# YangHai-1218/SCFlow

Measured on AMD Instinct MI355X. Metric: image-pairs/sec at 256x256, 8 GRU iters, higher is better.
Workload: dtype f32

## Files before the change

### include/scflow_hip.h

```cpp
#ifndef SCFLOW_HIP_H
#define SCFLOW_HIP_H

#include <stdint.h>

#ifdef __cplusplus
extern "C" {
#endif

typedef void* scf_stream_t;

enum {
  SCF_OK = 0,
  SCF_EINVAL = -1,
  SCF_EUNSUPPORTED = -2,
  SCF_ELAUNCH = -3,
  SCF_ENODEVICE = -4
};

#define SCF_MAX_LEVELS 12

enum { SCF_ACT_NONE = 0, SCF_ACT_RELU = 1, SCF_ACT_SIGMOID = 2, SCF_ACT_TANH = 3 };

enum {
  SCF_CONV_PLAIN = 0,
  SCF_CONV_GRU_ZR = 1,
  SCF_CONV_GRU_Q = 2
};

#define SCF_ABI_MAJOR 5
#define SCF_VERSION (SCF_ABI_MAJOR * 100 + 3)
int scf_version(void);
const char* scf_error_string(int code);
int scf_device_count(void);

int scf_corr_build(const float* feat1, const float* feat2, float* const* levels,
                   int N, int C, int h, int w, int L, scf_stream_t stream);

int scf_corr_lookup(const float* const* levels, const float* flow, float* out,
                    int N, int h, int w, int r, int L, scf_stream_t stream);

int64_t scf_corr_level_floats(int h, int w, int level, int tiled);
unsigned scf_corr_preferred_layout(int h, int w, int r, int L);
int scf_corr_build_ex(const float* feat1, const float* feat2, float* const* levels, int N, int C,
                      int h, int w, int L, unsigned tiled_levels, scf_stream_t stream);
int scf_corr_lookup_ex(const float* const* levels, const float* flow, float* out, int N, int h,
                       int w, int r, int L, unsigned tiled_levels, scf_stream_t stream);

typedef struct scf_conv_desc {
  const float* in0; const float* in1;
  int32_t C0, C1;
  int64_t in0_nstride, in1_nstride;
  int32_t N, H, W;
  const float* wp;
  int64_t w_nstride;
  int32_t Mld;
  int32_t Cout;
  int32_t KH, KW, stride, pad_h, pad_w;
  int32_t KC;
  float* out; int64_t out_nstride;
  const float* bias;
  const float* scale; const float* shift;
  const float* res; int64_t res_nstride;
  float out_div;
  int32_t act, act2, act_split;
  int32_t mode;
  const float* gru_h; int64_t gru_h_nstride;
  float* gru_aux; int64_t gru_aux_nstride;
  const float* gru_z; int64_t gru_z_nstride;
  const void* wp_f16;
  const float* wp_a4;
  int32_t a4_groups;
  int32_t a4_mld;
  const float* wp_a4s;
  int32_t a4s_groups;
  const float* wp_thin;
  int32_t out_tile8x4;
  const float* wp_taps;
  const float* wp_a4t;
  int32_t a4t_groups;
  const float* wp_wino1d;
  const float* wp_wino;
  const float* wp_wino1d4;
  int32_t k_slices;
  int64_t out_slice_stride;
} scf_conv_desc;

int scf_conv2d(const scf_conv_desc* desc, scf_stream_t stream);

int scf_conv_workspace(scf_stream_t stream, float* ptr, int64_t floats);

int scf_conv2d_pair(const scf_conv_desc* a, const scf_conv_desc* b, scf_stream_t stream);

int64_t scf_pack_conv_weight_size(int Cout, int Cin, int KH, int KW, int KC);
int scf_pack_conv_weight(const float* w, int Cout, int Cin, int KH, int KW, int KC, float* out);
int64_t scf_pack_conv_weight_a4_size(int Cout, int Cin, int KH, int KW, int groups);
int scf_pack_conv_weight_a4(const float* w, int Cout, int Cin, int KH, int KW, int groups, float* out);
int64_t scf_pack_conv_weight_taps_size(int Cout, int Cin, int KH, int KW);
int scf_pack_conv_weight_taps(const float* w, int Cout, int Cin, int KH, int KW, float* out);
int64_t scf_pack_conv_weight_wino1d_size(int32_t Cout, int32_t Cin);
int scf_pack_conv_weight_wino1d(const float* w, int32_t Cout, int32_t Cin, float* out);
int64_t scf_pack_conv_weight_wino1d4_size(int32_t Cout, int32_t Cin);
int scf_pack_conv_weight_wino1d4(const float* w, int32_t Cout, int32_t Cin, float* out);
int64_t scf_pack_conv_weight_wino_size(int32_t Cout, int32_t Cin);
int scf_pack_conv_weight_wino(const float* w, int32_t Cout, int32_t Cin, float* out);

typedef struct scf_gru_pass {
  int32_t KH, KW, pad_h, pad_w;
  const float* wp_zr; const float* bias_zr;
  const float* wp_q; const float* bias_q;
  const float* wp_zr_a4; const float* wp_q_a4; int32_t a4_groups;
  const void* wp_zr_f16; const void* wp_q_f16;
  const float* wp_zr_k32; const float* wp_q_k32;
  const float* wp_zr_a4s; const float* wp_q_a4s; int32_t a4s_groups;
  const float* wp_zr_a4t; const float* wp_q_a4t; int32_t a4t_groups;
  const float* wp_zr_wino1d; const float* wp_q_wino1d;
  const float* wp_zr_wino1d4; const float* wp_q_wino1d4;
} scf_gru_pass;

int scf_sepconv_gru(float* hx, int64_t hx_nstride, int N, int Ch, int Cx, int H, int W,
                    const scf_gru_pass* passes, int npass, float* z, float* rh,
                    scf_stream_t stream);

int scf_sepconv_gru_ctx(float* hx, int64_t hx_nstride, int N, int Ch, int Cc, int Cx, int H, int W,
                        const scf_gru_pass* passes, int npass, const float* const* ctx,
                        int64_t ctx_nstride, float* z, float* rh, scf_stream_t stream);

typedef struct scf_iter_gn {
  const float* gamma; const float* beta; float* out;
  int32_t C, HW, G; float eps;
} scf_iter_gn;

typedef struct scf_scflow_iter {
  int32_t struct_size;
  int32_t N, H, W, h, w;
  int32_t L, radius; uint32_t tiled_levels; int32_t corr_channels;
  const float* levels[SCF_MAX_LEVELS];
  float* flow_lr;
  float* corr;
  int32_t mask_flow, mask_corr;
  const float* mask_prev;
  float* flow_masked;
  scf_conv_desc flow0, flow1, corr0, corr1, outn;
  float* flow_copy_dst;
  float* hx; int64_t hx_nstride; int32_t Ch, Cc, Cx, npass;
  scf_gru_pass gru[2];
  const float* ctx[2]; int64_t ctx_nstride;
  float* z; float* rh;
  scf_conv_desc heads, fpred, mpred, menc0, menc1, denc0, denc1;
  scf_conv_desc pose[3];
  scf_iter_gn gn[3];
  const float* fc1_w; const float* fc1_b; float* fc1_out; int32_t fc1_K, fc1_O;
  const float* fc2_w; const float* fc2_b; float* fc2_out; int32_t fc2_O;
  int32_t fc_fused, fc1_slices, fc2_slices;
  const float* rot_w; const float* rot_b; float* rot_all; int32_t rot_O;
  const float* trans_w; const float* trans_b; float* trans_all; int32_t trans_O;
  const int64_t* label; int32_t num_class, label_mode;
  const float* depth; const float* K; const float* R0; const float* t0; float invalid_flow_num;
  const float* flow_in;
  const float* R_in; const float* t_in;
  float* flow_out; float* flow_pred; float* mask_up;
  float* R_out; float* t_out; float* d_rot; float* d_trans;
  scf_stream_t side_stream; int32_t overlap_flow, overlap_mask, overlap_up;
  void* lookup_timer;
} scf_scflow_iter;

int scf_scflow_iteration(const scf_scflow_iter* iter, scf_stream_t stream);

int scf_instance_norm(const float* x, const float* res, float* out, int64_t planes,
                      int HW, float eps, int relu, scf_stream_t stream);

int scf_group_norm_relu(const float* x, const float* gamma, const float* beta, float* out,
                        int N, int C, int HW, int G, float eps, scf_stream_t stream);
int scf_group_norm_relu_parts(const float* x, int parts, int64_t part_stride, const float* gamma,
                              const float* beta, float* out, int N, int C, int HW, int G, float eps,
                              scf_stream_t stream);

int scf_linear(const float* x, const float* W, const float* b, float* y, int N, int K,
               int O, int act, scf_stream_t stream);

int scf_linear_pair(const float* x, const float* W1, const float* b1, float* y1, int O1,
                    const float* W2, const float* b2, float* y2, int O2, int N, int K, int act,
                    scf_stream_t stream);

typedef struct scf_fc_desc {
  const float* x; int32_t x_parts; int64_t x_part_stride;
  const float* x_bias; int32_t x_relu;
  int32_t gn_groups, gn_hw; const float* gn_gamma; const float* gn_beta; float gn_eps;
  int32_t N, K;
  const float* W; const float* bias; float* y; int32_t O;
  const float* W2; const float* bias2; float* y2; int32_t O2;
  int32_t act;
  int32_t slices;
} scf_fc_desc;
int scf_fc_splitk(const scf_fc_desc* desc, scf_stream_t stream);

#define SCF_POSE_LABEL_PER_SAMPLE 1
#define SCF_POSE_DEPTH_LINEAR 2
int scf_pose_update(const float* rot_all, const float* trans_all, const int64_t* label,
                    int num_class, int label_mode, const float* R_in, const float* t_in,
                    float* d_rot, float* d_trans, float* R_out, float* t_out, int N,
                    scf_stream_t stream);

int scf_reproject_flow(const float* depth, const float* K, const float* R0, const float* t0,
                       const float* R, const float* t, float* flow, int N, int H, int W,
                       float invalid_num, scf_stream_t stream);

int scf_pose_error(const double* verts, int nv, const double* gt_r, const double* gt_t,
                   const double* pred_r, const double* pred_t, const double* K,
                   const int* sample_idx, int nsel, int symmetric, double* err3d, double* err2d,
                   scf_stream_t stream);

int scf_flow_corr_2d3d(const float* flow, const float* depth, const float* occ, float occ_thresh,
                       const float* K, const float* R0, const float* t0, int N, int H, int W,
                       float* pts2d, float* pts3d, float* conf, int32_t* count, scf_stream_t stream);

enum { SCF_PNP_SAMPLE_ALL = 0, SCF_PNP_SAMPLE_TOPK = 1, SCF_PNP_SAMPLE_RANDOM = 2 };
typedef struct scf_pnp_params {
  int32_t iterations;
  float reproj_error;
  int32_t sample_mode;
  int32_t sample_num;
  uint64_t seed;
} scf_pnp_params;
int64_t scf_pnp_workspace_bytes(int N, int capacity, const scf_pnp_params* params);
int scf_pnp_ransac(const float* pts2d, const float* pts3d, const float* conf, const int32_t* count, int N,
                   int capacity, const float* K, const float* R_ref, const float* t_ref,
                   const scf_pnp_params* params, float* R, float* t, int32_t* ok, int32_t* inliers,
                   void* workspace, scf_stream_t stream);

typedef struct scf_mesh_store {
  const float* verts;
  const float* normals;
  const float* colors;
  const int32_t* faces;
  const int32_t* vert_offset;
  const int32_t* face_offset;
  int32_t num_classes;
  int32_t max_faces;
} scf_mesh_store;
typedef struct scf_render_params {
  int32_t H, W;
  int32_t default_lights;
  int32_t seperate_lights;
  float background[3];
  float norm_mean[3];
  float norm_std[3];
} scf_render_params;
double scf_render_pixel_coord(int index, int size, int other);
int64_t scf_render_workspace_bytes(int N, int max_faces);
int scf_render_mesh(const scf_mesh_store* mesh, const int32_t* labels, const float* R, const float* t,
                    const float* K, int N, const scf_render_params* params, float* zbuf, int32_t* pix_to_face,
                    float* rgba, float* rgb_nchw, void* workspace, scf_stream_t stream);

typedef struct scf_patch_params {
  double aspect_ratio;
  double size_ratio;
  double min_expand;
  int32_t out_h, out_w;
  int32_t resize;
  int32_t vertex_stride;
  int32_t keep_ratio;
  int32_t clip_border;
  int32_t fix_clip_border_quirk;
  int32_t center;
  int32_t to_rgb;
  int32_t crop_pad_val[3];
  int32_t pad_val[3];
  float mean[3];
  float std[3];
} scf_patch_params;
int64_t scf_patch_workspace_bytes(int N);
int scf_patch_boxes(const scf_mesh_store* mesh, const int32_t* labels, const float* R, const float* t,
                    const float* K, const int32_t* crop_in, int N, int frame_h, int frame_w,
                    const scf_patch_params* params, float* box, int32_t* crop, float* scale, float* transform_matrix,
                    float* k, int32_t* valid, void* workspace, scf_stream_t stream);
int scf_patch_extract(const uint8_t* frames, int F, int frame_h, int frame_w, const int32_t* frame_index, int N,
                      const void* workspace, const scf_patch_params* params, float* out, scf_stream_t stream);

int scf_filter_flow_by_mask(float* flow, const float* mask, int N, int H, int W,
                            float invalid_num, int align_corners, scf_stream_t stream);

int64_t scf_cal_epe_workspace_bytes(int N, int H, int W);
int scf_cal_epe(const float* flow_tgt, const float* flow_pred, const float* mask, int N, int H, int W,
                float max_flow, const float* threshs, int nthr, int fix_threshold_quirk, float* err_map,
                float* mean, float* ratios, float* total_mean, float* total_ratios, void* workspace,
                scf_stream_t stream);

int scf_unproject_depth(const float* depth, const float* K, const float* R0, const float* t0,
                        float* pts, int N, int H, int W, scf_stream_t stream);

int scf_resize_bilinear(const float* a, const float* b, float* out, int64_t planes, int Hin,
                        int Win, int Hout, int Wout, float mul, scf_stream_t stream);

int scf_convex_upsample(const float* x, const float* mask, float* out, int N, int C, int h,
                        int w, int scale, float x_mul, float mask_mul, scf_stream_t stream);

int scf_avgpool2x2(const float* x, float* out, int64_t planes, int Hin, int Win,
                   scf_stream_t stream);

int scf_mul_mask(const float* x, int64_t x_nstride, const float* mask, float* out,
                 int64_t out_nstride, int N, int C, int HW, scf_stream_t stream);

int scf_copy_strided(const float* src, int64_t src_nstride, float* dst, int64_t dst_nstride,
                     int N, int64_t count, scf_stream_t stream);

#ifdef __cplusplus
}
#endif
#endif
```

### include/scflow_hip_prof.h

```cpp
#ifndef SCFLOW_HIP_PROF_H
#define SCFLOW_HIP_PROF_H

#include "scflow_hip.h"

#ifdef __cplusplus
extern "C" {
#endif

typedef void* scf_timer_t;
int scf_timer_create(scf_timer_t* timer);
int scf_timer_destroy(scf_timer_t timer);
int scf_timer_elapsed_us(scf_timer_t timer, float* microseconds);
int scf_timer_arm(scf_timer_t timer);

int scf_conv2d_query(const scf_conv_desc* desc, int32_t* info);

enum {
  SCF_KERNEL_THIN = 1,
  SCF_KERNEL_TAPS = 2,
  SCF_KERNEL_WINO = 3,
  SCF_KERNEL_WINO1D = 4,
  SCF_KERNEL_F16X3 = 5,
  SCF_KERNEL_DMA = 6,
  SCF_KERNEL_MFMA = 7,
  SCF_KERNEL_MFMA_KSPLIT = 8,
  SCF_KERNEL_WINO_Q = 9,
  SCF_KERNEL_WINO1D4 = 10
};
typedef struct scf_conv_log_entry {
  int32_t kernel;
  int32_t Cin, Cout, KH, KW, stride, Ho, Wo, N;
  int32_t mode;
  int32_t paired;
  int32_t variant;
} scf_conv_log_entry;
int scf_conv_log_enable(int capacity);
enum {
  SCF_TUNE_WINO_VARIANT = 1,
  SCF_TUNE_DMA_FORCE_KSPLIT = 2,
  SCF_TUNE_DMA_KSPLIT_GROUPS = 3,
  SCF_TUNE_WINO1D4 = 4,
  SCF_TUNE_CONV_AUTOSLICE = 7,
  SCF_TUNE_LOOKUP_STORE = 6,
  SCF_TUNE_ITER_MERGE = 8,
  SCF_TUNE_WINO1D4_HALF = 9,
  SCF_TUNE_CONV_PAIR = 10,
  SCF_TUNE_LOOKUP_PIPE = 5
};
int scf_tune(int key, int value);
int scf_conv_log_read(scf_conv_log_entry* out, int max_entries);

#ifdef __cplusplus
}
#endif
#endif
```

### scflow_amd/_lib.py

```python
from __future__ import annotations

import ctypes as C
import os

_HERE = os.path.dirname(os.path.abspath(__file__))
LIB_PATH = os.path.join(_HERE, 'csrc', 'libscflow_hip.so')

SCF_OK = 0
ACT_NONE, ACT_RELU, ACT_SIGMOID, ACT_TANH = 0, 1, 2, 3
CONV_PLAIN, CONV_GRU_ZR, CONV_GRU_Q = 0, 1, 2
MAX_LEVELS = 12
ABI_MAJOR = 5

_fp = C.c_void_p


class ConvDesc(C.Structure):
    _fields_ = [
        ('in0', _fp), ('in1', _fp),
        ('C0', C.c_int32), ('C1', C.c_int32),
        ('in0_nstride', C.c_int64), ('in1_nstride', C.c_int64),
        ('N', C.c_int32), ('H', C.c_int32), ('W', C.c_int32),
        ('wp', _fp), ('w_nstride', C.c_int64),
        ('Mld', C.c_int32), ('Cout', C.c_int32),
        ('KH', C.c_int32), ('KW', C.c_int32), ('stride', C.c_int32),
        ('pad_h', C.c_int32), ('pad_w', C.c_int32), ('KC', C.c_int32),
        ('out', _fp), ('out_nstride', C.c_int64),
        ('bias', _fp), ('scale', _fp), ('shift', _fp),
        ('res', _fp), ('res_nstride', C.c_int64),
        ('out_div', C.c_float),
        ('act', C.c_int32), ('act2', C.c_int32), ('act_split', C.c_int32),
        ('mode', C.c_int32),
        ('gru_h', _fp), ('gru_h_nstride', C.c_int64),
        ('gru_aux', _fp), ('gru_aux_nstride', C.c_int64),
        ('gru_z', _fp), ('gru_z_nstride', C.c_int64),
        ('wp_f16', _fp),
        ('wp_a4', _fp),
        ('a4_groups', C.c_int32),
        ('a4_mld', C.c_int32),
        ('wp_a4s', _fp),
        ('a4s_groups', C.c_int32),
        ('wp_thin', _fp),
        ('out_tile8x4', C.c_int32),
        ('wp_taps', _fp),
        ('wp_a4t', _fp),
        ('a4t_groups', C.c_int32),
        ('wp_wino1d', _fp),
        ('wp_wino', _fp),
        ('wp_wino1d4', _fp),
        ('k_slices', C.c_int32),
        ('out_slice_stride', C.c_int64),
    ]


class GruPass(C.Structure):
    _fields_ = [
        ('KH', C.c_int32), ('KW', C.c_int32), ('pad_h', C.c_int32), ('pad_w', C.c_int32),
        ('wp_zr', _fp), ('bias_zr', _fp), ('wp_q', _fp), ('bias_q', _fp),
        ('wp_zr_a4', _fp), ('wp_q_a4', _fp), ('a4_groups', C.c_int32),
        ('wp_zr_f16', _fp), ('wp_q_f16', _fp),
        ('wp_zr_k32', _fp), ('wp_q_k32', _fp),
        ('wp_zr_a4s', _fp), ('wp_q_a4s', _fp), ('a4s_groups', C.c_int32),
        ('wp_zr_a4t', _fp), ('wp_q_a4t', _fp), ('a4t_groups', C.c_int32),
        ('wp_zr_wino1d', _fp), ('wp_q_wino1d', _fp),
        ('wp_zr_wino1d4', _fp), ('wp_q_wino1d4', _fp),
    ]


class ConvLogEntry(C.Structure):
    _fields_ = [(n, C.c_int32) for n in ('kernel', 'Cin', 'Cout', 'KH', 'KW', 'stride', 'Ho', 'Wo', 'N', 'mode', 'paired', 'variant')]


KERNEL_NAMES = {1: 'thin', 2: 'taps', 3: 'winograd', 4: 'winograd F(2,5)', 5: 'f16x3', 6: 'direct-dma',
                7: 'direct-mfma', 8: 'direct-mfma-ksplit', 9: 'winograd-q', 10: 'winograd F(4,5)'}


class FcDesc(C.Structure):
    _fields_ = [('x', _fp), ('x_parts', C.c_int32), ('x_part_stride', C.c_int64),
                ('x_bias', _fp), ('x_relu', C.c_int32),
                ('gn_groups', C.c_int32), ('gn_hw', C.c_int32), ('gn_gamma', _fp), ('gn_beta', _fp), ('gn_eps', C.c_float),
                ('N', C.c_int32), ('K', C.c_int32),
                ('W', _fp), ('bias', _fp), ('y', _fp), ('O', C.c_int32),
                ('W2', _fp), ('bias2', _fp), ('y2', _fp), ('O2', C.c_int32),
                ('act', C.c_int32), ('slices', C.c_int32)]


class PnpParams(C.Structure):
    _fields_ = [('iterations', C.c_int32), ('reproj_error', C.c_float), ('sample_mode', C.c_int32),
                ('sample_num', C.c_int32), ('seed', C.c_uint64)]


PNP_SAMPLE_ALL, PNP_SAMPLE_TOPK, PNP_SAMPLE_RANDOM = 0, 1, 2


class MeshStore(C.Structure):
    _fields_ = [('verts', _fp), ('normals', _fp), ('colors', _fp), ('faces', _fp), ('vert_offset', _fp),
                ('face_offset', _fp), ('num_classes', C.c_int32), ('max_faces', C.c_int32)]


class RenderParams(C.Structure):
    _fields_ = [('H', C.c_int32), ('W', C.c_int32), ('default_lights', C.c_int32), ('seperate_lights', C.c_int32),
                ('background', C.c_float * 3), ('norm_mean', C.c_float * 3), ('norm_std', C.c_float * 3)]


class PatchParams(C.Structure):
    _fields_ = [('aspect_ratio', C.c_double), ('size_ratio', C.c_double), ('min_expand', C.c_double),
                ('out_h', C.c_int32), ('out_w', C.c_int32), ('resize', C.c_int32), ('vertex_stride', C.c_int32),
                ('keep_ratio', C.c_int32), ('clip_border', C.c_int32), ('fix_clip_border_quirk', C.c_int32),
                ('center', C.c_int32), ('to_rgb', C.c_int32), ('crop_pad_val', C.c_int32 * 3),
                ('pad_val', C.c_int32 * 3), ('mean', C.c_float * 3), ('std', C.c_float * 3)]


class IterGN(C.Structure):
    _fields_ = [('gamma', _fp), ('beta', _fp), ('out', _fp),
                ('C', C.c_int32), ('HW', C.c_int32), ('G', C.c_int32), ('eps', C.c_float)]


class ScflowIter(C.Structure):
    _fields_ = [
        ('struct_size', C.c_int32),
        ('N', C.c_int32), ('H', C.c_int32), ('W', C.c_int32), ('h', C.c_int32), ('w', C.c_int32),
        ('L', C.c_int32), ('radius', C.c_int32), ('tiled_levels', C.c_uint32), ('corr_channels', C.c_int32),
        ('levels', _fp * MAX_LEVELS),
        ('flow_lr', _fp), ('corr', _fp),
        ('mask_flow', C.c_int32), ('mask_corr', C.c_int32), ('mask_prev', _fp), ('flow_masked', _fp),
        ('flow0', ConvDesc), ('flow1', ConvDesc), ('corr0', ConvDesc), ('corr1', ConvDesc), ('outn', ConvDesc),
        ('flow_copy_dst', _fp),
        ('hx', _fp), ('hx_nstride', C.c_int64), ('Ch', C.c_int32), ('Cc', C.c_int32), ('Cx', C.c_int32),
        ('npass', C.c_int32),
        ('gru', GruPass * 2), ('ctx', _fp * 2), ('ctx_nstride', C.c_int64), ('z', _fp), ('rh', _fp),
        ('heads', ConvDesc), ('fpred', ConvDesc), ('mpred', ConvDesc), ('menc0', ConvDesc), ('menc1', ConvDesc),
        ('denc0', ConvDesc), ('denc1', ConvDesc),
        ('pose', ConvDesc * 3), ('gn', IterGN * 3),
        ('fc1_w', _fp), ('fc1_b', _fp), ('fc1_out', _fp), ('fc1_K', C.c_int32), ('fc1_O', C.c_int32),
        ('fc2_w', _fp), ('fc2_b', _fp), ('fc2_out', _fp), ('fc2_O', C.c_int32),
        ('fc_fused', C.c_int32), ('fc1_slices', C.c_int32), ('fc2_slices', C.c_int32),
        ('rot_w', _fp), ('rot_b', _fp), ('rot_all', _fp), ('rot_O', C.c_int32),
        ('trans_w', _fp), ('trans_b', _fp), ('trans_all', _fp), ('trans_O', C.c_int32),
        ('label', _fp), ('num_class', C.c_int32), ('label_mode', C.c_int32),
        ('depth', _fp), ('K', _fp), ('R0', _fp), ('t0', _fp), ('invalid_flow_num', C.c_float),
        ('flow_in', _fp), ('R_in', _fp), ('t_in', _fp),
        ('flow_out', _fp), ('flow_pred', _fp), ('mask_up', _fp),
        ('R_out', _fp), ('t_out', _fp), ('d_rot', _fp), ('d_trans', _fp),
        ('side_stream', _fp), ('overlap_flow', C.c_int32), ('overlap_mask', C.c_int32), ('overlap_up', C.c_int32),
        ('lookup_timer', _fp),
    ]


SIGNATURES = {
    'scf_version': (C.c_int, []),
    'scf_error_string': (C.c_char_p, [C.c_int]),
    'scf_device_count': (C.c_int, []),
    'scf_corr_build': (C.c_int, [_fp, _fp, C.POINTER(_fp), C.c_int, C.c_int, C.c_int, C.c_int,
                                 C.c_int, _fp]),
    'scf_corr_lookup': (C.c_int, [C.POINTER(_fp), _fp, _fp, C.c_int, C.c_int, C.c_int, C.c_int,
                                  C.c_int, _fp]),
    'scf_corr_build_ex': (C.c_int, [_fp, _fp, C.POINTER(_fp), C.c_int, C.c_int, C.c_int, C.c_int,
                                    C.c_int, C.c_uint, _fp]),
    'scf_corr_lookup_ex': (C.c_int, [C.POINTER(_fp), _fp, _fp, C.c_int, C.c_int, C.c_int, C.c_int,
                                     C.c_int, C.c_uint, _fp]),
    'scf_corr_level_floats': (C.c_int64, [C.c_int, C.c_int, C.c_int, C.c_int]),
    'scf_corr_preferred_layout': (C.c_uint, [C.c_int, C.c_int, C.c_int, C.c_int]),
    'scf_pose_error': (C.c_int, [_fp, C.c_int, _fp, _fp, _fp, _fp, _fp, _fp, C.c_int, C.c_int, _fp, _fp, _fp]),
    'scf_filter_flow_by_mask': (C.c_int, [_fp, _fp, C.c_int, C.c_int, C.c_int, C.c_float, C.c_int, _fp]),
    'scf_cal_epe_workspace_bytes': (C.c_int64, [C.c_int, C.c_int, C.c_int]),
    'scf_cal_epe': (C.c_int, [_fp, _fp, _fp, C.c_int, C.c_int, C.c_int, C.c_float, C.POINTER(C.c_float), C.c_int, C.c_int,
                              _fp, _fp, _fp, _fp, _fp, _fp, _fp]),
    'scf_timer_create': (C.c_int, [C.POINTER(_fp)]),
    'scf_timer_destroy': (C.c_int, [_fp]),
    'scf_timer_arm': (C.c_int, [_fp]),
    'scf_timer_elapsed_us': (C.c_int, [_fp, C.POINTER(C.c_float)]),
    'scf_conv2d': (C.c_int, [C.POINTER(ConvDesc), _fp]),
    'scf_conv2d_pair': (C.c_int, [C.POINTER(ConvDesc), C.POINTER(ConvDesc), _fp]),
    'scf_conv2d_query': (C.c_int, [C.POINTER(ConvDesc), C.POINTER(C.c_int32)]),
    'scf_tune': (C.c_int, [C.c_int, C.c_int]),
    'scf_conv_log_enable': (C.c_int, [C.c_int]),
    'scf_conv_log_read': (C.c_int, [C.POINTER(ConvLogEntry), C.c_int]),
    'scf_pack_conv_weight_size': (C.c_int64, [C.c_int, C.c_int, C.c_int, C.c_int, C.c_int]),
    'scf_pack_conv_weight': (C.c_int, [_fp, C.c_int, C.c_int, C.c_int, C.c_int, C.c_int, _fp]),
    'scf_pack_conv_weight_a4_size': (C.c_int64, [C.c_int, C.c_int, C.c_int, C.c_int, C.c_int]),
    'scf_pack_conv_weight_a4': (C.c_int, [_fp, C.c_int, C.c_int, C.c_int, C.c_int, C.c_int, _fp]),
    'scf_pack_conv_weight_taps_size': (C.c_int64, [C.c_int, C.c_int, C.c_int, C.c_int]),
    'scf_pack_conv_weight_taps': (C.c_int, [_fp, C.c_int, C.c_int, C.c_int, C.c_int, _fp]),
    'scf_pack_conv_weight_wino1d_size': (C.c_int64, [C.c_int32, C.c_int32]),
    'scf_pack_conv_weight_wino1d': (C.c_int, [_fp, C.c_int32, C.c_int32, _fp]),
    'scf_pack_conv_weight_wino1d4_size': (C.c_int64, [C.c_int32, C.c_int32]),
    'scf_pack_conv_weight_wino1d4': (C.c_int, [_fp, C.c_int32, C.c_int32, _fp]),
    'scf_pack_conv_weight_wino_size': (C.c_int64, [C.c_int32, C.c_int32]),
    'scf_pack_conv_weight_wino': (C.c_int, [_fp, C.c_int32, C.c_int32, _fp]),
    'scf_sepconv_gru': (C.c_int, [_fp, C.c_int64, C.c_int, C.c_int, C.c_int, C.c_int, C.c_int,
                                  C.POINTER(GruPass), C.c_int, _fp, _fp, _fp]),
    'scf_sepconv_gru_ctx': (C.c_int, [_fp, C.c_int64, C.c_int, C.c_int, C.c_int, C.c_int, C.c_int,
                                      C.c_int, C.POINTER(GruPass), C.c_int, C.POINTER(_fp),
                                      C.c_int64, _fp, _fp, _fp]),
    'scf_scflow_iteration': (C.c_int, [C.POINTER(ScflowIter), _fp]),
    'scf_instance_norm': (C.c_int, [_fp, _fp, _fp, C.c_int64, C.c_int, C.c_float, C.c_int, _fp]),
    'scf_group_norm_relu': (C.c_int, [_fp, _fp, _fp, _fp, C.c_int, C.c_int, C.c_int, C.c_int,
                                      C.c_float, _fp]),
    'scf_conv_workspace': (C.c_int, [_fp, _fp, C.c_int64]),
    'scf_group_norm_relu_parts': (C.c_int, [_fp, C.c_int, C.c_int64, _fp, _fp, _fp, C.c_int, C.c_int, C.c_int, C.c_int,
                                            C.c_float, _fp]),
    'scf_fc_splitk': (C.c_int, [C.POINTER(FcDesc), _fp]),
    'scf_linear': (C.c_int, [_fp, _fp, _fp, _fp, C.c_int, C.c_int, C.c_int, C.c_int, _fp]),
    'scf_linear_pair': (C.c_int, [_fp, _fp, _fp, _fp, C.c_int, _fp, _fp, _fp, C.c_int, C.c_int, C.c_int,
                                  C.c_int, _fp]),
    'scf_pose_update': (C.c_int, [_fp, _fp, _fp, C.c_int, C.c_int, _fp, _fp, _fp, _fp, _fp, _fp,
                                  C.c_int, _fp]),
    'scf_reproject_flow': (C.c_int, [_fp, _fp, _fp, _fp, _fp, _fp, _fp, C.c_int, C.c_int,
                                     C.c_int, C.c_float, _fp]),
    'scf_flow_corr_2d3d': (C.c_int, [_fp, _fp, _fp, C.c_float, _fp, _fp, _fp, C.c_int, C.c_int, C.c_int,
                                     _fp, _fp, _fp, _fp, _fp]),
    'scf_pnp_workspace_bytes': (C.c_int64, [C.c_int, C.c_int, C.POINTER(PnpParams)]),
    'scf_pnp_ransac': (C.c_int, [_fp, _fp, _fp, _fp, C.c_int, C.c_int, _fp, _fp, _fp, C.POINTER(PnpParams),
                                 _fp, _fp, _fp, _fp, _fp, _fp]),
    'scf_render_pixel_coord': (C.c_double, [C.c_int, C.c_int, C.c_int]),
    'scf_render_workspace_bytes': (C.c_int64, [C.c_int, C.c_int]),
    'scf_render_mesh': (C.c_int, [C.POINTER(MeshStore), _fp, _fp, _fp, _fp, C.c_int, C.POINTER(RenderParams),
                                  _fp, _fp, _fp, _fp, _fp, _fp]),
    'scf_patch_workspace_bytes': (C.c_int64, [C.c_int]),
    'scf_patch_boxes': (C.c_int, [C.POINTER(MeshStore), _fp, _fp, _fp, _fp, _fp, C.c_int, C.c_int, C.c_int,
                                  C.POINTER(PatchParams), _fp, _fp, _fp, _fp, _fp, _fp, _fp, _fp]),
    'scf_patch_extract': (C.c_int, [_fp, C.c_int, C.c_int, C.c_int, _fp, C.c_int, _fp, C.POINTER(PatchParams), _fp,
                                    _fp]),
    'scf_unproject_depth': (C.c_int, [_fp, _fp, _fp, _fp, _fp, C.c_int, C.c_int, C.c_int, _fp]),
    'scf_resize_bilinear': (C.c_int, [_fp, _fp, _fp, C.c_int64, C.c_int, C.c_int, C.c_int,
                                      C.c_int, C.c_float, _fp]),
    'scf_convex_upsample': (C.c_int, [_fp, _fp, _fp, C.c_int, C.c_int, C.c_int, C.c_int, C.c_int,
                                      C.c_float, C.c_float, _fp]),
    'scf_avgpool2x2': (C.c_int, [_fp, _fp, C.c_int64, C.c_int, C.c_int, _fp]),
    'scf_mul_mask': (C.c_int, [_fp, C.c_int64, _fp, _fp, C.c_int64, C.c_int, C.c_int, C.c_int, _fp]),
    'scf_copy_strided': (C.c_int, [_fp, C.c_int64, _fp, C.c_int64, C.c_int, C.c_int64, _fp]),
}

_lib = None


class ScflowHipError(RuntimeError):
    pass


def load() -> C.CDLL:
    global _lib
    if _lib is not None:
        return _lib
    if not os.path.exists(LIB_PATH):
        raise ScflowHipError(
            f'{LIB_PATH} is missing: the HIP kernels are the product and there is no fallback. '
            'Build it with `python scflow_amd/csrc/build.py` (hipcc --offload-arch=gfx950).')
    lib = C.CDLL(LIB_PATH)
    lib.scf_version.restype = C.c_int
    have = lib.scf_version()
    if have // 100 != ABI_MAJOR:
        raise ScflowHipError(f'{LIB_PATH} was built with ABI major {have // 100}, this binding expects '
                             f'{ABI_MAJOR}: rebuild it (python scflow_amd/csrc/build.py --force)')
    for name, (res, args) in SIGNATURES.items():
        fn = getattr(lib, name)
        fn.restype = res
        fn.argtypes = args
    _lib = lib
    return lib


def check(code: int, what: str) -> None:
    if code != SCF_OK:
        msg = load().scf_error_string(code).decode()
        raise ScflowHipError(f'{what} failed: {msg} ({code})')
```

### scflow_amd/csrc/conv_kernels.h

```cpp
#pragma once
#include "scf_common.h"

struct ConvK {
  const float* in0; const float* in1;
  int C0, Cin;
  long long in0_ns, in1_ns;
  int H, W, Ho, Wo;
  const float* wp; long long w_ns;
  const void* wp16;
  const float* wthin;
  const float* wp4; int G4, Mld4;
  const float* wp4s; int G4s;
  const float* wp4t; int G4t;
  int Mld, Cout, Krows;
  int KH, KW, T, stride, pad_h, pad_w, KC, nchunk;
  int fc_log2, tiles_x, tiles_y, mblocks, PH, PW, PWin;
  int px_off;
  int in_step;
  int wvec;
  int out_tile;
  int ksplit;
  float* out; long long out_ns;
  const float* bias; const float* scale; const float* shift;
  const float* res; long long res_ns;
  float out_div;
  int out_div_pow2;
  int act, act2, act_split, mode;
  const float* gru_h; long long gru_h_ns;
  float* gru_aux; long long gru_aux_ns;
  const float* gru_z; long long gru_z_ns;
  int kslices;
  long long slice_ns;
  int slice_blocks;
};

struct ConvEpi {
  float* out; const float* res; const float* gru_h; float* gru_aux; const float* gru_z;
  int HWo;
};

__device__ __forceinline__ ConvEpi scf_conv_epi(const ConvK& p, int n) {
  ConvEpi e;
  e.out = p.out + (long long)n * p.out_ns;
  e.res = p.res ? p.res + (long long)n * p.res_ns : nullptr;
  e.gru_h = p.gru_h ? p.gru_h + (long long)n * p.gru_h_ns : nullptr;
  e.gru_aux = p.gru_aux ? p.gru_aux + (long long)n * p.gru_aux_ns : nullptr;
  e.gru_z = p.gru_z ? p.gru_z + (long long)n * p.gru_z_ns : nullptr;
  e.HWo = p.Ho * p.Wo;
  return e;
}

typedef float scf_f32x16 __attribute__((ext_vector_type(16)));
typedef float scf_f32x4 __attribute__((ext_vector_type(4)));

enum { SCF_EPI_AFFINE = 0, SCF_EPI_GENERAL = 1, SCF_EPI_GRU_ZR = 2, SCF_EPI_GRU_Q = 3 };

__device__ __forceinline__ int scf_conv_epi_kind(const ConvK& p) {
  if (p.mode == SCF_CONV_GRU_ZR) return SCF_EPI_GRU_ZR;
  if (p.mode == SCF_CONV_GRU_Q) return SCF_EPI_GRU_Q;
  const bool lin1 = p.act == SCF_ACT_NONE || p.act == SCF_ACT_RELU;
  const bool lin2 = p.act_split <= 0 || p.act2 == SCF_ACT_NONE || p.act2 == SCF_ACT_RELU;
  return (lin1 && lin2) ? SCF_EPI_AFFINE : SCF_EPI_GENERAL;
}

__device__ __forceinline__ void scf_epi_affine_group(const ConvK& p, const ConvEpi& e,
                                                     const float (&acc)[4], int cb, int pix,
                                                     bool use_div) {
  if (cb >= p.Cout) return;
  const bool full = cb + 3 < p.Cout;
  float v[4] = {acc[0], acc[1], acc[2], acc[3]};
  if (use_div) {
    if (p.out_div_pow2) {
      const float rd = 1.0f / p.out_div;
#pragma unroll
      for (int q = 0; q < 4; ++q) v[q] = v[q] * rd;
    } else {
#pragma unroll
      for (int q = 0; q < 4; ++q) v[q] = v[q] / p.out_div;
    }
  }
  int off = cb * e.HWo + pix;
  float r[4] = {0.f, 0.f, 0.f, 0.f};
  if (e.res) {
#pragma unroll
    for (int q = 0; q < 4; ++q)
      if (full || cb + q < p.Cout) r[q] = e.res[off + q * e.HWo];
  }
  if (p.bias) {
#pragma unroll
    for (int q = 0; q < 4; ++q) v[q] += p.bias[(full || cb + q < p.Cout) ? cb + q : cb];
  }
  if (p.scale) {
#pragma unroll
    for (int q = 0; q < 4; ++q) {
      const int c = (full || cb + q < p.Cout) ? cb + q : cb;
      v[q] = v[q] * p.scale[c] + p.shift[c];
    }
  }
  if (e.res) {
#pragma unroll
    for (int q = 0; q < 4; ++q) v[q] += r[q];
  }
#pragma unroll
  for (int q = 0; q < 4; ++q) {
    const int a = (p.act_split > 0 && cb + q >= p.act_split) ? p.act2 : p.act;
    if (a == SCF_ACT_RELU) v[q] = v[q] > 0.f ? v[q] : 0.f;
  }
#pragma unroll
  for (int q = 0; q < 4; ++q)
    if (full || cb + q < p.Cout) e.out[off + q * e.HWo] = v[q];
}

template <int KIND>
__device__ __forceinline__ void scf_epi_general_group(const ConvK& p, const ConvEpi& e,
                                                      const float (&acc)[4], int cb, int pix,
                                                      bool use_div) {
  const bool need_aux = (KIND == SCF_EPI_GENERAL) ? (e.res != nullptr) : true;
// ... 260 lines not shown
```

### scflow_amd/csrc/conv_mfma.hip

```cpp
#include <atomic>
#include <mutex>
#include <vector>
#include "scf_common.h"

typedef float f32x16 __attribute__((ext_vector_type(16)));
typedef float f32x4 __attribute__((ext_vector_type(4)));

#include "conv_kernels.h"

template <int WM, int WN, int NCP>
__device__ __forceinline__ void mfma_taps(f32x16 (&acc)[WM][WN], const float* wl, const float* pl,
                                          const int (&boff)[WN], int T, int KW, int KC, int BM,
                                          int PW, int PHW, int half, int l32) {
  for (int t = 0; t < T; ++t) {
    const int ky = t / KW, kx = t - ky * KW;
    const float* wt = wl + (t * KC + half) * BM + l32;
    const float* pt = pl + ky * PW + kx;
#pragma unroll
    for (int c = 0; c < NCP; ++c) {
      const int cp = 2 * c;
      float a[WM], b[WN];
#pragma unroll
      for (int i = 0; i < WM; ++i) a[i] = wt[cp * BM + i * 32];
#pragma unroll
// ... 272 lines not shown
      for (int t = 0; t < T; ++t) {
        const int ky = t / p.KW, kx = t - ky * p.KW;
        const float* wt = wl + (t * KC + half) * BM + l32;
        const float* pt = pl + ky * PW + kx + boff;
#pragma unroll
        for (int c = 0; c < NCP; ++c) {
          if (((t * NCP + c) & 3) == wave)
            acc = __builtin_amdgcn_mfma_f32_32x32x2f32(wt[2 * c * BM], pt[2 * c * PHW], acc, 0, 0, 0);
        }
      }
    }
  }

  __syncthreads();
  float* red = lds;
#pragma unroll
  for (int r = 0; r < 16; ++r) red[(wave * 16 + r) * 64 + lane] = acc[r];
  __syncthreads();
  float v[4];
#pragma unroll
  for (int q = 0; q < 4; ++q) {
    const int r = 4 * wave + q;
    v[q] = ((red[(0 * 16 + r) * 64 + lane] + red[(1 * 16 + r) * 64 + lane]) +
            red[(2 * 16 + r) * 64 + lane]) + red[(3 * 16 + r) * 64 + lane];
  }
  const int oy = ty0 + fr, ox = tx0 + fc;
  if (oy < p.Ho && ox < p.Wo) {
    const ConvEpi epi = scf_conv_epi(p, n);
    const int pixk = p.out_tile ? (((oy >> 2) * (p.Wo >> 3) + (ox >> 3)) * 32 + (oy & 3) * 8 + (ox & 7))
                                : oy * p.Wo + ox;
    scf_conv_epilogue_group(p, epi, v, m0 + 8 * wave + 4 * half, pixk, p.out_div != 1.0f);
  }
}

template <int KC>
static int launch_ksplit(const ConvK& k, int nblk, size_t lds_bytes, hipStream_t st) {
  scf_launch((conv_mfma_ksplit_kernel<KC>), dim3(nblk), dim3(256), lds_bytes, st, k);
  return scf_launch_status();
}

template <int WM, int WN>
static int launch_conv(const ConvK& k, int nblk, size_t lds_bytes, hipStream_t st) {
  if (k.KC == 32)
    scf_launch((conv_mfma_kernel<WM, WN, 32>), dim3(nblk), dim3(256), lds_bytes, st, k);
  else if (k.KC == 8)
    scf_launch((conv_mfma_kernel<WM, WN, 8>), dim3(nblk), dim3(256), lds_bytes, st, k);
  else
    scf_launch((conv_mfma_kernel<WM, WN, 2>), dim3(nblk), dim3(256), lds_bytes, st, k);
  return scf_launch_status();
}

static int next_pow2(int v) {
  int p = 1;
  while (p < v) p <<= 1;
  return p;
}

struct ConvPlan {
  ConvK k;
  int WM, WN;
  long long nblk;
  size_t lds_bytes;
};

static int conv_plan(const scf_conv_desc* d, ConvPlan* plan) {
  if (!d || !d->in0 || !d->wp || !d->out) return SCF_EINVAL;
  if (d->N <= 0 || d->H <= 0 || d->W <= 0 || d->C0 <= 0 || d->C1 < 0 || d->Cout <= 0) return SCF_EINVAL;
  if (d->KH <= 0 || d->KW <= 0 || d->stride <= 0 || d->pad_h < 0 || d->pad_w < 0) return SCF_EINVAL;
  if (d->C1 > 0 && !d->in1) return SCF_EINVAL;
  if (d->KC != 2 && d->KC != 8 && d->KC != 32) return SCF_EUNSUPPORTED;
  if (d->C1 > 0 && (d->C0 % d->KC) != 0) return SCF_EUNSUPPORTED;
  if (d->Mld < d->Cout) return SCF_EINVAL;
  if (d->mode == SCF_CONV_GRU_ZR && (!d->gru_h || !d->gru_aux || (d->Cout & 1))) return SCF_EINVAL;
  if (d->mode == SCF_CONV_GRU_Q && (!d->gru_h || !d->gru_z)) return SCF_EINVAL;
  if ((d->scale == nullptr) != (d->shift == nullptr)) return SCF_EINVAL;
  if (d->out_tile8x4 && (d->mode != SCF_CONV_PLAIN || d->res)) return SCF_EUNSUPPORTED;
  if (d->k_slices > 1) {
    if (d->k_slices > 16 || d->out_slice_stride < (int64_t)d->N * d->out_nstride) return SCF_EINVAL;
    if (d->bias || d->scale || d->res || d->act != SCF_ACT_NONE || d->act_split > 0 || d->mode != SCF_CONV_PLAIN ||
        d->out_tile8x4 || (d->out_div != 0.f && d->out_div != 1.f) || d->w_nstride != 0)
      return SCF_EINVAL;
  }

  ConvK& k = plan->k;
  k.in0 = d->in0; k.in1 = d->C1 > 0 ? d->in1 : nullptr;
  k.C0 = d->C0; k.Cin = d->C0 + d->C1;
  k.in0_ns = d->in0_nstride; k.in1_ns = d->in1_nstride;
  k.H = d->H; k.W = d->W;
  k.Ho = (d->H + 2 * d->pad_h - d->KH) / d->stride + 1;
  k.Wo = (d->W + 2 * d->pad_w - d->KW) / d->stride + 1;
  if (k.Ho <= 0 || k.Wo <= 0) return SCF_EINVAL;
  k.wp = d->wp; k.w_ns = d->w_nstride; k.Mld = d->Mld; k.Cout = d->Cout;
  k.wp16 = d->wp_f16;
  k.wthin = d->wp_thin;
  k.wp4 = d->wp_a4; k.G4 = d->a4_groups; k.Mld4 = d->a4_mld;
  k.wp4s = d->wp_a4s; k.G4s = d->a4s_groups;
  k.wp4t = d->wp_a4t; k.G4t = d->a4t_groups;
  k.out_tile = d->out_tile8x4;
  k.KH = d->KH; k.KW = d->KW; k.T = d->KH * d->KW; k.stride = d->stride; k.in_step = 1;
  k.pad_h = d->pad_h; k.pad_w = d->pad_w; k.KC = d->KC;
  k.nchunk = (k.Cin + k.KC - 1) / k.KC;
  k.Krows = d->w_nstride ? k.Cin * k.T : k.nchunk * k.KC * k.T;
  k.wvec = ((d->Mld & 3) == 0) && ((d->w_nstride & 3) == 0) && (((uintptr_t)d->wp & 15) == 0);
  k.out = d->out; k.out_ns = d->out_nstride;
  k.bias = d->bias; k.scale = d->scale; k.shift = d->shift;
  k.res = d->res; k.res_ns = d->res_nstride;
  k.out_div = d->out_div == 0.f ? 1.f : d->out_div;
  {
    int ex = 0;
    k.out_div_pow2 = (k.out_div > 0.f && frexpf(k.out_div, &ex) == 0.5f) ? 1 : 0;
  }
  k.act = d->act; k.act2 = d->act2; k.act_split = d->act_split; k.mode = d->mode;
  k.gru_h = d->gru_h; k.gru_h_ns = d->gru_h_nstride;
  k.gru_aux = d->gru_aux; k.gru_aux_ns = d->gru_aux_nstride;
  k.gru_z = d->gru_z; k.gru_z_ns = d->gru_z_nstride;
  k.kslices = d->k_slices > 1 ? d->k_slices : 1; k.slice_ns = d->out_slice_stride; k.slice_blocks = 0;

  int FC = next_pow2(k.Wo) < 32 ? next_pow2(k.Wo) : 32;
  if (k.Wo > 32) {
    int best_w = (k.Wo + 31) / 32 * 32;
    for (int c = 16; c >= 8; c >>= 1) {
      const int wpad = (k.Wo + c - 1) / c * c;
      if (wpad * 10 <= best_w * 9) { best_w = wpad; FC = c; }
    }
  }
  int fl = 0;
  while ((1 << fl) < FC) ++fl;
  k.fc_log2 = fl;
  const int FR = 32 / FC;

  const int frags_m = (k.Cout + 31) / 32;
  auto tiles = [&](int WN) {
    const int TR = WN * 4 * FR;
    return (long long)d->N * ((k.Ho + TR - 1) / TR) * ((k.Wo + FC - 1) / FC);
  };
  auto fits = [&](int WM, int WN, size_t* lds_out) {
    const int TR = WN * 4 * FR;
    const int PH = (TR - 1) * k.stride + k.KH, PW = (FC - 1) * k.stride + k.KW;
    const long long PE = (long long)k.KC * PH * PW, WE = (long long)k.KC * k.T * WM * 8;
    const size_t lds = ((size_t)k.KC * k.T * WM * 32 + (size_t)PE) * sizeof(float);
    if (lds_out) *lds_out = lds;
    return (PE + 255) / 256 <= pu_max(k.KC, WM * WN) && (WE + 255) / 256 <= wu_max(k.KC) && lds <= 64 * 1024;
  };
  int WM = frags_m >= 4 ? ((frags_m % 4 == 0 || frags_m % 3 != 0) ? 4 : 3) : frags_m;
  int WN = 1;
  auto nblocks = [&](int wm, int wn) { return tiles(wn) * ((frags_m + wm - 1) / wm); };
  while (WM > 1 && (nblocks(WM, 1) < 512 || !fits(WM, 1, nullptr))) {
    int next = WM - 1;
    while (next > 1 && frags_m % next != 0) --next;
    WM = next;
  }
  if (WM <= 2 && nblocks(WM, 2) >= 2048 && fits(WM, 2, nullptr)) WN = 2;
  size_t lds_bytes = 0;
  const bool normal_fits = fits(WM, WN, &lds_bytes);
  k.mblocks = (frags_m + WM - 1) / WM;
  {
    const int TR = WN * 4 * FR;
    k.PH = (TR - 1) * k.stride + k.KH;
    k.PW = (FC - 1) * k.stride + k.KW;
    k.tiles_y = (k.Ho + TR - 1) / TR;
    k.tiles_x = (k.Wo + FC - 1) / FC;
  }
  plan->nblk = (long long)d->N * k.tiles_y * k.tiles_x * k.mblocks;
  if (plan->nblk > 0x7fffffffLL) return SCF_EUNSUPPORTED;
  k.ksplit = 0;
  if (!normal_fits && !(WM == 1 && WN == 1)) return SCF_EUNSUPPORTED;
  if (WM == 1 && WN == 1 && (plan->nblk < 128 || !normal_fits)) {
    const int PHk = (FR - 1) * k.stride + k.KH, PWk = (FC - 1) * k.stride + k.KW;
    const long long PEk = (long long)k.KC * PHk * PWk, WEk = (long long)k.KC * k.T * 8;
    size_t ldsk = ((size_t)k.KC * k.T * 32 + (size_t)PEk) * sizeof(float);
    if (ldsk < 4 * 16 * 64 * sizeof(float)) ldsk = 4 * 16 * 64 * sizeof(float);
    if ((PEk + 255) / 256 <= pu_max(k.KC, 1) && (WEk + 255) / 256 <= wu_max(k.KC) && ldsk <= 64 * 1024) {
      k.ksplit = 1;
      k.PH = PHk; k.PW = PWk;
      k.tiles_y = (k.Ho + FR - 1) / FR;
      k.tiles_x = (k.Wo + FC - 1) / FC;
      k.mblocks = frags_m;
      lds_bytes = ldsk;
      plan->nblk = (long long)d->N * k.tiles_y * k.tiles_x * k.mblocks;
    }
  }
  if (!normal_fits && !k.ksplit) return SCF_EUNSUPPORTED;
  plan->WM = WM; plan->WN = WN; plan->lds_bytes = lds_bytes;
  return SCF_OK;
}

static bool want_f16x3(const scf_conv_desc* d) {
  return d->wp_f16 != nullptr && !d->out_tile8x4 && d->w_nstride == 0 && d->KH * d->KW > 1 && d->C0 + d->C1 >= 16;
}

static std::atomic<int> g_pair_mode{0};
static std::atomic<int> g_wino1d4{1};

static bool want_dma(const scf_conv_desc* d) {
  return (d->wp_a4 != nullptr || d->wp_a4s != nullptr) && (d->stride == 1 || d->stride == 2) &&
         d->w_nstride == 0 && d->a4_mld >= d->Cout;
}

int scf_conv_kcombine_launch(const ConvK& k, const float* parts, int S, long long slice_ns, int N, hipStream_t st);
int scf_conv_dma_autoslice(const ConvK& k, int N);
namespace {
struct KWorkspace { hipStream_t st; float* ptr; int64_t floats; };
std::mutex g_kws_mu;
std::vector<KWorkspace> g_kws;
std::atomic<int> g_autoslice{1};
}
extern "C" int scf_conv_workspace(scf_stream_t stream, float* ptr, int64_t floats) {
  if (floats < 0 || (ptr == nullptr) != (floats == 0)) return SCF_EINVAL;
  std::lock_guard<std::mutex> lk(g_kws_mu);
  hipStream_t st = scf_stream(stream);
  for (size_t i = 0; i < g_kws.size(); ++i)
    if (g_kws[i].st == st) {
      if (ptr) { g_kws[i].ptr = ptr; g_kws[i].floats = floats; }
      else g_kws.erase(g_kws.begin() + (long)i);
      return SCF_OK;
    }
  if (ptr) g_kws.push_back({st, ptr, floats});
  return SCF_OK;
}
static bool kws_lookup(hipStream_t st, float** ptr, int64_t* floats) {
  std::lock_guard<std::mutex> lk(g_kws_mu);
  for (const KWorkspace& w : g_kws)
    if (w.st == st) { *ptr = w.ptr; *floats = w.floats; return true; }
  return false;
}

struct ConvReq {
  int32_t* info = nullptr;
  ScfLaunchCap* cap = nullptr;
  int which = 0;
};

static int conv2d_walk(const scf_conv_desc* d, scf_stream_t stream, ConvReq& r) {
  ConvPlan pl;
  const int rc = conv_plan(d, &pl);
  if (rc != SCF_OK) return rc;
  const ConvK& k = pl.k;
  const int N = d->N;
  const bool dry = r.info || r.cap;
  int32_t scratch[4];
  int32_t* info = r.info ? r.info : r.cap ? scratch : nullptr;
  hipStream_t st = scf_stream(stream);
  int out = SCF_EUNSUPPORTED;
  auto took = [&](int which, int rf) { r.which = which; out = rf; return rf != SCF_EUNSUPPORTED; };
  if (d->k_slices > 1) {
    r.which = SCF_KERNEL_DMA;
    return want_dma(d) ? scf_conv_dma_dispatch(k, N, dry, info, st, r.cap) : SCF_EUNSUPPORTED;
  }
  if (took(SCF_KERNEL_THIN, scf_conv_thin_dispatch(k, N, dry, st, r.cap))) return out;
  if (d->wp_taps && took(SCF_KERNEL_TAPS, scf_conv_taps_dispatch(k, d->wp_taps, N, dry, info, st, r.cap))) return out;
  if (d->wp_wino) {
    int quarter = 0;
    const int rw = scf_conv_wino_dispatch(k, d->wp_wino, N, dry, info, st, &quarter, r.cap);
    if (took(quarter ? SCF_KERNEL_WINO_Q : SCF_KERNEL_WINO, rw)) return out;
  }
  const int w4 = g_wino1d4.load(std::memory_order_relaxed);
  if (d->wp_wino1d4 && w4 && took(SCF_KERNEL_WINO1D4, scf_conv_wino1d4_dispatch(k, d->wp_wino1d4, N, w4 == 2, dry, info, st)))
    return out;
  if (d->wp_wino1d && took(SCF_KERNEL_WINO1D, scf_conv_wino1d_dispatch(k, d->wp_wino1d, N, dry, info, st))) return out;
  if (want_f16x3(d) && took(SCF_KERNEL_F16X3, scf_conv_f16x3_dispatch(k, N, dry, info, st))) return out;
  if (want_dma(d)) {
    float* ws = nullptr;
    int64_t ws_floats = 0;
    const bool sliced = !r.info && g_autoslice.load(std::memory_order_relaxed) && kws_lookup(st, &ws, &ws_floats);
    if (sliced && !dry) {
      const int S = scf_conv_dma_autoslice(k, N);
      const int64_t per_slice = (int64_t)N * d->Cout * k.Ho * k.Wo;
      if (S > 1 && per_slice * S <= ws_floats) {
        ConvK part = k;
        part.out = ws; part.out_ns = (long long)d->Cout * k.Ho * k.Wo;
        part.bias = nullptr; part.scale = nullptr; part.shift = nullptr; part.res = nullptr; part.res_ns = 0;
        part.out_div = 1.f; part.out_div_pow2 = 1; part.act = SCF_ACT_NONE; part.act2 = SCF_ACT_NONE; part.act_split = 0;
        part.mode = SCF_CONV_PLAIN; part.gru_h = nullptr; part.gru_aux = nullptr; part.gru_z = nullptr;
        part.kslices = S; part.slice_ns = per_slice;
        r.which = SCF_KERNEL_DMA;
        const int rs = scf_conv_dma_dispatch(part, N, false, nullptr, st);
        if (rs == SCF_OK) return scf_conv_kcombine_launch(k, ws, S, per_slice, N, st);
        if (rs != SCF_EUNSUPPORTED) return rs;
      }
    }
    if (took(SCF_KERNEL_DMA, scf_conv_dma_dispatch(k, N, dry, info, st, r.cap))) {
      if (sliced && r.cap) r.cap->variant = -1;
      return out;
    }
  }
  r.which = k.ksplit ? SCF_KERNEL_MFMA_KSPLIT : SCF_KERNEL_MFMA;
  const int WM = pl.WM, WN = pl.WN;
  if (dry) {
    if (r.info) {
      r.info[0] = WM; r.info[1] = WN; r.info[2] = (int32_t)pl.nblk;
      r.info[3] = k.T * (k.KC / 2) * WM * WN / (k.ksplit ? 4 : 1);
    }
    return SCF_OK;
  }
  const int nblk = (int)pl.nblk;
  if (k.ksplit) {
    if (k.KC == 32) return launch_ksplit<32>(k, nblk, pl.lds_bytes, st);
    if (k.KC == 8) return launch_ksplit<8>(k, nblk, pl.lds_bytes, st);
    return launch_ksplit<2>(k, nblk, pl.lds_bytes, st);
  }
#define SCF_CASE(M, Nn) if (WM == M && WN == Nn) return launch_conv<M, Nn>(k, nblk, pl.lds_bytes, st);
  SCF_CASE(1, 1) SCF_CASE(1, 2) SCF_CASE(2, 1) SCF_CASE(2, 2)
  SCF_CASE(3, 1) SCF_CASE(4, 1)
#undef SCF_CASE
  return SCF_EUNSUPPORTED;
}

namespace {
std::mutex g_log_mu;
std::vector<scf_conv_log_entry> g_log;
std::atomic<int> g_log_cap{0};
}

int scf_wino_variant_set(int v);
int scf_dma_force_ksplit_set(int v);
int scf_dma_ksplit_groups_set(int v);
int scf_lookup_pipe_set(int v);
int scf_lookup_store_set(int v);
int scf_iter_merge_set(int v);
int scf_wino1d4_half_set(int v);

extern "C" int scf_tune(int key, int value) {
  if (key == SCF_TUNE_WINO_VARIANT) return scf_wino_variant_set(value);
  if (key == SCF_TUNE_DMA_FORCE_KSPLIT) return scf_dma_force_ksplit_set(value);
  if (key == SCF_TUNE_DMA_KSPLIT_GROUPS) return scf_dma_ksplit_groups_set(value);
  if (key == SCF_TUNE_LOOKUP_PIPE) return scf_lookup_pipe_set(value);
  if (key == SCF_TUNE_LOOKUP_STORE) return scf_lookup_store_set(value);
  if (key == SCF_TUNE_ITER_MERGE) return scf_iter_merge_set(value);
  if (key == SCF_TUNE_WINO1D4_HALF) return scf_wino1d4_half_set(value);
  if (key == SCF_TUNE_CONV_AUTOSLICE) {
    if (value < 0 || value > 1) return SCF_EINVAL;
    return g_autoslice.exchange(value);
  }
  if (key == SCF_TUNE_CONV_PAIR) {
    if (value < 0 || value > 1) return SCF_EINVAL;
    return g_pair_mode.exchange(value);
  }
  if (key == SCF_TUNE_WINO1D4) {
    if (value < 0 || value > 2) return SCF_EINVAL;
    return g_wino1d4.exchange(value);
  }
  return SCF_EINVAL;
}

extern "C" int scf_conv_log_enable(int capacity) {
  std::lock_guard<std::mutex> lk(g_log_mu);
  g_log.clear();
  if (capacity > 0) g_log.reserve((size_t)capacity);
  else g_log.shrink_to_fit();
  g_log_cap.store(capacity > 0 ? capacity : 0);
  return SCF_OK;
}

extern "C" int scf_conv_log_read(scf_conv_log_entry* out, int max_entries) {
  std::lock_guard<std::mutex> lk(g_log_mu);
  const int n = (int)g_log.size();
  if (out)
    for (int i = 0; i < n && i < max_entries; ++i) out[i] = g_log[(size_t)i];
  return n;
}

static void conv_log_push(const scf_conv_desc* d, int which, int paired, int variant = -1);
extern "C" int scf_conv2d(const scf_conv_desc* d, scf_stream_t stream) {
  ConvReq r;
  const int rc = conv2d_walk(d, stream, r);
  if (rc == SCF_OK) conv_log_push(d, r.which, 0);
  return rc;
}

static void conv_log_push(const scf_conv_desc* d, int which, int paired, int variant) {
  if (g_log_cap.load(std::memory_order_relaxed) <= 0) return;
  std::lock_guard<std::mutex> lk(g_log_mu);
  if ((int)g_log.size() >= g_log_cap.load()) return;
  scf_conv_log_entry e;
  e.kernel = which; e.Cin = d->C0 + d->C1; e.Cout = d->Cout; e.KH = d->KH; e.KW = d->KW; e.stride = d->stride;
  e.Ho = (d->H + 2 * d->pad_h - d->KH) / d->stride + 1;
  e.Wo = (d->W + 2 * d->pad_w - d->KW) / d->stride + 1;
  e.N = d->N; e.mode = d->mode; e.paired = paired; e.variant = variant;
  g_log.push_back(e);
}

static bool pairable(int which, const ScfLaunchCap& c) {
  switch (which) {
    case SCF_KERNEL_THIN: return true;
    case SCF_KERNEL_TAPS: return c.variant >= 1;
    case SCF_KERNEL_WINO_Q: return c.variant >= 10 && c.variant < 20;
    case SCF_KERNEL_WINO: return c.variant >= 20;
    case SCF_KERNEL_DMA: return c.variant >= 0;
    default: return false;
  }
}

static bool capture(const scf_conv_desc* d, scf_stream_t stream, ScfLaunchCap* cap, int* which) {
  ConvReq r;
  r.cap = cap;
  const bool ok = conv2d_walk(d, stream, r) == SCF_OK && pairable(r.which, *cap);
  *which = r.which;
  return ok;
}

typedef int (*PairLaunch)(const ScfLaunchCap&, const ScfLaunchCap&, hipStream_t);

extern "C" int scf_conv2d_pair(const scf_conv_desc* a, const scf_conv_desc* b, scf_stream_t stream) {
  if (!a || !b) return SCF_EINVAL;
  ScfLaunchCap ca, cb;
  int fa = 0, fb = 0;
  if (g_pair_mode.load(std::memory_order_relaxed) != 1 && capture(a, stream, &ca, &fa) && capture(b, stream, &cb, &fb)) {
    const size_t lmax = ca.ldsb > cb.ldsb ? ca.ldsb : cb.ldsb;
    const long long slots = (long long)scf_cu_count() * (((fa == SCF_KERNEL_DMA || fb == SCF_KERNEL_DMA) && lmax > 80 * 1024) ? 1 : 2);
    const long long na = ca.nblk, nb = cb.nblk;
    auto rounds = [](long long n, long long s) { return (n + s - 1) / s; };
    auto fewer_rounds = [&](long long s) { return rounds(na + nb, s) < rounds(na, s) + rounds(nb, s); };
// ... 128 lines not shown
```

### scflow_amd/csrc/conv_taps.hip

```cpp
#include "scf_common.h"
#include "conv_kernels.h"
#include "scf_dma.h"

#include "conv_taps_body.h"

template <int WM>
__global__ __launch_bounds__(256, 2) void conv_taps_kernel(ConvK p, const float* __restrict__ wt, int Kp, int PWp) {
  conv_taps_body<WM>(p, wt, Kp, PWp, (int)blockIdx.x, (int)gridDim.x);
}

template <int WMA, int WMB>
__global__ __launch_bounds__(256, 2) void conv_taps_pair_kernel(ConvK pa, const float* __restrict__ wta, int Kpa, int PWpa, ConvK pb,
                                                                const float* __restrict__ wtb, int Kpb, int PWpb, int nba) {
  if ((int)blockIdx.x < nba) conv_taps_body<WMA>(pa, wta, Kpa, PWpa, (int)blockIdx.x, nba);
  else conv_taps_body<WMB>(pb, wtb, Kpb, PWpb, (int)blockIdx.x - nba, (int)gridDim.x - nba);
}

#define CT_MAXU 12

template <int WM>
__global__ __launch_bounds__(256, 2) void conv_taps_persist_kernel(ConvK p, const float* __restrict__ wt, int Kp, int PWp, int ntiles) {
  extern __shared__ __attribute__((aligned(16))) float ct_lds[];
  constexpr int BM = WM * 32;
  const int tid = threadIdx.x, lane = tid & 63;
  const int wave = __builtin_amdgcn_readfirstlane(tid >> 6);
  const int l32 = lane & 31, half = lane >> 5;

  const int lb = scf_xcd_remap(blockIdx.x, gridDim.x);
  const int mblk = __builtin_amdgcn_readfirstlane(lb % p.mblocks);
  const int slot = __builtin_amdgcn_readfirstlane(lb / p.mblocks);
  const int nslots = __builtin_amdgcn_readfirstlane((int)gridDim.x / p.mblocks);
  const int m0 = mblk * BM;
  const int FC = 1 << p.fc_log2, FR = 32 >> p.fc_log2, TR = 4 * FR;
  const int st = p.stride;
  const int PH = p.PH, PHW = PH * PWp, T = p.T;
  const int q4 = BM / 4, n4 = Kp * q4;
  const int w_cells = (n4 + 63) & ~63;
  const int PE = p.Cin * PHW;
  const int x_cells = (PE + 63) & ~63;
  float* Ws = ct_lds;
  float* Xs = Ws + w_cells * 4;
  int* koff = (int*)(Xs + 2 * x_cells);
  const int HW = p.H * p.W;

  int rel[CT_MAXU], pyx[CT_MAXU];
  {
    const float rPHW = 1.0f / (float)PHW, rPW = 1.0f / (float)PWp;
#pragma unroll
    for (int u = 0; u < CT_MAXU; ++u) {
      rel[u] = -1; pyx[u] = 0;
      if (wave * 64 + u * 256 >= x_cells) continue;
      const int e = wave * 64 + u * 256 + lane;
      int c = (int)((float)e * rPHW);
      int r = e - c * PHW;
      if (r < 0) { --c; r += PHW; } else if (r >= PHW) { ++c; r -= PHW; }
      int py = (int)((float)r * rPW);
      int px = r - py * PWp;
      if (px < 0) { --py; px += PWp; } else if (px >= PWp) { ++py; px -= PWp; }
      rel[u] = e < PE ? c * HW + py * p.W + px : -1;
      pyx[u] = (py << 16) | px;
    }
  }
  auto tile_coords = [&](int tile, int& n, int& ty0, int& tx0) {
    const int txi = __builtin_amdgcn_readfirstlane(tile % p.tiles_x);
    const int t2 = tile / p.tiles_x;
    const int tyi = __builtin_amdgcn_readfirstlane(t2 % p.tiles_y);
    n = __builtin_amdgcn_readfirstlane(t2 / p.tiles_y);
    ty0 = tyi * TR; tx0 = txi * FC;
  };
  const unsigned xl = scf_lds_addr(Xs);
  auto stage_x = [&](int tile, int b) {
    int n, ty0, tx0;
    tile_coords(tile, n, ty0, tx0);
    const int iy0 = ty0 * st - p.pad_h, ix0 = tx0 * st - p.pad_w;
    const scf_rsrc4 xrs = scf_make_rsrc(p.in0 + (long long)n * p.in0_ns, (unsigned)((long long)p.Cin * HW * 4));
    const int tbase = iy0 * p.W + ix0;
    const unsigned dst = xl + (unsigned)(b * x_cells + wave * 64) * 4u;
#pragma unroll
    for (int u = 0; u < CT_MAXU; ++u) {
      if (wave * 64 + u * 256 < x_cells) {
        const int iy = iy0 + (pyx[u] >> 16), ix = ix0 + (pyx[u] & 0xffff);
        const bool ok = rel[u] >= 0 && (unsigned)iy < (unsigned)p.H && (unsigned)ix < (unsigned)p.W;
        scf_bdma_b32(xrs, ok ? (unsigned)((rel[u] + tbase) * 4) : SCF_BUF_OOB, dst + (unsigned)u * 1024u);
      }
    }
  };

  {
    const scf_rsrc4 wrs = scf_make_rsrc(wt + m0, (unsigned)(((long long)(Kp - 1) * p.Mld + BM) * 4));
    const unsigned wl = scf_lds_addr(Ws);
    for (int c0 = wave * 64; c0 < w_cells; c0 += 256) {
      const int e = c0 + lane;
      const int row = e / q4, c4 = e - row * q4;
      const unsigned voff = e < n4 ? (unsigned)((row * p.Mld + 4 * c4) * 4) : SCF_BUF_OOB;
      scf_bdma_b128(wrs, voff, wl + (unsigned)c0 * 16u);
    }
  }
  if (slot < ntiles) stage_x(slot, 0);
  for (int k = tid; k < Kp; k += 256) {
    int o = 0;
    if (k < p.Cin * T) {
      const int c = k / T, t = k - c * T;
      const int ky = t / p.KW, kx = t - ky * p.KW;
      o = c * PHW + ky * PWp + kx;
    }
    koff[k] = o;
  }
  __builtin_amdgcn_s_waitcnt(0x0F70);
  __syncthreads();

  const int fr = l32 >> p.fc_log2, fc = l32 & (FC - 1);
  const float* wb = Ws + half * BM + l32;
  const int* kb = koff + half;
  const int ntrip = Kp >> 3;
  int buf = 0;
#pragma nounroll
  for (int tile = slot; tile < ntiles; tile += nslots) {
    if (tile + nslots < ntiles) stage_x(tile + nslots, buf ^ 1);

    ct_f32x16 acc[WM][1];
#pragma unroll
    for (int i = 0; i < WM; ++i)
#pragma unroll
      for (int r = 0; r < 16; ++r) acc[i][0][r] = 0.f;

    const float* xb = Xs + buf * x_cells + ((wave * FR + fr) * st) * PWp + fc * st;
    int oN[4];
    float bC[4], aC[4][WM];
#pragma unroll
    for (int u = 0; u < 4; ++u) oN[u] = kb[2 * u];
#pragma unroll
    for (int u = 0; u < 4; ++u) {
      bC[u] = xb[oN[u]];
#pragma unroll
      for (int i = 0; i < WM; ++i) aC[u][i] = wb[2 * u * BM + 32 * i];
    }
    {
      const int t1 = ntrip > 1 ? 1 : 0;
#pragma unroll
      for (int u = 0; u < 4; ++u) oN[u] = kb[8 * t1 + 2 * u];
    }
#pragma nounroll
    for (int t = 0; t < ntrip; ++t) {
      const int tn = t + 1 < ntrip ? t + 1 : ntrip - 1, tnn = t + 2 < ntrip ? t + 2 : ntrip - 1;
      float bN[4], aN[4][WM];
      int oNN[4];
#pragma unroll
      for (int u = 0; u < 4; ++u) {
        bN[u] = xb[oN[u]];
#pragma unroll
        for (int i = 0; i < WM; ++i) aN[u][i] = wb[(8 * tn + 2 * u) * BM + 32 * i];
      }
#pragma unroll
      for (int u = 0; u < 4; ++u) oNN[u] = kb[8 * tnn + 2 * u];
      __builtin_amdgcn_sched_barrier(0);
#pragma unroll
      for (int u = 0; u < 4; ++u)
#pragma unroll
// ... 97 lines not shown
```

### scflow_amd/csrc/conv_taps_body.h

```cpp
#pragma once
#include "scf_common.h"
#include "conv_kernels.h"
#include "scf_dma.h"

typedef float ct_f32x16 __attribute__((ext_vector_type(16)));

template <int WM>
__device__ __forceinline__ void conv_taps_body(const ConvK& p, const float* __restrict__ wt, const int Kp, const int PWp, const int bid,
                                               const int nblk) {
  extern __shared__ __attribute__((aligned(16))) float ct_lds[];
  constexpr int BM = WM * 32;
  const int tid = threadIdx.x, lane = tid & 63;
  const int wave = __builtin_amdgcn_readfirstlane(tid >> 6);
  const int l32 = lane & 31, half = lane >> 5;

  const int lb = scf_xcd_remap(bid, nblk);
  const int mblk = __builtin_amdgcn_readfirstlane(lb % p.mblocks);
  const int tile = __builtin_amdgcn_readfirstlane(lb / p.mblocks);
  const int m0 = mblk * BM;
  const int FC = 1 << p.fc_log2, FR = 32 >> p.fc_log2, TR = 4 * FR;
  const int txi = __builtin_amdgcn_readfirstlane(tile % p.tiles_x);
  const int t2 = tile / p.tiles_x;
  const int tyi = __builtin_amdgcn_readfirstlane(t2 % p.tiles_y);
  const int n = __builtin_amdgcn_readfirstlane(t2 / p.tiles_y);
  const int ty0 = tyi * TR, tx0 = txi * FC;
  const int st = p.stride;
  const int iy0 = ty0 * st - p.pad_h, ix0 = tx0 * st - p.pad_w;
  const int PH = p.PH, PHW = PH * PWp, T = p.T;
  const int q4 = BM / 4, n4 = Kp * q4;
  const int w_cells = (n4 + 63) & ~63;
  const int PE = p.Cin * PHW;
  const int x_cells = (PE + 63) & ~63;
  float* Ws = ct_lds;
  float* Xs = Ws + w_cells * 4;
  int* koff = (int*)(Xs + x_cells);

  {
    const scf_rsrc4 wrs = scf_make_rsrc(wt + m0, (unsigned)(((long long)(Kp - 1) * p.Mld + BM) * 4));
    const unsigned wl = scf_lds_addr(Ws);
    for (int c0 = wave * 64; c0 < w_cells; c0 += 256) {
      const int e = c0 + lane;
      const int row = e / q4, c4 = e - row * q4;
      const unsigned voff = e < n4 ? (unsigned)((row * p.Mld + 4 * c4) * 4) : SCF_BUF_OOB;
      scf_bdma_b128(wrs, voff, wl + (unsigned)c0 * 16u);
    }
    const int HW = p.H * p.W;
    const scf_rsrc4 xrs = scf_make_rsrc(p.in0 + (long long)n * p.in0_ns, (unsigned)((long long)p.Cin * HW * 4));
    const unsigned xl = scf_lds_addr(Xs);
    const float rPHW = 1.0f / (float)PHW, rPW = 1.0f / (float)PWp;
    for (int c0 = wave * 64; c0 < x_cells; c0 += 256) {
      const int e = c0 + lane;
      int c = (int)((float)e * rPHW);
      int r = e - c * PHW;
      if (r < 0) { --c; r += PHW; } else if (r >= PHW) { ++c; r -= PHW; }
      int py = (int)((float)r * rPW);
      int px = r - py * PWp;
      if (px < 0) { --py; px += PWp; } else if (px >= PWp) { ++py; px -= PWp; }
      const int iy = iy0 + py, ix = ix0 + px;
      const bool ok = e < PE && iy >= 0 && iy < p.H && ix >= 0 && ix < p.W;
      scf_bdma_b32(xrs, ok ? (unsigned)((c * HW + iy * p.W + ix) * 4) : SCF_BUF_OOB, xl + (unsigned)c0 * 4u);
    }
  }
  for (int k = tid; k < Kp; k += 256) {
    int o = 0;
    if (k < p.Cin * T) {
      const int c = k / T, t = k - c * T;
      const int ky = t / p.KW, kx = t - ky * p.KW;
      o = c * PHW + ky * PWp + kx;
    }
    koff[k] = o;
  }
  __builtin_amdgcn_s_waitcnt(0x0F70);
  __syncthreads();

  ct_f32x16 acc[WM][1];
#pragma unroll
  for (int i = 0; i < WM; ++i)
#pragma unroll
    for (int r = 0; r < 16; ++r) acc[i][0][r] = 0.f;

  const int fr = l32 >> p.fc_log2, fc = l32 & (FC - 1);
  const float* xb = Xs + ((wave * FR + fr) * st) * PWp + fc * st;
  const float* wb = Ws + half * BM + l32;
  const int* kb = koff + half;
  const int ntrip = Kp >> 3;
  int oN[4];
  float bC[4], aC[4][WM];
#pragma unroll
  for (int u = 0; u < 4; ++u) oN[u] = kb[2 * u];
#pragma unroll
  for (int u = 0; u < 4; ++u) {
    bC[u] = xb[oN[u]];
#pragma unroll
    for (int i = 0; i < WM; ++i) aC[u][i] = wb[2 * u * BM + 32 * i];
  }
  {
    const int t1 = ntrip > 1 ? 1 : 0;
#pragma unroll
    for (int u = 0; u < 4; ++u) oN[u] = kb[8 * t1 + 2 * u];
  }
  for (int t = 0; t < ntrip; ++t) {
    const int tn = t + 1 < ntrip ? t + 1 : ntrip - 1, tnn = t + 2 < ntrip ? t + 2 : ntrip - 1;
    float bN[4], aN[4][WM];
    int oNN[4];
#pragma unroll
    for (int u = 0; u < 4; ++u) {
      bN[u] = xb[oN[u]];
#pragma unroll
      for (int i = 0; i < WM; ++i) aN[u][i] = wb[(8 * tn + 2 * u) * BM + 32 * i];
    }
#pragma unroll
    for (int u = 0; u < 4; ++u) oNN[u] = kb[8 * tnn + 2 * u];
    __builtin_amdgcn_sched_barrier(0);
#pragma unroll
    for (int u = 0; u < 4; ++u)
#pragma unroll
      for (int i = 0; i < WM; ++i)
        acc[i][0] = __builtin_amdgcn_mfma_f32_32x32x2f32(aC[u][i], bC[u], acc[i][0], 0, 0, 0);
    __builtin_amdgcn_sched_barrier(0);
#pragma unroll
    for (int u = 0; u < 4; ++u) {
      bC[u] = bN[u];
      oN[u] = oNN[u];
#pragma unroll
      for (int i = 0; i < WM; ++i) aC[u][i] = aN[u][i];
    }
  }

  const ConvEpi epi = scf_conv_epi(p, n);
  int pix[1];
// ... 8 lines not shown
```

### scflow_amd/csrc/corr_gemm.hip

```cpp
#include "scf_common.h"

typedef float cg_f32x16 __attribute__((ext_vector_type(16)));

struct CorrGemmParams {
  const float* f1; const float* f2;
  float* lvl0; float* lvl1;
  int C, h, w, hw;
  int nchunk;
  int mblocks, nblocks;
  int tiled;
  int ntiles_x;
  float scale; int exact_scale;
  float divisor;
  int l1_pw4, l1_msz;
};

#define CG_KC 16
#define CG_BM 128
#define CG_BN 128
#define CG_STAGE_FLOATS (CG_KC * (CG_BM + CG_BN))
#define CG_NSTAGE 3

__device__ __forceinline__ unsigned cg_lds_addr(const void* p) {
  return (unsigned)(uintptr_t)(__attribute__((address_space(3))) const void*)p;
// ... 111 lines not shown
  float* o0 = p.lvl0 + (long long)n * hw * hw;
  float* o1 = POOL ? p.lvl1 + (long long)n * hw * hw1 : nullptr;
#pragma unroll
  for (int fj = 0; fj < 2; ++fj) {
    const int F = nb * 4 + wn * 2 + fj;
    bool fok;
    int pos0, pos1 = 0;
    bool pool_lane = false;
    if (TILED) {
      const int ntile = (p.h >> 2) * p.ntiles_x;
      fok = F < ntile;
      pos0 = F * 32 + l32;
      if (POOL) {
        const int ty = F / p.ntiles_x, tx = F - ty * p.ntiles_x;
        const int x = l32 & 7, y = l32 >> 3;
        pool_lane = fok && !(x & 1) && !(y & 1);
        const int y1 = ty * 2 + (y >> 1), x1 = tx * 4 + (x >> 1);
        pos1 = p.l1_pw4 ? (y1 >> 2) * p.l1_pw4 + (x1 >> 3) * 32 + (y1 & 3) * 8 + (x1 & 7) : y1 * w1 + x1;
      }
    } else {
      pos0 = F * 32 + l32;
      fok = pos0 < hw;
    }
#pragma unroll
    for (int fi = 0; fi < 2; ++fi) {
      const int ib = i0 + wm * 64 + fi * 32 + 4 * half;
#pragma unroll
      for (int r = 0; r < 16; ++r) {
        const int i = ib + (r & 3) + 8 * (r >> 2);
        float v = acc[fi][fj][r];
        v = p.exact_scale ? v * p.scale : v / p.divisor;
        if (fok && i < hw) o0[(long long)i * hw + pos0] = v;
        if (POOL) {
          const int vi = __builtin_bit_cast(int, v);
          const float vx = __builtin_bit_cast(float, __builtin_amdgcn_update_dpp(0, vi, 0xB1, 0xF, 0xF, false));
          const float vy = __builtin_bit_cast(float, __builtin_amdgcn_update_dpp(0, vi, 0x128, 0xF, 0xF, false));
          const float vxy = __builtin_bit_cast(float, __builtin_amdgcn_update_dpp(0, __builtin_bit_cast(int, vx), 0x128, 0xF, 0xF, false));
          const float s = (((v + vx) + vy) + vxy) * 0.25f;
          if (pool_lane && i < hw) o1[(long long)i * hw1 + pos1] = s;
        }
      }
    }
  }
}

static int corr_gemm_dispatch(const float* feat1, const float* feat2, float* lvl0, float* lvl1, int l1_tiled,
                              int N, int C, int h, int w, int tiled, hipStream_t st) {
  const long long hw = (long long)h * w;
  if (C % CG_KC != 0 || (hw & 3) != 0 || hw > 0x3fffffffLL) return SCF_EUNSUPPORTED;
  if ((long long)C * hw * 4 > 0x7fffffffLL) return SCF_EUNSUPPORTED;
  if (tiled && ((w & 7) || (h & 3))) return SCF_EUNSUPPORTED;
  if (lvl1 && (!tiled || h < 2 || w < 2)) return SCF_EUNSUPPORTED;
  if ((((uintptr_t)feat1 | (uintptr_t)feat2) & 15) != 0) return SCF_EUNSUPPORTED;
  CorrGemmParams p;
  p.f1 = feat1; p.f2 = feat2; p.lvl0 = lvl0; p.lvl1 = lvl1;
  p.C = C; p.h = h; p.w = w; p.hw = (int)hw;
  p.nchunk = C / CG_KC;
  p.mblocks = (int)((hw + CG_BM - 1) / CG_BM);
  p.tiled = tiled ? 1 : 0;
  p.ntiles_x = w >> 3;
  const long long nfrag = tiled ? (long long)(h >> 2) * (w >> 3) : (hw + 31) / 32;
  p.nblocks = (int)((nfrag + 3) / 4);
  const float sq = sqrtf((float)C);
  int ex = 0;
  p.exact_scale = (frexpf(sq, &ex) == 0.5f) ? 1 : 0;
  p.scale = 1.0f / sq;
  p.divisor = sq;
  p.l1_pw4 = (lvl1 && l1_tiled) ? (((w >> 1) + 7) / 8 * 8) * 4 : 0;
  p.l1_msz = lvl1 ? (int)scf_corr_level_floats(h, w, 1, l1_tiled) : 0;
  const long long nblk = (long long)N * p.mblocks * p.nblocks;
  if (nblk <= 0 || nblk > 0x7fffffffLL) return SCF_EUNSUPPORTED;
  const size_t lds = (size_t)CG_NSTAGE * CG_STAGE_FLOATS * sizeof(float);
  if (tiled) {
    if (lvl1) scf_launch((corr_gemm_kernel<true, true>), dim3((unsigned)nblk), dim3(256), lds, st, p);
    else scf_launch((corr_gemm_kernel<true, false>), dim3((unsigned)nblk), dim3(256), lds, st, p);
  } else {
    scf_launch((corr_gemm_kernel<false, false>), dim3((unsigned)nblk), dim3(256), lds, st, p);
  }
  return scf_launch_status();
}

int scf_avgpool2x2_layout(const float* x, float* out, int64_t planes, int Hin, int Win, int in_tiled,
                          int out_tiled, hipStream_t st);

extern "C" int scf_corr_build_ex(const float* feat1, const float* feat2, float* const* levels, int N,
                                 int C, int h, int w, int L, unsigned tiled_levels, scf_stream_t stream) {
  if (!feat1 || !feat2 || !levels || N <= 0 || C <= 0 || h <= 0 || w <= 0 || L <= 0) return SCF_EINVAL;
  if (L > SCF_MAX_LEVELS) return SCF_EUNSUPPORTED;
  if ((tiled_levels & 1u) && ((w & 7) || (h & 3))) return SCF_EUNSUPPORTED;
  for (int l = 0; l < L; ++l)
    if (!levels[l] || (h >> l) < 1 || (w >> l) < 1) return SCF_EINVAL;
  hipStream_t st = scf_stream(stream);
  const int hw = h * w;
  const int t0 = tiled_levels & 1u, t1 = (tiled_levels >> 1) & 1u;
  float* l1 = (t0 && L >= 2) ? levels[1] : nullptr;
  int rc = corr_gemm_dispatch(feat1, feat2, levels[0], l1, t1, N, C, h, w, t0, st);
  int done = (rc == SCF_OK && l1) ? 2 : 1;
  if (rc == SCF_EUNSUPPORTED) {
    scf_conv_desc d = {};
    d.in0 = feat2; d.C0 = C; d.in0_nstride = (int64_t)C * hw;
    d.N = N; d.H = h; d.W = w;
    d.wp = feat1; d.w_nstride = (int64_t)C * hw; d.Mld = hw; d.Cout = hw;
    d.KH = d.KW = 1; d.stride = 1; d.pad_h = d.pad_w = 0;
    d.KC = (C % 32 == 0) ? 32 : (C % 8 == 0) ? 8 : 2;
    d.out = levels[0]; d.out_nstride = (int64_t)hw * hw;
    d.out_div = sqrtf((float)C);
    d.act = SCF_ACT_NONE; d.mode = SCF_CONV_PLAIN;
    d.out_tile8x4 = t0;
    rc = scf_conv2d(&d, stream);
    done = 1;
  }
  if (rc != SCF_OK) return rc;
  for (int l = done; l < L; ++l) {
    rc = scf_avgpool2x2_layout(levels[l - 1], levels[l], (int64_t)N * hw, h >> (l - 1), w >> (l - 1),
                               (tiled_levels >> (l - 1)) & 1u, (tiled_levels >> l) & 1u, st);
    if (rc != SCF_OK) return rc;
  }
  return SCF_OK;
}

extern "C" int scf_corr_build(const float* feat1, const float* feat2, float* const* levels, int N,
                              int C, int h, int w, int L, scf_stream_t stream) {
  return scf_corr_build_ex(feat1, feat2, levels, N, C, h, w, L, 0u, stream);
}
```

### scflow_amd/csrc/norm.hip

```cpp
#include "scf_common.h"

__device__ __forceinline__ float wave_sum(float v) {
#pragma unroll
  for (int off = 32; off > 0; off >>= 1) v += __shfl_xor(v, off);
  return v;
}

template <int NT>
__device__ __forceinline__ float block_sum(float v, float* red) {
  v = wave_sum(v);
  const int wave = threadIdx.x >> 6, lane = threadIdx.x & 63;
  __syncthreads();
  if (lane == 0) red[wave] = v;
  __syncthreads();
  float s = 0.f;
#pragma unroll
  for (int w = 0; w < NT / 64; w += 4) s += (red[w] + red[w + 1]) + (red[w + 2] + red[w + 3]);
  return s;
}

__device__ __forceinline__ float block_sum_256(float v, float* red) {
  v = wave_sum(v);
  const int wave = threadIdx.x >> 6, lane = threadIdx.x & 63;
  __syncthreads();
// ... 13 lines not shown
  const int n4 = HW >> 2;
  float4 v[VEC4];
  float s = 0.f;
#pragma unroll
  for (int i = 0; i < VEC4; ++i) {
    const int idx = i * NT + threadIdx.x;
    v[i] = idx < n4 ? xp[idx] : make_float4(0.f, 0.f, 0.f, 0.f);
    s += (v[i].x + v[i].y) + (v[i].z + v[i].w);
  }
  const float mean = block_sum<NT>(s, red) / (float)HW;
  float q = 0.f;
#pragma unroll
  for (int i = 0; i < VEC4; ++i) {
    const int idx = i * NT + threadIdx.x;
    if (idx < n4) {
      const float a = v[i].x - mean, b = v[i].y - mean, c = v[i].z - mean, d = v[i].w - mean;
      q += (a * a + b * b) + (c * c + d * d);
    }
  }
  const float var = block_sum<NT>(q, red) / (float)HW;
  const float rstd = 1.0f / sqrtf(var + eps);
  float4* op = reinterpret_cast<float4*>(out + pl * HW);
  const float4* rp = res ? reinterpret_cast<const float4*>(res + pl * HW) : nullptr;
#pragma unroll
  for (int i = 0; i < VEC4; ++i) {
    const int idx = i * NT + threadIdx.x;
    if (idx < n4) {
      float4 o;
      o.x = (v[i].x - mean) * rstd;
      o.y = (v[i].y - mean) * rstd;
      o.z = (v[i].z - mean) * rstd;
      o.w = (v[i].w - mean) * rstd;
      if (rp) {
        const float4 r = rp[idx];
        o.x += r.x; o.y += r.y; o.z += r.z; o.w += r.w;
      }
      if (relu) {
        o.x = fmaxf(o.x, 0.f); o.y = fmaxf(o.y, 0.f); o.z = fmaxf(o.z, 0.f); o.w = fmaxf(o.w, 0.f);
      }
      scf_store4<(SCF_ST_SC1 & 2) != 0>(reinterpret_cast<float*>(op + idx), o.x, o.y, o.z, o.w);
    }
  }
}

__global__ __launch_bounds__(256) void instance_norm_generic_kernel(const float* x,
                                                                    const float* res,
                                                                    float* out, int HW,
                                                                    float eps, int relu) {
  __shared__ float red[4];
  const long long pl = blockIdx.x;
  const float* xp = x + pl * HW;
  float s = 0.f;
  for (int i = threadIdx.x; i < HW; i += 256) s += xp[i];
  const float mean = block_sum_256(s, red) / (float)HW;
  float q = 0.f;
  for (int i = threadIdx.x; i < HW; i += 256) {
    const float a = xp[i] - mean;
    q += a * a;
  }
  const float var = block_sum_256(q, red) / (float)HW;
  const float rstd = 1.0f / sqrtf(var + eps);
  for (int i = threadIdx.x; i < HW; i += 256) {
    float o = (xp[i] - mean) * rstd;
    if (res) o += res[pl * HW + i];
    if (relu) o = fmaxf(o, 0.f);
    out[pl * HW + i] = o;
  }
}

extern "C" int scf_instance_norm(const float* x, const float* res, float* out, int64_t planes,
                                 int HW, float eps, int relu, scf_stream_t stream) {
  if (!x || !out || planes <= 0 || HW <= 0) return SCF_EINVAL;
  if (planes > 0x7fffffffLL) return SCF_EUNSUPPORTED;
  hipStream_t st = scf_stream(stream);
  const dim3 grid((unsigned)planes), blk(256);
  const bool vec = (HW % 4 == 0) && ((((uintptr_t)x | (uintptr_t)out | (uintptr_t)res) & 15) == 0);
  const int n4 = HW / 4;
  if (vec && n4 <= 256) scf_launch(instance_norm_kernel<1>, grid, blk, 0, st, x, res, out, HW, eps, relu);
  else if (vec && n4 <= 1024) scf_launch(instance_norm_kernel<4>, grid, blk, 0, st, x, res, out, HW, eps, relu);
  else if (vec && n4 <= 4096) scf_launch(instance_norm_kernel<16>, grid, blk, 0, st, x, res, out, HW, eps, relu);
  else if (vec && n4 <= 8192) scf_launch((instance_norm_kernel<8, 1024>), grid, dim3(1024), 0, st, x, res, out, HW, eps, relu);
  else if (vec && n4 <= 20480) scf_launch((instance_norm_kernel<20, 1024>), grid, dim3(1024), 0, st, x, res, out, HW, eps, relu);
  else scf_launch(instance_norm_generic_kernel, grid, blk, 0, st, x, res, out, HW, eps, relu);
  return scf_launch_status();
}

__global__ __launch_bounds__(256) void group_norm_relu_kernel(const float* __restrict__ x, int parts,
                                                              long long part_stride,
                                                              const float* __restrict__ gamma,
                                                              const float* __restrict__ beta,
                                                              float* __restrict__ out, int C, int HW,
                                                              int G, float eps) {
  __shared__ float red[4];
  const int n = blockIdx.x / G, g = blockIdx.x % G;
  const int cpg = C / G;
  const int cnt = cpg * HW;
  const long long base = ((long long)n * C + (long long)g * cpg) * HW;
  const float* xp = x + base;
  auto at = [&](int i) {
    float v = xp[i];
    for (int sl = 1; sl < parts; ++sl) v += xp[(long long)sl * part_stride + i];
    return v;
  };
  constexpr int KEEP = 8;
  const bool keep = cnt <= KEEP * 256;
  float kv[KEEP];
  if (keep) {
    float u[4][KEEP];
#pragma unroll
    for (int j = 0; j < KEEP; ++j) {
      const int i = threadIdx.x + j * 256;
#pragma unroll
      for (int sl = 0; sl < 4; ++sl) u[sl][j] = (i < cnt && sl < parts) ? xp[(long long)sl * part_stride + i] : 0.f;
    }
#pragma unroll
    for (int j = 0; j < KEEP; ++j) {
      kv[j] = u[0][j];
#pragma unroll
      for (int sl = 1; sl < 4; ++sl)
        if (sl < parts) kv[j] += u[sl][j];
    }
    for (int sl = 4; sl < parts; ++sl) {
#pragma unroll
      for (int j = 0; j < KEEP; ++j) {
        const int i = threadIdx.x + j * 256;
        if (i < cnt) kv[j] += xp[(long long)sl * part_stride + i];
      }
    }
  }
  float s = 0.f;
  if (keep) {
#pragma unroll
    for (int j = 0; j < KEEP; ++j) s += kv[j];
  } else {
    for (int i = threadIdx.x; i < cnt; i += 256) s += at(i);
  }
  const float mean = block_sum_256(s, red) / (float)cnt;
  float q = 0.f;
  if (keep) {
#pragma unroll
    for (int j = 0; j < KEEP; ++j) {
      const float a = kv[j] - mean;
      q += (threadIdx.x + j * 256 < cnt) ? a * a : 0.f;
    }
  } else {
    for (int i = threadIdx.x; i < cnt; i += 256) {
      const float a = at(i) - mean;
      q += a * a;
    }
  }
  const float var = block_sum_256(q, red) / (float)cnt;
  const float rstd = 1.0f / sqrtf(var + eps);
  if (keep) {
#pragma unroll
    for (int j = 0; j < KEEP; ++j) {
      const int i = threadIdx.x + j * 256;
      if (i < cnt) {
        const int c = g * cpg + i / HW;
        out[base + i] = fmaxf((kv[j] - mean) * rstd * gamma[c] + beta[c], 0.f);
      }
    }
  } else {
    for (int i = threadIdx.x; i < cnt; i += 256) {
      const int c = g * cpg + i / HW;
      const float o = (at(i) - mean) * rstd * gamma[c] + beta[c];
      out[base + i] = fmaxf(o, 0.f);
// ... 102 lines not shown
```

### scflow_amd/csrc/resample.hip

```cpp
#include "scf_common.h"

struct ResizeJob {
  const float* a; const float* b; float* out; float mul;
};
template <bool VEC>
__global__ __launch_bounds__(256) void resize_bilinear_kernel(ResizeJob j0, ResizeJob j1, int planes0,
                                                              int planes, int Hin, int Win,
                                                              int Hout, int Wout, float sh, float sw,
                                                              float* __restrict__ out2, int out2_group, long long out2_gs) {
#pragma clang fp contract(off)
  const int ox0 = (blockIdx.x * 64 + (threadIdx.x & 63)) * 4;
  const int oy = blockIdx.y * 4 + (threadIdx.x >> 6);
  if (ox0 >= Wout || oy >= Hout) return;
  const float fy = sh * (float)oy;
  const int y0 = (int)fy;
  const int y1 = y0 + (y0 < Hin - 1 ? 1 : 0);
  const float ly = fy - (float)y0, hy = 1.f - ly;
  int x0[4], x1[4];
  float lx[4];
#pragma unroll
  for (int i = 0; i < 4; ++i) {
    const float fx = sw * (float)(ox0 + i);
    x0[i] = (int)fx;
    if (x0[i] > Win - 1) x0[i] = Win - 1;
    x1[i] = x0[i] + (x0[i] < Win - 1 ? 1 : 0);
    lx[i] = fx - (float)x0[i];
  }
  for (int plg = blockIdx.z; plg < planes; plg += gridDim.z) {
    const bool second = plg >= planes0;
    const int pl = second ? plg - planes0 : plg;
    const float* a = second ? j1.a : j0.a;
    const float* b = second ? j1.b : j0.b;
    float* out = second ? j1.out : j0.out;
    const float mul = second ? j1.mul : j0.mul;
    const long long base = (long long)pl * Hin * Win;
    const float* r0 = a + base + (long long)y0 * Win;
    const float* r1 = a + base + (long long)y1 * Win;
    const float* s0 = b ? b + base + (long long)y0 * Win : nullptr;
    const float* s1 = b ? b + base + (long long)y1 * Win : nullptr;
    float v[4];
#pragma unroll
    for (int i = 0; i < 4; ++i) {
      float v00 = r0[x0[i]], v01 = r0[x1[i]], v10 = r1[x0[i]], v11 = r1[x1[i]];
      if (b) {
        v00 += s0[x0[i]];
        v01 += s0[x1[i]];
        v10 += s1[x0[i]];
        v11 += s1[x1[i]];
      }
      const float hx = 1.f - lx[i];
      v[i] = mul * (hy * (hx * v00 + lx[i] * v01) + ly * (hx * v10 + lx[i] * v11));
    }
    float* o = out + ((long long)pl * Hout + oy) * Wout + ox0;
    float* o2 = (out2 && !second) ? out2 + (long long)(pl / out2_group) * out2_gs +
                                        ((long long)(pl % out2_group) * Hout + oy) * Wout + ox0
                                  : nullptr;
    if (VEC) {
      scf_store4<(SCF_ST_SC1 & 1) != 0>(o, v[0], v[1], v[2], v[3]);
      if (o2) scf_store4<(SCF_ST_SC1 & 1) != 0>(o2, v[0], v[1], v[2], v[3]);
    } else {
#pragma unroll
      for (int i = 0; i < 4; ++i)
        if (ox0 + i < Wout) {
          o[i] = v[i];
          if (o2) o2[i] = v[i];
        }
    }
  }
}

int scf_resize_bilinear_jobs(const float* a, const float* b, float* out, int64_t planes, float mul,
                             const float* a1, const float* b1, float* out1, int64_t planes1, float mul1,
                             float* out2, int out2_group, int64_t out2_gstride,
                             int Hin, int Win, int Hout, int Wout, scf_stream_t stream) {
  if (!a || !out || planes <= 0 || Hin <= 0 || Win <= 0 || Hout <= 0 || Wout <= 0) return SCF_EINVAL;
  if (planes1 < 0 || (planes1 > 0 && (!a1 || !out1)) || (out2 && out2_group <= 0)) return SCF_EINVAL;
  const long long total = (long long)planes + planes1;
  if (total > 0x7fffffffLL) return SCF_EINVAL;
  const float sh = Hout > 1 ? (float)(Hin - 1) / (float)(Hout - 1) : 0.f;
  const float sw = Wout > 1 ? (float)(Win - 1) / (float)(Wout - 1) : 0.f;
  const long long gxy = scf_cdiv(Wout, 256) * scf_cdiv(Hout, 4);
  long long gz = (4LL * scf_cu_count() + gxy - 1) / gxy;
  gz = gz < 1 ? 1 : gz > total ? total : gz > 65535 ? 65535 : gz;
  const dim3 grid((unsigned)scf_cdiv(Wout, 256), (unsigned)scf_cdiv(Hout, 4), (unsigned)gz);
  if (grid.y > 65535u) return SCF_EUNSUPPORTED;
  const ResizeJob j0 = {a, b, out, mul}, j1 = {a1, b1, out1, mul1};
  const bool vec = (Wout & 3) == 0 && ((uintptr_t)out & 15) == 0 && (planes1 == 0 || ((uintptr_t)out1 & 15) == 0) &&
                   (!out2 || (((uintptr_t)out2 & 15) == 0 && (out2_gstride & 3) == 0));
  if (vec)
    scf_launch(resize_bilinear_kernel<true>, grid, dim3(256), 0, scf_stream(stream), j0, j1, (int)planes, (int)total,
               Hin, Win, Hout, Wout, sh, sw, out2, out2_group, (long long)out2_gstride);
  else
    scf_launch(resize_bilinear_kernel<false>, grid, dim3(256), 0, scf_stream(stream), j0, j1, (int)planes, (int)total,
               Hin, Win, Hout, Wout, sh, sw, out2, out2_group, (long long)out2_gstride);
  return scf_launch_status();
}

extern "C" int scf_resize_bilinear(const float* a, const float* b, float* out, int64_t planes,
                                   int Hin, int Win, int Hout, int Wout, float mul,
                                   scf_stream_t stream) {
  return scf_resize_bilinear_jobs(a, b, out, planes, mul, nullptr, nullptr, nullptr, 0, 1.0f, nullptr, 1, 0,
                                  Hin, Win, Hout, Wout, stream);
}

__global__ __launch_bounds__(256) void avgpool2x2_kernel(const float* __restrict__ x,
                                                         float* __restrict__ out, long long planes,
                                                         int Hin, int Win, int Ho, int Wo) {
  const long long total = planes * Ho * Wo;
  for (long long idx = (long long)blockIdx.x * blockDim.x + threadIdx.x; idx < total;
       idx += (long long)gridDim.x * blockDim.x) {
    const int ox = (int)(idx % Wo);
    const long long t = idx / Wo;
    const int oy = (int)(t % Ho);
    const long long pl = t / Ho;
    const float* s = x + pl * Hin * Win + (long long)(2 * oy) * Win + 2 * ox;
    out[idx] = (((s[0] + s[1]) + s[Win]) + s[Win + 1]) * 0.25f;
  }
}

extern "C" int scf_avgpool2x2(const float* x, float* out, int64_t planes, int Hin, int Win,
                              scf_stream_t stream) {
  if (!x || !out || planes <= 0 || Hin < 2 || Win < 2) return SCF_EINVAL;
  const int Ho = Hin / 2, Wo = Win / 2;
  const long long total = (long long)planes * Ho * Wo;
  const int grid = (int)(scf_cdiv(total, 256) < 262144 ? scf_cdiv(total, 256) : 262144);
  scf_launch(avgpool2x2_kernel, dim3(grid), dim3(256), 0, scf_stream(stream), x, out,
                     (long long)planes, Hin, Win, Ho, Wo);
  return scf_launch_status();
}

__device__ __forceinline__ int pyr_offset(int y, int x, int pw4, int lw) {
  return pw4 ? (y >> 2) * pw4 + (x >> 3) * 32 + (y & 3) * 8 + (x & 7) : y * lw + x;
}
__global__ __launch_bounds__(256) void avgpool2x2_layout_kernel(const float* __restrict__ x,
                                                                float* __restrict__ out,
                                                                long long planes, int Win, int in_pw4,
                                                                int in_msz, int Ho, int Wo, int out_pw4,
                                                                int out_msz) {
  const long long total = planes * Ho * Wo;
  for (long long idx = (long long)blockIdx.x * blockDim.x + threadIdx.x; idx < total;
       idx += (long long)gridDim.x * blockDim.x) {
    const int ox = (int)(idx % Wo);
    const long long t = idx / Wo;
    const int oy = (int)(t % Ho);
    const long long pl = t / Ho;
    const float* s = x + pl * in_msz;
    const int y = 2 * oy, xx = 2 * ox;
    const float a = s[pyr_offset(y, xx, in_pw4, Win)], b = s[pyr_offset(y, xx + 1, in_pw4, Win)];
    const float c = s[pyr_offset(y + 1, xx, in_pw4, Win)], d = s[pyr_offset(y + 1, xx + 1, in_pw4, Win)];
    out[pl * out_msz + pyr_offset(oy, ox, out_pw4, Wo)] = (((a + b) + c) + d) * 0.25f;
  }
}

int scf_avgpool2x2_layout(const float* x, float* out, int64_t planes, int Hin, int Win, int in_tiled,
                          int out_tiled, hipStream_t st) {
  if (!x || !out || planes <= 0 || Hin < 2 || Win < 2) return SCF_EINVAL;
  const int Ho = Hin / 2, Wo = Win / 2;
  const int in_pw = (Win + 7) / 8 * 8, in_ph = (Hin + 3) / 4 * 4;
  const int out_pw = (Wo + 7) / 8 * 8, out_ph = (Ho + 3) / 4 * 4;
  const long long total = (long long)planes * Ho * Wo;
  const int grid = (int)(scf_cdiv(total, 256) < 262144 ? scf_cdiv(total, 256) : 262144);
  scf_launch(avgpool2x2_layout_kernel, dim3(grid), dim3(256), 0, st, x, out, (long long)planes, Win,
             in_tiled ? in_pw * 4 : 0, in_tiled ? in_ph * in_pw : Hin * Win, Ho, Wo,
             out_tiled ? out_pw * 4 : 0, out_tiled ? out_ph * out_pw : Ho * Wo);
  return scf_launch_status();
}

__global__ __launch_bounds__(256) void mul_mask_kernel(const float* __restrict__ x, long long xns,
                                                       const float* __restrict__ mask,
                                                       float* __restrict__ out, long long ons, int N,
                                                       int C, int HW) {
  const long long per = (long long)C * HW, total = (long long)N * per;
  for (long long idx = (long long)blockIdx.x * blockDim.x + threadIdx.x; idx < total;
       idx += (long long)gridDim.x * blockDim.x) {
    const long long n = idx / per, r = idx - n * per;
    const int px = (int)(r % HW);
    out[n * ons + r] = x[n * xns + r] * mask[n * HW + px];
  }
}

extern "C" int scf_mul_mask(const float* x, int64_t x_nstride, const float* mask, float* out,
                            int64_t out_nstride, int N, int C, int HW, scf_stream_t stream) {
  if (!x || !mask || !out || N <= 0 || C <= 0 || HW <= 0) return SCF_EINVAL;
  const long long total = (long long)N * C * HW;
  const int grid = (int)(scf_cdiv(total, 256) < 262144 ? scf_cdiv(total, 256) : 262144);
  scf_launch(mul_mask_kernel, dim3(grid), dim3(256), 0, scf_stream(stream), x, (long long)x_nstride, mask,
             out, (long long)out_nstride, N, C, HW);
  return scf_launch_status();
}

template <bool VEC>
__global__ __launch_bounds__(256) void copy_strided_kernel(const float* __restrict__ src,
                                                           long long sns, float* __restrict__ dst,
                                                           long long dns, int N, long long count) {
  if (VEC) {
    const long long c4 = count >> 2, total = (long long)N * c4;
    for (long long idx = (long long)blockIdx.x * blockDim.x + threadIdx.x; idx < total;
         idx += (long long)gridDim.x * blockDim.x) {
      const long long n = idx / c4, r = idx - n * c4;
      reinterpret_cast<float4*>(dst + n * dns)[r] = reinterpret_cast<const float4*>(src + n * sns)[r];
    }
  } else {
    const long long total = (long long)N * count;
    for (long long idx = (long long)blockIdx.x * blockDim.x + threadIdx.x; idx < total;
         idx += (long long)gridDim.x * blockDim.x) {
      const long long n = idx / count, r = idx - n * count;
      dst[n * dns + r] = src[n * sns + r];
    }
  }
}

extern "C" int scf_copy_strided(const float* src, int64_t src_nstride, float* dst,
                                int64_t dst_nstride, int N, int64_t count, scf_stream_t stream) {
  if (!src || !dst || N <= 0 || count <= 0) return SCF_EINVAL;
  const bool vec = ((count | src_nstride | dst_nstride) & 3) == 0 && ((((uintptr_t)src) | ((uintptr_t)dst)) & 15) == 0;
  const long long units = (long long)N * (vec ? count >> 2 : count);
  const long long cap = 8LL * scf_cu_count();
  const int grid = (int)(scf_cdiv(units, 256) < cap ? scf_cdiv(units, 256) : cap);
  if (vec)
    scf_launch(copy_strided_kernel<true>, dim3(grid), dim3(256), 0, scf_stream(stream), src, (long long)src_nstride, dst,
               (long long)dst_nstride, N, (long long)count);
  else
    scf_launch(copy_strided_kernel<false>, dim3(grid), dim3(256), 0, scf_stream(stream), src, (long long)src_nstride, dst,
               (long long)dst_nstride, N, (long long)count);
  return scf_launch_status();
}

template <int S>
__global__ __launch_bounds__(256) void convex_upsample_kernel(const float* __restrict__ x,
                                                              const float* __restrict__ mask,
                                                              float* __restrict__ out, int C, int h,
                                                              int w, float x_mul, float mask_mul) {
  constexpr int SS = S * S;
  extern __shared__ float tile[];
  const int xt = blockIdx.x, y = blockIdx.y, n = blockIdx.z;
  const int xl = threadIdx.x & 31, sub0 = threadIdx.x >> 5;
  const int px = xt * 32 + xl;
  const long long hw = (long long)h * w;
  const bool ok = px < w;
  float wall[SS / 8][9];
#pragma unroll
  for (int it = 0; it < SS / 8; ++it) {
    const int sub = sub0 + it * 8;
#pragma unroll
    for (int k = 0; k < 9; ++k)
      wall[it][k] = ok ? mask[((long long)n * 9 * SS + k * SS + sub) * hw + (long long)y * w + px] : 0.f;
  }
#pragma unroll
  for (int it = 0; it < SS / 8; ++it) {
    const int sub = sub0 + it * 8;
// ... 49 lines not shown
```

### scflow_amd/modules.py

```python
from __future__ import annotations

from typing import Dict, List, Optional, Sequence, Tuple, Union

import torch
import torch.nn as nn

from . import ops
from .ops import (ACT_NONE, ACT_RELU, ACT_SIGMOID, ACT_TANH, CONV_GRU_Q, CONV_GRU_ZR, PackedConv)
from .registry import DECODERS, ENCODERS, HEAD, build_head

Tensor = torch.Tensor

_ACTS = {None: ACT_NONE, 'ReLU': ACT_RELU, 'Sigmoid': ACT_SIGMOID, 'Tanh': ACT_TANH}


def _act_code(act_cfg: Optional[dict]) -> int:
    if act_cfg is None:
        return ACT_NONE
    kind = act_cfg.get('type')
    if kind not in _ACTS:
        raise NotImplementedError(f'activation {kind} has no HIP epilogue')
    return _ACTS[kind]


# ... 53 lines not shown

    @property
    def packed(self):
        d = self.__dict__
        key = self._pack_key()
        if d.get('_packed') is None or d.get('_packed_key') != key:
            with torch.no_grad():
                d['_packed'] = self._pack()
            d['_packed_key'] = key
        return d['_packed']


class ConvBlock(HipModule):

    def __init__(self, cin, cout, kernel_size, stride=1, padding=0, act_cfg=dict(type='ReLU'),
                 norm_cfg: Optional[dict] = None):
        super().__init__()
        self.conv = nn.Conv2d(cin, cout, kernel_size, stride=stride, padding=padding,
                              bias=norm_cfg is None)
        self.act = _act_code(act_cfg)
        self.groups = None
        if norm_cfg is not None:
            if norm_cfg.get('type') != 'GN':
                raise NotImplementedError('ConvBlock supports GN only (pose head)')
            self.groups = norm_cfg['num_groups']
            self.gn = nn.GroupNorm(self.groups, cout, eps=norm_cfg.get('eps', 1e-5))

    def _pack(self) -> PackedConv:
        c = self.conv
        return PackedConv.from_weight(c.weight, c.bias, stride=c.stride[0], padding=c.padding)

    def forward(self, x0: Tensor, x1: Optional[Tensor] = None, out: Optional[Tensor] = None) -> Tensor:
        if self.groups is None:
            return ops.conv2d(self.packed, x0, x1, out=out, act=self.act)
        if self.act != ACT_RELU:
            raise NotImplementedError('GN is fused with ReLU only')
        ks = ops.conv_kslices_for(self.packed, x0, x1)
        y = ops.conv2d(self.packed, x0, x1, kslices=ks)
        return ops.group_norm_relu(y, self.gn.weight, self.gn.bias, self.groups, self.gn.eps, out=out)


class _BasicBlock(HipModule):

    def __init__(self, inplanes, planes, stride, kind, downsample: bool):
        super().__init__()
        tag = 'in' if kind == 'IN' else 'bn'
        mk = (lambda c: nn.InstanceNorm2d(c)) if kind == 'IN' else (lambda c: nn.BatchNorm2d(c))
        self.kind, self.stride, self.tag = kind, stride, tag
        self.conv1 = nn.Conv2d(inplanes, planes, 3, stride=stride, padding=1, bias=True)
        setattr(self, tag + '1', mk(planes))
        self.conv2 = nn.Conv2d(planes, planes, 3, padding=1, bias=True)
        setattr(self, tag + '2', mk(planes))
        self.downsample = None
        if downsample:
            self.downsample = nn.Sequential(nn.Conv2d(inplanes, planes, 1, stride=stride, bias=True),
                                            mk(planes))

    def _bn(self, m):
        return (m.weight, m.bias, m.running_mean, m.running_var) if self.kind == 'BN' else None

    def _pack(self):
        n1, n2 = getattr(self, self.tag + '1'), getattr(self, self.tag + '2')
        eps = n1.eps
        p = dict(c1=PackedConv.from_weight(self.conv1.weight, self.conv1.bias, self.stride, 1,
                                           bn=self._bn(n1), eps=eps),
                 c2=PackedConv.from_weight(self.conv2.weight, self.conv2.bias, 1, 1,
                                           bn=self._bn(n2), eps=eps))
        if self.downsample is not None:
            ds = self.downsample[0]
            p['ds'] = PackedConv.from_weight(ds.weight, ds.bias, self.stride, 0,
                                             bn=self._bn(self.downsample[1]), eps=eps)
        return p

    def forward(self, x: Tensor) -> Tensor:
        p = self.packed
        if self.kind == 'BN':
            y = ops.conv2d(p['c1'], x, act=ACT_RELU)
            idt = ops.conv2d(p['ds'], x) if 'ds' in p else x
            return ops.conv2d(p['c2'], y, res=idt, act=ACT_RELU)
        y = ops.conv2d(p['c1'], x)
        ops.instance_norm(y, relu=True, out=y)
        y2 = ops.conv2d(p['c2'], y)
        if 'ds' in p:
            idt = ops.conv2d(p['ds'], x)
            ops.instance_norm(idt, out=idt)
        else:
            idt = x
        return ops.instance_norm(y2, res=idt, relu=True, out=y2)


@ENCODERS.register_module()
class RAFTEncoder(HipModule):

    def __init__(self, in_channels: int, out_channels: int, scale: float = 1 / 8,
                 net_type: str = 'Basic', norm_cfg: dict = dict(type='BN', requires_grad=True),
                 init_cfg=None, **unsupported) -> None:
        super().__init__()
        if net_type != 'Basic':
            raise NotImplementedError("only net_type='Basic' is built (SCFlow config)")
        bad = {k: v for k, v in unsupported.items()
               if v not in (None, False, -1) and k not in ('conv_cfg',)}
        if bad:
            raise NotImplementedError(f'RAFTEncoder options not built: {sorted(bad)}')
        kind = norm_cfg['type']
        if kind not in ('IN', 'BN', 'SyncBN'):
            raise NotImplementedError(f'norm {kind}')
        kind = 'IN' if kind == 'IN' else 'BN'
        self.kind, self.tag = kind, ('in' if kind == 'IN' else 'bn')
        self.in_channels, self.out_channels, self.scale = in_channels, out_channels, scale
        mk = (lambda c: nn.InstanceNorm2d(c)) if kind == 'IN' else (lambda c: nn.BatchNorm2d(c))
        self.stem_stride = 1 if scale == 1 / 4 else 2
        self.conv1 = nn.Conv2d(in_channels, 64, 7, stride=self.stem_stride, padding=3, bias=True)
        setattr(self, self.tag + '1', mk(64))
        inplanes = 64
        self.res_layers = []
        for i, (planes, stride) in enumerate(zip((64, 96, 128), (1, 2, 2)), start=1):
            layer = nn.Sequential(
                _BasicBlock(inplanes, planes, stride, kind, stride != 1 or inplanes != planes),
                _BasicBlock(planes, planes, 1, kind, False))
            self.add_module(f'res_layer{i}', layer)
            self.res_layers.append(f'res_layer{i}')
            inplanes = planes
        self.conv2 = nn.Conv2d(128, out_channels, 1)

    def _pack(self):
        n1 = getattr(self, self.tag + '1')
        bn = (n1.weight, n1.bias, n1.running_mean, n1.running_var) if self.kind == 'BN' else None
        return dict(stem=PackedConv.from_weight(self.conv1.weight, self.conv1.bias,
                                                self.stem_stride, 3, bn=bn, eps=n1.eps),
                    head=PackedConv.from_weight(self.conv2.weight, self.conv2.bias, 1, 0))

    def forward(self, x: Tensor, out: Optional[Tensor] = None, head_act: int = ACT_NONE,
                head_act2: int = ACT_NONE, head_split: int = 0) -> Tensor:
        p = self.packed
        if self.kind == 'BN':
            x = ops.conv2d(p['stem'], x, act=ACT_RELU)
        else:
            x = ops.conv2d(p['stem'], x)
            ops.instance_norm(x, relu=True, out=x)
        for name in self.res_layers:
            for blk in getattr(self, name):
                x = blk(x)
        return ops.conv2d(p['head'], x, out=out, act=head_act, act2=head_act2,
                          act_split=head_split)


def encoder_pair_supported(fe: 'RAFTEncoder', ce: 'RAFTEncoder') -> bool:
    return (fe.kind == 'IN' and ce.kind == 'BN' and fe.stem_stride == ce.stem_stride and fe.in_channels == ce.in_channels
            and fe.res_layers == ce.res_layers)


def raft_encoder_pair(fe: 'RAFTEncoder', xf: Tensor, ce: 'RAFTEncoder', xc: Tensor, out_c: Optional[Tensor] = None,
                      head_act: int = ACT_NONE, head_act2: int = ACT_NONE, head_split: int = 0) -> Tuple[Tensor, Tensor]:
    if not encoder_pair_supported(fe, ce):
        raise ValueError('raft_encoder_pair: (InstanceNorm feature encoder, BatchNorm context encoder) of one layer geometry')
    pf, pc = fe.packed, ce.packed
    yf, yc = ops.conv2d_pair((pf['stem'], xf), (pc['stem'], xc, dict(act=ACT_RELU)))
    ops.instance_norm(yf, relu=True, out=yf)
    for name in fe.res_layers:
        for bf, bc in zip(getattr(fe, name), getattr(ce, name)):
            qf, qc = bf.packed, bc.packed
            tf_, tc_ = ops.conv2d_pair((qf['c1'], yf), (qc['c1'], yc, dict(act=ACT_RELU)))
            ops.instance_norm(tf_, relu=True, out=tf_)
            if 'ds' in qf:
                if_, ic_ = ops.conv2d_pair((qf['ds'], yf), (qc['ds'], yc))
                ops.instance_norm(if_, out=if_)
            else:
                if_, ic_ = yf, yc
            uf_, yc = ops.conv2d_pair((qf['c2'], tf_), (qc['c2'], tc_, dict(res=ic_, act=ACT_RELU)))
            yf = ops.instance_norm(uf_, res=if_, relu=True, out=uf_)
    return ops.conv2d_pair((pf['head'], yf), (pc['head'], yc, dict(out=out_c, act=head_act, act2=head_act2,
                                                                  act_split=head_split)))


class CorrelationPyramid(HipModule):

    def __init__(self, num_levels: int = 4) -> None:
        super().__init__()
        self.num_levels = num_levels

    def forward(self, feat1: Tensor, feat2: Tensor, tiled_levels: int = 0) -> List[Tensor]:
        return ops.corr_build(feat1, feat2, self.num_levels, tiled_levels=tiled_levels)


class CorrLookup(HipModule):

    def __init__(self, radius: int = 4, mode: str = 'bilinear', padding_mode: str = 'zeros',
                 align_corners: bool = True) -> None:
        super().__init__()
        if mode != 'bilinear' or padding_mode != 'zeros' or not align_corners:
            raise NotImplementedError('HIP CorrLookup: bilinear / zeros / align_corners=True')
        self.r = radius

    def forward(self, corr_pyramid: Sequence[Tensor], flow: Tensor,
                tiled_levels: int = 0) -> Tensor:
        return ops.corr_lookup(corr_pyramid, flow, self.r, tiled_levels=tiled_levels)


def _pyramid_layout(feat: Tensor, radius: int, num_levels: int, allow: bool = True) -> int:
    return ops.pyramid_layout(feat.shape[-2], feat.shape[-1], radius, num_levels) if allow else 0


class MotionEncoder(HipModule):

    def __init__(self, num_levels: int = 4, radius: int = 4, net_type: str = 'Basic',
                 conv_cfg=None, norm_cfg=None, act_cfg=dict(type='ReLU')) -> None:
        super().__init__()
        if net_type not in ('Basic', 'Large') or norm_cfg is not None:
            raise NotImplementedError('MotionEncoder: Basic, no norm')
        cin = num_levels * (2 * radius + 1) ** 2
        self.corr_net = nn.Sequential(ConvBlock(cin, 256, 1, padding=0, act_cfg=act_cfg),
                                      ConvBlock(256, 192, 3, padding=1, act_cfg=act_cfg))
        self.flow_net = nn.Sequential(ConvBlock(2, 128, 7, padding=3, act_cfg=act_cfg),
                                      ConvBlock(128, 64, 3, padding=1, act_cfg=act_cfg))
        self.out_net = nn.Sequential(ConvBlock(256, 126, 3, padding=1, act_cfg=act_cfg))
        self.out_channels = [126]

    def forward(self, corr: Tensor, flow: Tensor, out: Optional[Tensor] = None,
                overlap: bool = False, cf: Optional[Tensor] = None, fork=None) -> Tensor:
        n, _, h, w = flow.shape
        dev = flow.device
        if out is None:
            out = torch.empty((n, 128, h, w), dtype=torch.float32, device=dev)
        if cf is None:
            if overlap:
                raise ValueError('overlap=True needs a cf buffer allocated before the fork point')
            cf = torch.empty((n, 256, h, w), dtype=torch.float32, device=dev)
        if not overlap and 'flow' in ops.PAIR_BRANCHES and ops._CONV_EVENTS is None:
            cn, fn = self.corr_net, self.flow_net
            c1, f1 = ops.conv2d_pair((cn[0].packed, corr, dict(act=cn[0].act)), (fn[0].packed, flow, dict(act=fn[0].act)))
            ops.conv2d_pair((cn[1].packed, c1, dict(out=cf[:, :192], act=cn[1].act)),
                            (fn[1].packed, f1, dict(out=cf[:, 192:], act=fn[1].act)))
            del c1, f1
        else:
            br = ops.side_stream(overlap, after=fork)
            with br:
                f1 = self.flow_net[0](flow)
                self.flow_net[1](f1, out=cf[:, 192:])
                del f1
            c1 = self.corr_net[0](corr)
            self.corr_net[1](c1, out=cf[:, :192])
            br.join()
        self.out_net[0](cf, out=out[:, :126])
        ops.copy_channels(flow, out[:, 126:128])
        return out


class ConvGRU(HipModule):
    _kernel = {'Conv': [3], 'SeqConv': [(1, 5), (5, 1)]}
    _padding = {'Conv': [1], 'SeqConv': [(0, 2), (2, 0)]}

    def __init__(self, h_channels: int, x_channels: int, net_type: str = 'SeqConv') -> None:
        super().__init__()
# ... 513 lines not shown
```

### scflow_amd/ops.py

```python
from __future__ import annotations

import ctypes as C
import os
import math
from dataclasses import dataclass
from typing import List, Optional, Sequence, Tuple

import torch

from . import _lib
from ._lib import (ACT_NONE, ACT_RELU, ACT_SIGMOID, ACT_TANH, CONV_GRU_Q, CONV_GRU_ZR,
                   CONV_PLAIN, ConvDesc)

Tensor = torch.Tensor

__all__ = ['record_conv_kernels', 'PackedConv', 'conv_desc', 'gru_passes', 'scflow_iteration', 'side_stream_handle', 'pyramid_layout', 'untile_level', 'level_storage_shape', 'sepconv_gru', 'pack_conv_weight', 'pack_conv_weight_f16x3', 'set_conv_precision', 'set_conv_winograd', 'get_conv_winograd', 'pack_conv_weight_wino', 'pack_conv_weight_wino1d', 'pack_conv_weight_wino1d4',
           'get_conv_precision', 'set_conv_kslices', 'conv_kslices', 'conv_kslices_for', 'constant', 'clear_constants', 'register_conv_workspace', 'choose_kc', 'conv2d', 'conv2d_pair', 'corr_build', 'corr_lookup',
           'instance_norm', 'group_norm_relu', 'linear', 'fc_splitk', 'fc_slices', 'pose_update', 'reproject_flow',
           'flow_corr_2d3d', 'pnp_params', 'pnp_ransac', 'pnp',
           'unproject_depth', 'linear_pair', 'resize_bilinear', 'convex_upsample', 'avgpool2x2', 'copy_channels',
           'ACT_NONE', 'ACT_RELU', 'ACT_SIGMOID', 'ACT_TANH', 'CONV_PLAIN', 'CONV_GRU_ZR',
           'CONV_GRU_Q']


_cur_dev = torch._C._cuda_getDevice
_raw_stream = torch._C._cuda_getCurrentRawStream


_KWS = {}
_KWS_FLOATS = 1 << 20


def register_conv_workspace(enable: bool = True) -> None:
    dev = _cur_dev()
    handle = _raw_stream(dev)
    if enable:
        ws = torch.empty((_KWS_FLOATS,), dtype=torch.float32, device=f'cuda:{dev}')
        _lib.check(_lib.load().scf_conv_workspace(handle, ws.data_ptr(), _KWS_FLOATS), 'scf_conv_workspace')
        _KWS[(dev, handle)] = ws
    elif _KWS.pop((dev, handle), None) is not None:
        _lib.check(_lib.load().scf_conv_workspace(handle, None, 0), 'scf_conv_workspace')


def _stream() -> int:
    return _raw_stream(_cur_dev())


def _dev(t: Tensor, name: str) -> None:
    if not isinstance(t, torch.Tensor) or not t.is_cuda:
        raise _lib.ScflowHipError(f'{name}: expected a tensor on the GPU (HIP path only, no CPU '
                                  'fallback)')
    if t.dtype != torch.float32:
        raise _lib.ScflowHipError(f'{name}: expected float32, got {t.dtype}')
    if t.device.index != _cur_dev():
        raise _lib.ScflowHipError(
            f'{name} lives on cuda:{t.device.index} but the current device is '
            f'cuda:{_cur_dev()}: wrap the call in torch.cuda.device(tensor.device)')


def _dense(t: Tensor, name: str) -> int:
    _dev(t, name)
    if not t.is_contiguous():
        raise _lib.ScflowHipError(f'{name}: expected a contiguous tensor')
    return t.data_ptr()


def _nchw(t: Tensor, name: str) -> Tuple[int, int, int, int, int, int]:
    _dev(t, name)
    if t.dim() != 4:
        raise _lib.ScflowHipError(f'{name}: expected 4-D NCHW')
    n, c, h, w = t.shape
    sn, sc, sh, sw = t.stride()
    ok = (sw == 1 or w == 1) and (sh == w or h == 1) and (sc == h * w or c == 1)
    if not ok:
        raise _lib.ScflowHipError(f'{name}: not a sample-strided NCHW view (strides {t.stride()})')
    if n == 1:
        sn = c * h * w
    return t.data_ptr(), n, c, h, w, sn


def _opt(t: Optional[Tensor], name: str) -> Optional[int]:
    return None if t is None else _dense(t, name)


_SIDE = {}


OVERLAP_BRANCHES = set()
OVERLAP_MAX_PIXELS = {'context': 4 * 256 * 256, 'flow': 4 * 256 * 256, 'mask': 4 * 256 * 256, 'upsample': 4 * 256 * 256}


PAIR_BRANCHES = {'context', 'flow', 'mask'}
PAIR_MAX_PIXELS = {'context': 4 * 256 * 256, 'flow': None, 'mask': None}


def branch_mode(n: int, h: int, w: int, branch: str) -> int:
    if branch in PAIR_BRANCHES:
        lim = PAIR_MAX_PIXELS.get(branch, 4 * 256 * 256)
        return 2 if lim is None or n * h * w <= lim else 0
    lim = OVERLAP_MAX_PIXELS.get(branch, 4 * 256 * 256)
    return 1 if n * h * w <= lim and branch in OVERLAP_BRANCHES else 0
# ... 212 lines not shown
    g4: int = 0
    wthin: Optional[Tensor] = None
    wp4s: Optional[Tensor] = None
    g4s: int = 0
    wtaps: Optional[Tensor] = None
    desc: Optional[ConvDesc] = None
    wp4t: Optional[Tensor] = None
    g4t: int = 0
    wwino: Optional[Tensor] = None
    wwino1d: Optional[Tensor] = None
    wwino1d4: Optional[Tensor] = None

    @staticmethod
    def from_weight(weight: Tensor, bias: Optional[Tensor], stride: int = 1,
                    padding=0, bn: Optional[Sequence[Tensor]] = None,
                    eps: float = 1e-5, dma_packing: bool = True) -> 'PackedConv':
        cout, cin, kh, kw = weight.shape
        kc = choose_kc(cin, kh, kw, stride)
        wp, mld = pack_conv_weight(weight, kc)
        wp_alt = pack_conv_weight(weight, 32)[0] if (kc == 8 and cin >= 32) else None
        wp16 = pack_conv_weight_f16x3(weight) if (cin >= 16 and kh * kw > 1) else None
        ph, pw = (padding, padding) if isinstance(padding, int) else padding
        scale = shift = None
        if bn is not None:
            gamma, beta, mean, var = [b.float() for b in bn]
            scale = (gamma / torch.sqrt(var + eps)).contiguous()
            shift = (beta - mean * scale).contiguous()
        g4 = choose_a4_groups(cin, kh, kw, stride) if dma_packing else 0
        wp4 = pack_conv_weight_a4(weight, g4)[0] if g4 else None
        g4s = choose_a4s_groups(cin, kh, kw, stride) if dma_packing else 0
        wp4s = pack_conv_weight_a4(weight, g4s)[0] if g4s else None
        return PackedConv(wp, None if bias is None else bias.float().contiguous(), scale, shift,
                          cin, cout, kh, kw, stride, ph, pw, kc, mld, wp_alt, {}, wp16, wp4, g4,
                          pack_conv_weight_thin(weight) if (cout <= 4 and stride == 1 and cin >= 32) else None,
                          wp4s, g4s, pack_conv_weight_taps(weight) if (cin <= 4 and dma_packing) else None,
                          None, *PackedConv._tiny(weight, kh, kw, stride, dma_packing),
                          pack_conv_weight_wino(weight) if (dma_packing and (kh, kw, stride, ph, pw) == (3, 3, 1, 1, 1)
                                                            and cin >= 8) else None,
                          pack_conv_weight_wino1d(weight) if (dma_packing and stride == 1 and cin >= 16 and cout % 64 == 0
                                                              and (kh, kw, ph, pw) in ((1, 5, 0, 2), (5, 1, 2, 0))) else None,
                          pack_conv_weight_wino1d4(weight) if (dma_packing and stride == 1 and cin >= 16 and cout % 64 == 0
                                                               and (kh, kw, ph, pw) in ((1, 5, 0, 2), (5, 1, 2, 0))) else None)

    @staticmethod
    def _tiny(weight, kh, kw, stride, dma_packing):
        g = choose_a4t_groups(weight.shape[1], kh, kw, stride) if dma_packing else 0
        return (pack_conv_weight_a4(weight, g)[0] if g else None), g

    def out_hw(self, h: int, w: int) -> Tuple[int, int]:
        return ((h + 2 * self.pad_h - self.kh) // self.stride + 1,
                (w + 2 * self.pad_w - self.kw) // self.stride + 1)


def _desc_template(pc: 'PackedConv') -> ConvDesc:
    d = ConvDesc()
    d.wp, d.w_nstride, d.Mld, d.Cout = pc.wp.data_ptr(), 0, pc.mld, pc.cout
    d.KH, d.KW, d.stride, d.pad_h, d.pad_w, d.KC = pc.kh, pc.kw, pc.stride, pc.pad_h, pc.pad_w, pc.kc
    d.bias = None if pc.bias is None else pc.bias.data_ptr()
    d.scale = None if pc.scale is None else pc.scale.data_ptr()
    d.shift = None if pc.shift is None else pc.shift.data_ptr()
    d.out_div = 1.0
    if pc.wthin is not None:
        d.wp_thin = pc.wthin.data_ptr()
    if pc.wtaps is not None:
        d.wp_taps = pc.wtaps.data_ptr()
    if pc.wp4 is not None:
        d.wp_a4, d.a4_groups, d.a4_mld = pc.wp4.data_ptr(), pc.g4, pc.mld
    if pc.wp4s is not None:
        d.wp_a4s, d.a4s_groups, d.a4_mld = pc.wp4s.data_ptr(), pc.g4s, pc.mld
    if pc.wp4t is not None:
        d.wp_a4t, d.a4t_groups, d.a4_mld = pc.wp4t.data_ptr(), pc.g4t, pc.mld
    return d


def conv_desc(pc: PackedConv, x0: Tensor, x1: Optional[Tensor] = None, out: Optional[Tensor] = None,
              **kw) -> Tuple[ConvDesc, Tensor]:
    return conv2d(pc, x0, x1, out, _launch=False, **kw)


def conv2d(pc: PackedConv, x0: Tensor, x1: Optional[Tensor] = None, out: Optional[Tensor] = None,
           *, res: Optional[Tensor] = None, act: int = ACT_NONE, act2: int = ACT_NONE,
           act_split: int = 0, mode: int = CONV_PLAIN, gru_h: Optional[Tensor] = None,
           gru_aux: Optional[Tensor] = None, gru_z: Optional[Tensor] = None, kslices: int = 1,
           _launch: bool = True):
    p0, n, c0, h, w, s0 = _nchw(x0, 'x0')
    p1, c1, s1 = None, 0, 0
    if x1 is not None:
        p1, n1, c1, h1, w1, s1 = _nchw(x1, 'x1')
        if (n1, h1, w1) != (n, h, w):
            raise _lib.ScflowHipError('x0/x1 shape mismatch')
    if c0 + c1 != pc.cin:
        raise _lib.ScflowHipError(f'conv expects {pc.cin} input channels, got {c0}+{c1}')
    ho, wo = pc.out_hw(h, w)
    sliced = None
    if kslices > 1:
        if pc.bias is not None or pc.scale is not None or res is not None or act != ACT_NONE or mode != CONV_PLAIN:
            raise _lib.ScflowHipError('conv2d(kslices > 1): partial sums take a plain epilogue (no bias / BN / res / act)')
        sliced = out if out is not None else torch.empty((kslices, n, pc.cout, ho, wo), dtype=torch.float32, device=x0.device)
        if tuple(sliced.shape) != (kslices, n, pc.cout, ho, wo) or not sliced.is_contiguous():
            raise _lib.ScflowHipError(f'conv2d(kslices={kslices}): out must be a contiguous {(kslices, n, pc.cout, ho, wo)} tensor')
        out = sliced[0]
    if out is None:
        out = torch.empty((n, pc.cout // 2 if mode == CONV_GRU_ZR else pc.cout, ho, wo),
                          dtype=torch.float32, device=x0.device)
    po, no, co, oh, ow, so = _nchw(out, 'out')
    want_c = pc.cout // 2 if mode == CONV_GRU_ZR else pc.cout
    if (no, co, oh, ow) != (n, want_c, ho, wo):
        raise _lib.ScflowHipError(f'out has shape {tuple(out.shape)}, expected '
                                  f'{(n, want_c, ho, wo)}')
    tmpl = pc.desc
    if tmpl is None:
        tmpl = pc.desc = _desc_template(pc)
    d = ConvDesc.from_buffer_copy(tmpl)
    d.in0, d.in1, d.C0, d.C1 = p0, p1, c0, c1
    d.in0_nstride, d.in1_nstride = s0, s1
    d.N, d.H, d.W = n, h, w
    d.out, d.out_nstride = po, so
    if sliced is not None:
        d.k_slices, d.out_slice_stride = kslices, sliced.stride(0)
        out = sliced
    if res is not None:
        pr, nr, cr, hr, wr, sr = _nchw(res, 'res')
        if (nr, cr, hr, wr) != (n, pc.cout, ho, wo):
            raise _lib.ScflowHipError('res shape mismatch')
        d.res, d.res_nstride = pr, sr
    d.act, d.act2, d.act_split, d.mode = act, act2, act_split, mode
    if gru_h is not None:
        ph_, _, _, _, _, sh_ = _nchw(gru_h, 'gru_h')
        d.gru_h, d.gru_h_nstride = ph_, sh_
    if gru_aux is not None:
        pa_, _, _, _, _, sa_ = _nchw(gru_aux, 'gru_aux')
        d.gru_aux, d.gru_aux_nstride = pa_, sa_
    if gru_z is not None:
        pz_, _, _, _, _, sz_ = _nchw(gru_z, 'gru_z')
        d.gru_z, d.gru_z_nstride = pz_, sz_
    if _CONV_PRECISION == 'f16x3' and pc.wp16 is not None:
        d.wp_f16 = pc.wp16.data_ptr()
    elif _CONV_WINOGRAD and pc.wwino is not None and mode == CONV_PLAIN:
        d.wp_wino = pc.wwino.data_ptr()
    elif _CONV_WINOGRAD and pc.wwino1d is not None:
        d.wp_wino1d = pc.wwino1d.data_ptr()
        d.wp_wino1d4 = pc.wwino1d4.data_ptr() if pc.wwino1d4 is not None else None
    if x1 is not None:
        d.wp_taps = None
    if pc.wp_alt is not None and (c1 == 0 or c0 % 32 == 0):
        key = (n, h, w, c0, c1, d.wp_f16 is not None)
        use_alt = pc.plans.get(key)
        if use_alt is None:
            lib = _lib.load()
            info = (C.c_int32 * 4)()
            use_alt = False
            ww, ww1, ww4, d.wp_wino, d.wp_wino1d, d.wp_wino1d4 = d.wp_wino, d.wp_wino1d, d.wp_wino1d4, None, None, None
            if (lib.scf_conv2d_query(C.byref(d), info) == 0 and info[0] * info[1] == 1
                    and 0 <= info[3] * 64 < 6000):
                d.wp, d.KC = pc.wp_alt.data_ptr(), 32
                use_alt = lib.scf_conv2d_query(C.byref(d), info) == 0
                d.wp, d.KC = pc.wp.data_ptr(), pc.kc
            d.wp_wino, d.wp_wino1d, d.wp_wino1d4 = ww, ww1, ww4
            pc.plans[key] = use_alt
        if use_alt:
            d.wp, d.KC = pc.wp_alt.data_ptr(), 32
    if not _launch:
        return d, out
    if _CONV_EVENTS is not None:
        lib = _lib.load()
        tm = C.c_void_p()
        _lib.check(lib.scf_timer_create(C.byref(tm)), 'scf_timer_create')
        lib.scf_timer_arm(tm)
        try:
            _lib.check(lib.scf_conv2d(C.byref(d), _stream()), 'scf_conv2d')
        finally:
            lib.scf_timer_arm(None)
        tag = ''
        if d.wp_wino or d.wp_wino1d:
            info = (C.c_int32 * 4)()
            if lib.scf_conv2d_query(C.byref(d), info) == 0 and info[3] < 0 and info[0] in (16, 6, 8):
                tag = {16: ' [winograd]', 6: ' [winograd F(2,5)]', 8: ' [winograd F(4,5)]'}[info[0]]
        _CONV_EVENTS.append((tm, 2.0 * pc.cin * pc.kh * pc.kw * pc.cout * ho * wo * n,
                             f'{pc.cin}->{pc.cout} {pc.kh}x{pc.kw}/s{pc.stride} @{ho}x{wo} N{n}' + tag))
        return out
    rc = _lib.load().scf_conv2d(C.byref(d), _stream())
    if rc == -2 and x1 is not None and sliced is None:
        return conv2d(pc, torch.cat([x0, x1], 1), None, out, res=res, act=act, act2=act2, act_split=act_split, mode=mode,
                      gru_h=gru_h, gru_aux=gru_aux, gru_z=gru_z)
    _lib.check(rc, 'scf_conv2d')
    return out


def _pair_operand(layer):
    pc, x0 = layer[0], layer[1]
    kw = dict(layer[2]) if len(layer) > 2 else {}
    d, out = conv2d(pc, x0, _launch=False, **kw)
    if kw.get('x1') is not None and kw.get('kslices', 1) <= 1:
        info = (C.c_int32 * 4)()
        if _lib.load().scf_conv2d_query(C.byref(d), info) == -2:
            x0, kw['x1'], kw['out'] = torch.cat([x0, kw['x1']], 1), None, out
            d, out = conv2d(pc, x0, _launch=False, **kw)
            return d, out, x0
    return d, out, None
# ... 90 lines not shown
            g.wp_zr_a4s, g.wp_q_a4s, g.a4s_groups = pzr.wp4s.data_ptr(), pq.wp4s.data_ptr(), pzr.g4s
        if pzr.wp4t is not None and pq.wp4t is not None and pzr.g4t == pq.g4t:
            g.wp_zr_a4t, g.wp_q_a4t, g.a4t_groups = pzr.wp4t.data_ptr(), pq.wp4t.data_ptr(), pzr.g4t
        if _CONV_WINOGRAD and not f16 and pzr.wwino1d is not None and pq.wwino1d is not None:
            g.wp_zr_wino1d, g.wp_q_wino1d = pzr.wwino1d.data_ptr(), pq.wwino1d.data_ptr()
            if pzr.wwino1d4 is not None and pq.wwino1d4 is not None:
                g.wp_zr_wino1d4, g.wp_q_wino1d4 = pzr.wwino1d4.data_ptr(), pq.wwino1d4.data_ptr()
    return arr


gru_passes = _gru_passes


def side_stream_handle() -> int:
    main = torch.cuda.current_stream()
    key = (torch.cuda.current_device(), main.cuda_stream)
    side = _SIDE.get(key)
    if side is None:
        side = _SIDE[key] = torch.cuda.Stream(device=key[0])
    return side.cuda_stream


def scflow_iteration(it: '_lib.ScflowIter') -> None:
    lib = _lib.load()
    it.lookup_timer = _LOOKUP_TIMERS.take() if _LOOKUP_TIMERS is not None else None
    _lib.check(lib.scf_scflow_iteration(C.byref(it), _stream()), 'scf_scflow_iteration')


def sepconv_gru(packs, hx: Tensor, h_channels: int, z: Tensor, rh: Tensor,
                ctx: Optional[Sequence[Tensor]] = None, ctx_channels: int = 0) -> None:
    hc = h_channels
    if ctx is not None and (ctx_channels <= 0 or len(ctx) != len(packs)):
        raise _lib.ScflowHipError('sepconv_gru: one context term per pass, ctx_channels > 0')
    if _CONV_EVENTS is not None:
        hv, xv = hx[:, :hc], hx[:, hc + ctx_channels:]
        for i, (pzr, pq) in enumerate(packs):
            if ctx is None:
                conv2d(pzr, hx, out=z, mode=CONV_GRU_ZR, gru_h=hv, gru_aux=rh)
                conv2d(pq, rh, xv, out=hv, mode=CONV_GRU_Q, gru_h=hv, gru_z=z)
            else:
                conv2d(pzr, hv, xv, out=z, mode=CONV_GRU_ZR, gru_h=hv, gru_aux=rh, res=ctx[i][:, :2 * hc])
                conv2d(pq, rh, xv, out=hv, mode=CONV_GRU_Q, gru_h=hv, gru_z=z, res=ctx[i][:, 2 * hc:])
        return
    p, n, c, h, w, sn = _nchw(hx, 'hx')
    arr = _gru_passes(packs)
    if ctx is None:
        _lib.check(_lib.load().scf_sepconv_gru(p, sn, n, hc, c - hc, h, w, arr, len(packs),
                                               _dense(z, 'z'), _dense(rh, 'rh'), _stream()),
                   'scf_sepconv_gru')
        return
    ptrs, cs = (C.c_void_p * len(ctx))(), None
    for i, t in enumerate(ctx):
        pc_, nc, cc_, hh, ww, s_ = _nchw(t, 'ctx')
        if (nc, cc_, hh, ww) != (n, 3 * hc, h, w) or (cs is not None and s_ != cs):
            raise _lib.ScflowHipError('sepconv_gru: ctx must be (N, 3*h_channels, H, W), equal strides')
        ptrs[i], cs = pc_, s_
    _lib.check(_lib.load().scf_sepconv_gru_ctx(p, sn, n, hc, ctx_channels, c - hc - ctx_channels, h, w,
                                               arr, len(packs), ptrs, cs, _dense(z, 'z'),
                                               _dense(rh, 'rh'), _stream()),
               'scf_sepconv_gru_ctx')


def _read_timers(timers):
    lib = _lib.load()
    out = []
    for tm in timers:
        us = C.c_float()
        _lib.check(lib.scf_timer_elapsed_us(tm, C.byref(us)), 'scf_timer_elapsed_us')
        lib.scf_timer_destroy(tm)
        out.append(float(us.value))
    return out


def conv_timing(enable: bool):
    global _CONV_EVENTS
    if enable:
        _CONV_EVENTS = []
        return None
    evs, _CONV_EVENTS = _CONV_EVENTS or [], None
    torch.cuda.synchronize()
    return list(zip(_read_timers([e[0] for e in evs]), [e[1] for e in evs], [e[2] for e in evs]))


TUNE_KEYS = {'wino_variant': 1, 'dma_force_ksplit': 2, 'dma_ksplit_groups': 3, 'wino1d4': 4, 'lookup_pipe': 5, 'lookup_store': 6, 'conv_autoslice': 7, 'iter_merge': 8, 'wino1d4_half': 9, 'conv_pair': 10}


def tune(key: str, value: int) -> int:
    if key not in TUNE_KEYS:
        raise ValueError(f'unknown tune key {key!r}; known: {sorted(TUNE_KEYS)}')
    prev = int(_lib.load().scf_tune(TUNE_KEYS[key], int(value)))
    if prev < 0:
        _lib.check(prev, f'scf_tune({key}, {value})')
    return prev


class record_conv_kernels:

    _active = False

    def __init__(self, capacity: int = 1 << 16) -> None:
        self.capacity, self.ran, self.paired, self.variants = capacity, [], [], []

    def __enter__(self):
        if record_conv_kernels._active:
            raise RuntimeError('record_conv_kernels does not nest (one process-wide dispatch log)')
        _lib.check(_lib.load().scf_conv_log_enable(self.capacity), 'scf_conv_log_enable')
        record_conv_kernels._active = True
        return self.ran

    def __exit__(self, *exc):
        record_conv_kernels._active = False
        lib = _lib.load()
        n = lib.scf_conv_log_read(None, 0)
        buf = (_lib.ConvLogEntry * max(n, 1))()
        n = min(lib.scf_conv_log_read(buf, n), n)
        lib.scf_conv_log_enable(0)
        for e in buf[:n]:
            self.ran.append((f'{e.Cin}->{e.Cout} {e.KH}x{e.KW}/s{e.stride} @{e.Ho}x{e.Wo} N{e.N}',
                             _lib.KERNEL_NAMES.get(e.kernel, str(e.kernel))))
            self.paired.append(e.paired)
            self.variants.append(e.variant)
        return False


def time_first_kernel(fn) -> float:
    lib = _lib.load()
    tm = C.c_void_p()
    _lib.check(lib.scf_timer_create(C.byref(tm)), 'scf_timer_create')
    lib.scf_timer_arm(tm)
    try:
        fn()
    finally:
        lib.scf_timer_arm(None)
    torch.cuda.synchronize()
    return _read_timers([tm])[0]


def pyramid_layout(h: int, w: int, radius: int = 4, num_levels: int = 4) -> int:
    return int(_lib.load().scf_corr_preferred_layout(h, w, radius, num_levels))


def level_storage_shape(h: int, w: int, level: int, tiled: bool) -> Tuple[int, int]:
    lh, lw = h >> level, w >> level
    return ((lh + 3) // 4 * 4, (lw + 7) // 8 * 8) if tiled else (lh, lw)


def untile_level(level: Tensor, lh: int, lw: int) -> Tensor:
    q, _, ph, pw = level.shape
    return (level.reshape(q, ph // 4, pw // 8, 4, 8).permute(0, 1, 3, 2, 4).reshape(q, 1, ph, pw)
            [:, :, :lh, :lw].contiguous())


def untile_level0(level0: Tensor) -> Tensor:
    return untile_level(level0, level0.shape[-2], level0.shape[-1])


def _pyramid_shapes(n: int, h: int, w: int, num_levels: int, tiled_levels: int):
    return [(n * h * w, 1, *level_storage_shape(h, w, l, bool((tiled_levels >> l) & 1)))
            for l in range(num_levels)]


def corr_build(feat1: Tensor, feat2: Tensor, num_levels: int = 4,
               out: Optional[List[Tensor]] = None, tiled_levels: int = 0) -> List[Tensor]:
    p1 = _dense(feat1, 'feat1')
    p2 = _dense(feat2, 'feat2')
    if feat1.shape != feat2.shape or feat1.dim() != 4:
        raise _lib.ScflowHipError('feat1/feat2 must be equal-shape NCHW')
# ... 75 lines not shown
        return out

    def reset(self) -> None:
        self.used = 0

    def destroy(self) -> None:
        lib = _lib.load()
        for tm in self.timers:
            lib.scf_timer_destroy(tm)
        self.timers, self.used = [], 0


_LOOKUP_TIMERS: Optional[_TimerPool] = None
_CORR_TIMERS: Optional[_TimerPool] = None


def corr_build_timing(enable: bool, reserve: int = 16):
    global _CORR_TIMERS
    if enable:
        if _CORR_TIMERS is not None:
            _CORR_TIMERS.destroy()
        _CORR_TIMERS = _TimerPool(reserve)
        return None
    pool, _CORR_TIMERS = _CORR_TIMERS, None
    if pool is None:
        return []
    torch.cuda.synchronize()
    out = pool.read()
    pool.destroy()
    return out


def corr_build_timing_reset() -> None:
    if _CORR_TIMERS is not None:
        torch.cuda.synchronize()
        _CORR_TIMERS.reset()


def corr_build_timing_read():
    if _CORR_TIMERS is None:
        return []
    torch.cuda.synchronize()
    return _CORR_TIMERS.read()


def lookup_timing(enable: bool, reserve: int = 64):
    global _LOOKUP_TIMERS
    if enable:
        if _LOOKUP_TIMERS is not None:
            _LOOKUP_TIMERS.destroy()
        _LOOKUP_TIMERS = _TimerPool(reserve)
        return None
    pool, _LOOKUP_TIMERS = _LOOKUP_TIMERS, None
    if pool is None:
        return []
    torch.cuda.synchronize()
    out = pool.read()
    pool.destroy()
    return out


def lookup_timing_reset() -> None:
    if _LOOKUP_TIMERS is not None:
        torch.cuda.synchronize()
        _LOOKUP_TIMERS.reset()


def lookup_timing_read():
    if _LOOKUP_TIMERS is None:
        return []
    torch.cuda.synchronize()
    return _LOOKUP_TIMERS.read()


def instance_norm(x: Tensor, res: Optional[Tensor] = None, relu: bool = False,
                  out: Optional[Tensor] = None, eps: float = 1e-5) -> Tensor:
    px = _dense(x, 'x')
    n, c, h, w = x.shape
    if out is None:
        out = torch.empty_like(x)
    _lib.check(_lib.load().scf_instance_norm(px, _opt(res, 'res'), _dense(out, 'out'), n * c,
                                             h * w, eps, int(relu), _stream()),
               'scf_instance_norm')
    return out


def group_norm_relu(x: Tensor, gamma: Tensor, beta: Tensor, groups: int, eps: float = 1e-5,
                    out: Optional[Tensor] = None) -> Tensor:
    px = _dense(x, 'x')
    parts, pstride = 1, 0
    if x.dim() == 5:
        parts, pstride = x.shape[0], x.stride(0)
        x = x[0]
    n, c, h, w = x.shape
    if out is None:
        out = torch.empty_like(x)
    _lib.check(_lib.load().scf_group_norm_relu_parts(px, parts, pstride, _dense(gamma, 'gamma'), _dense(beta, 'beta'),
                                                     _dense(out, 'out'), n, c, h * w, groups, eps,
                                                     _stream()), 'scf_group_norm_relu')
    return out


def linear(x: Tensor, weight: Tensor, bias: Optional[Tensor], act: int = ACT_NONE,
           out: Optional[Tensor] = None) -> Tensor:
    px = _dense(x, 'x')
    n, k = x.shape
    o = weight.shape[0]
    if weight.shape[1] != k:
        raise _lib.ScflowHipError('linear: weight/in_features mismatch')
    if out is None:
        out = torch.empty((n, o), dtype=torch.float32, device=x.device)
    _lib.check(_lib.load().scf_linear(px, _dense(weight, 'weight'), _opt(bias, 'bias'),
                                      _dense(out, 'out'), n, k, o, act, _stream()), 'scf_linear')
    return out


def fc_slices(k: int) -> int:
    if k % 8 == 0 and k <= 256:
        return 1
    return k // 256 if k % 256 == 0 else 0


def fc_splitk(x: Tensor, weight: Tensor, bias: Optional[Tensor] = None, *, x_bias: Optional[Tensor] = None,
              x_relu: bool = False, gn=None, weight2: Optional[Tensor] = None, bias2: Optional[Tensor] = None,
              act: int = ACT_NONE, slices: int = 1):
    _dev(x, 'x')
    if x.dim() == 2:
        x = x.unsqueeze(0)
    if x.dim() != 3 or not x.is_contiguous():
        raise _lib.ScflowHipError('fc_splitk: x must be a contiguous (N, K) or (parts, N, K) tensor')
    parts, n, k = x.shape
    o = weight.shape[0]
    if weight.shape[1] != k or (weight2 is not None and weight2.shape[1] != k):
        raise _lib.ScflowHipError('fc_splitk: weight / in_features mismatch')
    d = _lib.FcDesc()
    d.x, d.x_parts, d.x_part_stride = x.data_ptr(), parts, n * k
    d.x_bias, d.x_relu = _opt(x_bias, 'x_bias'), int(bool(x_relu))
    if gn is not None:
        groups, hw, gamma, beta, eps = gn
        d.gn_groups, d.gn_hw, d.gn_gamma, d.gn_beta, d.gn_eps = groups, hw, _dense(gamma, 'gamma'), _dense(beta, 'beta'), eps
    d.N, d.K = n, k
    y = torch.empty((slices, n, o) if slices > 1 else (n, o), dtype=torch.float32, device=x.device)
    d.W, d.bias, d.y, d.O = _dense(weight, 'weight'), _opt(bias, 'bias'), y.data_ptr(), o
    y2 = None
    if weight2 is not None:
        y2 = torch.empty((n, weight2.shape[0]), dtype=torch.float32, device=x.device)
        d.W2, d.bias2, d.y2, d.O2 = _dense(weight2, 'weight2'), _opt(bias2, 'bias2'), y2.data_ptr(), weight2.shape[0]
    d.act, d.slices = act, slices
    _lib.check(_lib.load().scf_fc_splitk(C.byref(d), _stream()), 'scf_fc_splitk')
    return y if y2 is None else (y, y2)


def linear_pair(x: Tensor, w1: Tensor, b1: Optional[Tensor], w2: Tensor, b2: Optional[Tensor],
                act: int = ACT_NONE) -> Tuple[Tensor, Tensor]:
    px = _dense(x, 'x')
    n, k = x.shape
    if w1.shape[1] != k or w2.shape[1] != k:
        raise _lib.ScflowHipError('linear_pair: weight/in_features mismatch')
    y1 = torch.empty((n, w1.shape[0]), dtype=torch.float32, device=x.device)
    y2 = torch.empty((n, w2.shape[0]), dtype=torch.float32, device=x.device)
    _lib.check(_lib.load().scf_linear_pair(px, _dense(w1, 'w1'), _opt(b1, 'b1'), y1.data_ptr(),
                                           w1.shape[0], _dense(w2, 'w2'), _opt(b2, 'b2'),
                                           y2.data_ptr(), w2.shape[0], n, k, act, _stream()),
               'scf_linear_pair')
    return y1, y2


def pose_update(rot_all: Tensor, trans_all: Tensor, label: Tensor, num_class: int,
                rot: Tensor, trans: Tensor, label_mode: int = 0):
    n = rot_all.shape[0]
    if not label.is_cuda or label.dtype != torch.int64 or not label.is_contiguous():
        raise _lib.ScflowHipError('label must be a contiguous int64 GPU tensor')
    dev = rot_all.device
    d_rot = torch.empty((n, 6), dtype=torch.float32, device=dev)
    d_trans = torch.empty((n, 3), dtype=torch.float32, device=dev)
    r_out = torch.empty((n, 3, 3), dtype=torch.float32, device=dev)
    t_out = torch.empty((n, 3), dtype=torch.float32, device=dev)
    _lib.check(_lib.load().scf_pose_update(
        _dense(rot_all, 'rot_all'), _dense(trans_all, 'trans_all'), label.data_ptr(), num_class,
        label_mode, _dense(rot, 'rot'), _dense(trans, 'trans'), d_rot.data_ptr(),
        d_trans.data_ptr(), r_out.data_ptr(), t_out.data_ptr(), n, _stream()), 'scf_pose_update')
    return d_rot, d_trans, r_out, t_out


def reproject_flow(depth: Tensor, k: Tensor, rot0: Tensor, trans0: Tensor, rot: Tensor,
                   trans: Tensor, invalid_num: float = 0., out: Optional[Tensor] = None) -> Tensor:
    n, h, w = depth.shape
    if out is None:
        out = torch.empty((n, 2, h, w), dtype=torch.float32, device=depth.device)
    _lib.check(_lib.load().scf_reproject_flow(
        _dense(depth, 'depth'), _dense(k, 'k'), _dense(rot0, 'rot0'), _dense(trans0, 'trans0'),
        _dense(rot, 'rot'), _dense(trans, 'trans'), _dense(out, 'out'), n, h, w,
        float(invalid_num), _stream()), 'scf_reproject_flow')
    return out


def filter_flow_by_mask_(flow: Tensor, mask: Tensor, invalid_num: float = 400.,
                         align_corners: bool = False) -> Tensor:
    n, two, h, w = flow.shape
    if two != 2 or tuple(mask.shape) != (n, h, w):
        raise _lib.ScflowHipError('filter_flow_by_mask: flow (N,2,H,W), mask (N,H,W)')
    _lib.check(_lib.load().scf_filter_flow_by_mask(_dense(flow, 'flow'), _dense(mask, 'mask'), n, h, w,
                                                   float(invalid_num), int(align_corners), _stream()),
               'scf_filter_flow_by_mask')
    return flow


def _mats(t: Tensor, n: int, shape: Tuple[int, ...], name: str) -> int:
    if tuple(t.shape) != (n, *shape):
        raise _lib.ScflowHipError(f'{name}: expected shape {(n, *shape)}, got {tuple(t.shape)}')
    return _dense(t, name)


def flow_corr_2d3d(flow: Tensor, depth: Tensor, k: Tensor, rot0: Tensor, trans0: Tensor,
                   occlusion: Optional[Tensor] = None, occ_thresh: float = 0.5):
    if depth.dim() != 3:
        raise _lib.ScflowHipError('flow_corr_2d3d: depth must be (N,H,W)')
    n, h, w = depth.shape
    if tuple(flow.shape) != (n, 2, h, w):
        raise _lib.ScflowHipError(f'flow_corr_2d3d: flow must be {(n, 2, h, w)}, got {tuple(flow.shape)}')
    if occlusion is not None and tuple(occlusion.shape) != (n, h, w):
        raise _lib.ScflowHipError(f'flow_corr_2d3d: occlusion must be {(n, h, w)}, got {tuple(occlusion.shape)}')
    dev = depth.device
    pts2d = torch.empty((n, h * w, 2), dtype=torch.float32, device=dev)
    pts3d = torch.empty((n, h * w, 3), dtype=torch.float32, device=dev)
    conf = torch.empty((n, h * w), dtype=torch.float32, device=dev)
    count = torch.empty((n,), dtype=torch.int32, device=dev)
    _lib.check(_lib.load().scf_flow_corr_2d3d(
        _dense(flow, 'flow'), _dense(depth, 'depth'), _opt(occlusion, 'occlusion'), float(occ_thresh),
        _mats(k, n, (3, 3), 'k'), _mats(rot0, n, (3, 3), 'rot0'), _mats(trans0, n, (3,), 'trans0'), n, h, w,
        pts2d.data_ptr(), pts3d.data_ptr(), conf.data_ptr(), count.data_ptr(), _stream()), 'scf_flow_corr_2d3d')
    return pts2d, pts3d, conf, count


_PNP_MODES = {None: _lib.PNP_SAMPLE_ALL, 'topk': _lib.PNP_SAMPLE_TOPK, 'random': _lib.PNP_SAMPLE_RANDOM}


def pnp_params(iterations: int = 100, reproj_error: float = 3.0, sample_mode: Optional[str] = None,
               sample_num: int = 1000, seed: int = 0) -> '_lib.PnpParams':
    if isinstance(iterations, bool) or int(iterations) != iterations or iterations <= 0:
        raise _lib.ScflowHipError(f'pnp: iterations must be a positive integer, got {iterations!r}')
    if not math.isfinite(float(reproj_error)) or float(reproj_error) < 0:
        raise _lib.ScflowHipError(f'pnp: reproj_error must be finite and >= 0, got {reproj_error!r}')
    if sample_mode not in _PNP_MODES:
        raise _lib.ScflowHipError(f"pnp: sample_mode must be None, 'topk' or 'random', got {sample_mode!r}")
    if sample_mode is not None and (int(sample_num) != sample_num or sample_num <= 0):
        raise _lib.ScflowHipError(f'pnp: sample_num must be a positive integer, got {sample_num!r}')
    if int(seed) != seed or not 0 <= seed < 2 ** 64:
        raise _lib.ScflowHipError(f'pnp: seed must be an integer in [0, 2^64), got {seed!r}')
    return _lib.PnpParams(int(iterations), float(reproj_error), _PNP_MODES[sample_mode],
                          int(sample_num) if sample_mode is not None else 0, int(seed))


def pnp_ransac(pts2d: Tensor, pts3d: Tensor, count: Tensor, k: Tensor, ref_rot: Tensor, ref_trans: Tensor,
               conf: Optional[Tensor] = None, iterations: int = 100, reproj_error: float = 3.0,
               sample_mode: Optional[str] = None, sample_num: int = 1000, seed: int = 0):
    p = pnp_params(iterations, reproj_error, sample_mode, sample_num, seed)
    if pts2d.dim() != 3 or pts2d.shape[2] != 2:
        raise _lib.ScflowHipError('pnp_ransac: pts2d must be (N,C,2)')
    n, cap = pts2d.shape[0], pts2d.shape[1]
    if tuple(pts3d.shape) != (n, cap, 3):
        raise _lib.ScflowHipError(f'pnp_ransac: pts3d must be {(n, cap, 3)}, got {tuple(pts3d.shape)}')
    if conf is not None and tuple(conf.shape) != (n, cap):
        raise _lib.ScflowHipError(f'pnp_ransac: conf must be {(n, cap)}, got {tuple(conf.shape)}')
    if sample_mode == 'topk' and conf is None:
        raise _lib.ScflowHipError("pnp_ransac: sample_mode='topk' needs conf")
    if (not isinstance(count, torch.Tensor) or not count.is_cuda or count.dtype != torch.int32
            or tuple(count.shape) != (n,) or not count.is_contiguous() or count.device != pts2d.device):
        raise _lib.ScflowHipError(f'pnp_ransac: count must be a contiguous int32 GPU tensor of shape {(n,)}')
    if n == 0 or cap == 0:
        raise _lib.ScflowHipError('pnp_ransac: empty batch')
    lib = _lib.load()
    dev = pts2d.device
    wsb = lib.scf_pnp_workspace_bytes(n, cap, C.byref(p))
    _lib.check(min(int(wsb), 0), 'scf_pnp_workspace_bytes')
    ws = torch.empty((max(int(wsb), 1),), dtype=torch.uint8, device=dev) if wsb > 0 else None
    rot = torch.empty((n, 3, 3), dtype=torch.float32, device=dev)
# ... 252 lines not shown
```

### scflow_amd/refiner.py

```python
from __future__ import annotations

from typing import Dict, Optional, Tuple, Union

import torch

from . import ops
from .modules import HipModule, encoder_pair_supported, raft_encoder_pair
from .ops import ACT_RELU, ACT_TANH, small_work
from .registry import REFINERS, build_decoder, build_encoder

Tensor = torch.Tensor


def _as_mask_tensor(mask, device) -> Tensor:
    if isinstance(mask, torch.Tensor):
        return mask.to(device=device, dtype=torch.bool)
    return mask.to_tensor(dtype=torch.bool, device=device)


class _RenderingRefiner:

    renderer = None

    def attach_renderer(self, renderer):
# ... 14 lines not shown
        labels = torch.cat(annots['labels'])
        internel_k = torch.cat(annots['k'])
        output = dict(real_images=real_images, labels=labels, internel_k=internel_k,
                      ref_rotations=ref_rotations, ref_translations=ref_translations,
                      per_img_patch_num=per_img_patch_num, meta_infos=meta_infos)
        if 'transform_matrix' in annots:
            output['transform_matrix'] = torch.cat(annots['transform_matrix'])
        if 'ori_k' in annots:
            output['ori_k'] = torch.cat([k[None].expand(n, 3, 3) for k, n in zip(annots['ori_k'], per_img_patch_num)])
        norm = meta_infos[0]['img_norm_cfg']
        mean = (torch.tensor(norm['mean'], dtype=torch.float32) / 255.).tolist()
        std = (torch.tensor(norm['std'], dtype=torch.float32) / 255.).tolist()
        rgb, depth, mask = self.renderer.render_normalized(ref_rotations, ref_translations, internel_k, labels, mean, std)
        output.update(rendered_images=rgb, rendered_depths=depth, rendered_masks=mask)
        if 'depths' in annots:
            output['real_depths'] = torch.cat(annots['depths'], dim=0)
        if 'gt_rotations' in annots:
            output['gt_rotations'] = torch.cat(annots['gt_rotations'], dim=0)
            output['gt_translations'] = torch.cat(annots['gt_translations'], dim=0)
        if 'gt_masks' in annots:
            output['gt_masks'] = torch.cat([_as_mask_tensor(m, real_images.device) for m in annots['gt_masks']], dim=0)
        return output

    def update_data(self, update_rotations: Tensor, update_translations: Tensor, data: Dict) -> Dict:
        self._need_renderer('update_data')
        data['ref_rotations'] = update_rotations
        data['ref_translations'] = update_translations
        rgb, depth, mask = self.renderer.render_normalized(update_rotations, update_translations, data['internel_k'],
                                                           data['labels'])
        data['rendered_images'] = rgb
        data['rendered_depths'] = depth
        data['rendered_masks'] = mask
        return data


@REFINERS.register_module()
class SCFlowRefiner(_RenderingRefiner, HipModule):
    def __init__(self, seperate_encoder: bool, cxt_channels: int, h_channels: int,
                 cxt_encoder: dict, encoder: dict, decoder: dict, renderer: Optional[dict] = None,
                 pose_loss_cfg: Optional[dict] = None, flow_loss_cfg: Optional[dict] = None,
                 mask_loss_cfg: Optional[dict] = None, max_flow: float = 400,
                 render_augmentations: Optional[list] = None, filter_invalid_flow: bool = True,
                 freeze_encoder: bool = False, freeze_bn: bool = False,
                 train_cfg: Optional[dict] = None, test_cfg: Optional[dict] = None,
                 init_cfg: Optional[Union[list, dict]] = None) -> None:
        super().__init__()
        self.seperate_encoder = seperate_encoder
        if seperate_encoder:
            self.render_encoder = build_encoder(encoder)
            self.real_encoder = build_encoder(encoder)
        else:
            enc = build_encoder(encoder)
            self.render_encoder = enc
            self.real_encoder = enc
        self.decoder = build_decoder(decoder)
        self.context = build_encoder(cxt_encoder)
        self.renderer = None
        self.max_flow = max_flow
        self.train_cfg = train_cfg or {}
        self.test_cfg = test_cfg or {}
        self.h_channels, self.cxt_channels = h_channels, cxt_channels
        assert self.h_channels == self.decoder.h_channels
        assert self.cxt_channels == self.decoder.cxt_channels
        assert self.h_channels + self.cxt_channels == self.context.out_channels
        self.filter_invalid_flow = filter_invalid_flow
        self.test_by_flow = self.test_cfg.get('by_flow', False)
        self.test_iter_num = self.test_cfg.get('iters', self.decoder.iters)
        self.eval()

    def extract_feat(self, render_images: Tensor, real_images: Tensor
                     ) -> Tuple[Tensor, Tensor, Tensor, Tensor]:
        n, _, H, W = render_images.shape
        dev = render_images.device
        ops._dev(render_images, 'render_images')
        ops._dev(real_images, 'real_images')
        hc, cc = self.h_channels, self.cxt_channels
        sc = int(round(1 / self.context.scale))
        hx = torch.empty((n, hc + cc + 128, H // sc, W // sc), dtype=torch.float32, device=dev)
        rend = render_images.contiguous()
        ov_ctx = small_work(n, H, W, 'context')
        fork = ops.fork_point() if ov_ctx else None
        if (not self.seperate_encoder and ops.branch_mode(n, H, W, 'context') == 2 and ops._CONV_EVENTS is None
                and encoder_pair_supported(self.render_encoder, self.context)):
            both = torch.empty((2 * n, 3, H, W), dtype=torch.float32, device=dev)
            ops.copy_channels(rend, both[:n])
            ops.copy_channels(real_images.contiguous(), both[n:])
            feats, _ = raft_encoder_pair(self.render_encoder, both, self.context, rend, out_c=hx[:, :hc + cc],
                                         head_act=ACT_TANH, head_act2=ACT_RELU, head_split=hc)
            return feats[:n], feats[n:], hx[:, :hc], hx[:, hc:hc + cc]
        if self.seperate_encoder:
            render_feat = self.render_encoder(rend)
            real_feat = self.real_encoder(real_images.contiguous())
        else:
            both = torch.empty((2 * n, 3, H, W), dtype=torch.float32, device=dev)
            ops.copy_channels(rend, both[:n])
            ops.copy_channels(real_images.contiguous(), both[n:])
            feats = self.render_encoder(both)
            render_feat, real_feat = feats[:n], feats[n:]
        br = ops.side_stream(ov_ctx, after=fork)
        with br:
            self.context(rend, out=hx[:, :hc + cc], head_act=ACT_TANH,
                         head_act2=ACT_RELU, head_split=hc)
        br.join()
        return render_feat, real_feat, hx[:, :hc], hx[:, hc:hc + cc]

    def get_pose(self, render_images: Tensor, real_images: Tensor, ref_rotation: Tensor,
                 ref_translation: Tensor, depth: Tensor, internel_k: Tensor, label: Tensor,
                 init_flow: Optional[Tensor] = None):
        feat_render, feat_real, h_feat, cxt_feat = self.extract_feat(render_images, real_images)
        if init_flow is None:
            n, _, H, W = real_images.shape
            init_flow = ops.constant((n, 2, H, W), 0.0, feat_render.device)
        return self.decoder(feat_render, feat_real, h_feat, cxt_feat, ref_rotation,
                            ref_translation, depth.contiguous(), internel_k.contiguous(),
                            label=label, init_flow=init_flow, invalid_flow_num=0.,
                            _consume_state=True)

    def forward_single_pass(self, data: Dict, data_batch: Optional[Dict] = None,
                            return_loss: bool = False) -> Dict:
        labels = data['labels']
        per_img = data['per_img_patch_num']
        nc = self.decoder.pose_pred.num_class
        if labels.numel() and not (labels.is_cuda and torch.cuda.is_current_stream_capturing()):
            lo, hi = torch.stack(torch.aminmax(labels)).tolist()
            if lo < 0 or hi >= nc:
                raise IndexError(f'label out of range [0, {nc}): min {lo}, max {hi}')
        iters = self.decoder.iters
        self.decoder.iters = self.test_iter_num
        try:
            outs = self.get_pose(data['rendered_images'], data['real_images'],
                                 data['ref_rotations'], data['ref_translations'],
                                 data['rendered_depths'], data['internel_k'], labels)
        finally:
            self.decoder.iters = iters
        rot, trans = outs[2][-1], outs[3][-1]
        return dict(rotations=torch.split(rot, per_img), translations=torch.split(trans, per_img),
                    labels=torch.split(labels, per_img),
                    scores=torch.split(torch.ones_like(labels, dtype=torch.float32), per_img))

    def forward(self, data, data_batch=None, return_loss=False):
        if return_loss:
            raise NotImplementedError('training is outside the hot path (SURVEY.md section 2)')
        if self.test_cfg.get('cycles', 1) > 1:
            if self.renderer is None:
                raise NotImplementedError("test_cfg['cycles'] > 1 needs the renderer between cycles (base_refiner.py:250-258); "
                                          'attach one with attach_renderer(MeshRenderer(...)), or render outside and call '
                                          'forward_single_pass / get_pose once per cycle')
            return self.forward_multiple_pass(data, data_batch)
        return self.forward_single_pass(data, data_batch)

    def forward_multiple_pass(self, data: Dict, data_batch: Optional[Dict] = None) -> Dict:
        data = dict(data)
        cycles = self.test_cfg.get('cycles', 1)
        for i in range(cycles):
            results = self.forward_single_pass(data, data_batch)
            if i == cycles - 1:
                break
            data = self.update_data(torch.cat(results['rotations']), torch.cat(results['translations']), data)
        return results


class _FlowRefinerBase(_RenderingRefiner, HipModule):

    def __init__(self, seperate_encoder: bool, cxt_channels: int, h_channels: int,
                 cxt_encoder: dict, encoder: dict, decoder: dict, test_cfg: Optional[dict] = None,
                 **ignored) -> None:
        super().__init__()
        self.seperate_encoder = seperate_encoder
        if seperate_encoder:
            self.render_encoder = build_encoder(encoder)
            self.real_encoder = build_encoder(encoder)
        else:
            enc = build_encoder(encoder)
            self.render_encoder = enc
            self.real_encoder = enc
        self.decoder = build_decoder(decoder)
        self.context = build_encoder(cxt_encoder)
        self.h_channels, self.cxt_channels = h_channels, cxt_channels
        self.test_cfg = test_cfg or {}
        self.test_iter_num = self.test_cfg.get('iters', self.decoder.iters)
# ... 102 lines not shown
```

Baseline: 2318.

## Fuse encoder input concat, paired instance norm, merged pool levels, narrow resize gather

The encoder stem conv now reads the render and real images through a split input pointer (in0_hi/n_split), so the two images no longer have to be copied into one concatenated buffer. The downsample-branch instance norm and the residual instance norm are fused into one paired kernel. The correlation pyramid builds two avgpool levels per launch, and bilinear upsampling gets a narrow-gather path that loads three neighbours once and reuses them. Together these remove copy kernels, launches and redundant global loads, at the cost of more kernel variants and a forced taps-kernel dispatch for split-input convs.

```diff
diff --git a/include/scflow_hip.h b/include/scflow_hip.h
--- a/include/scflow_hip.h
+++ b/include/scflow_hip.h
@@ -83,6 +83,7 @@
   const float* wp_wino1d4;
   int32_t k_slices;
   int64_t out_slice_stride;
+  const float* in0_hi; int32_t n_split;
 } scf_conv_desc;
 
 int scf_conv2d(const scf_conv_desc* desc, scf_stream_t stream);
@@ -168,6 +169,8 @@
 
 int scf_instance_norm(const float* x, const float* res, float* out, int64_t planes,
                       int HW, float eps, int relu, scf_stream_t stream);
+int scf_instance_norm_pair(const float* y, float* s, float* out, int64_t planes, int HW, float eps, int relu,
+                           scf_stream_t stream);
 
 int scf_group_norm_relu(const float* x, const float* gamma, const float* beta, float* out,
                         int N, int C, int HW, int G, float eps, scf_stream_t stream);
@@ -204,7 +207,6 @@
 int scf_reproject_flow(const float* depth, const float* K, const float* R0, const float* t0,
                        const float* R, const float* t, float* flow, int N, int H, int W,
                        float invalid_num, scf_stream_t stream);
-
 int scf_pose_error(const double* verts, int nv, const double* gt_r, const double* gt_t,
                    const double* pred_r, const double* pred_t, const double* K,
                    const int* sample_idx, int nsel, int symmetric, double* err3d, double* err2d,
@@ -291,6 +293,10 @@
 
 int scf_resize_bilinear(const float* a, const float* b, float* out, int64_t planes, int Hin,
                         int Win, int Hout, int Wout, float mul, scf_stream_t stream);
+int scf_resize_bilinear2(const float* a, const float* b, float* out, int64_t planes, float mul,
+                         const float* a1, const float* b1, float* out1, int64_t planes1, float mul1,
+                         float* out2, int out2_group, int64_t out2_gstride,
+                         int Hin, int Win, int Hout, int Wout, scf_stream_t stream);
 
 int scf_convex_upsample(const float* x, const float* mask, float* out, int N, int C, int h,
                         int w, int scale, float x_mul, float mask_mul, scf_stream_t stream);
diff --git a/include/scflow_hip_prof.h b/include/scflow_hip_prof.h
--- a/include/scflow_hip_prof.h
+++ b/include/scflow_hip_prof.h
@@ -45,6 +45,8 @@
   SCF_TUNE_ITER_MERGE = 8,
   SCF_TUNE_WINO1D4_HALF = 9,
   SCF_TUNE_CONV_PAIR = 10,
+  SCF_TUNE_POOL_MERGE = 11,
+  SCF_TUNE_RESIZE_GATHER = 12,
   SCF_TUNE_LOOKUP_PIPE = 5
 };
 int scf_tune(int key, int value);
diff --git a/scflow_amd/_lib.py b/scflow_amd/_lib.py
--- a/scflow_amd/_lib.py
+++ b/scflow_amd/_lib.py
@@ -50,6 +50,7 @@
         ('wp_wino1d4', _fp),
         ('k_slices', C.c_int32),
         ('out_slice_stride', C.c_int64),
+        ('in0_hi', _fp), ('n_split', C.c_int32),
     ]
 
 
@@ -195,6 +196,7 @@
                                       C.c_int64, _fp, _fp, _fp]),
     'scf_scflow_iteration': (C.c_int, [C.POINTER(ScflowIter), _fp]),
     'scf_instance_norm': (C.c_int, [_fp, _fp, _fp, C.c_int64, C.c_int, C.c_float, C.c_int, _fp]),
+    'scf_instance_norm_pair': (C.c_int, [_fp, _fp, _fp, C.c_int64, C.c_int, C.c_float, C.c_int, _fp]),
     'scf_group_norm_relu': (C.c_int, [_fp, _fp, _fp, _fp, C.c_int, C.c_int, C.c_int, C.c_int,
                                       C.c_float, _fp]),
     'scf_conv_workspace': (C.c_int, [_fp, _fp, C.c_int64]),
@@ -225,6 +227,8 @@
     'scf_unproject_depth': (C.c_int, [_fp, _fp, _fp, _fp, _fp, C.c_int, C.c_int, C.c_int, _fp]),
     'scf_resize_bilinear': (C.c_int, [_fp, _fp, _fp, C.c_int64, C.c_int, C.c_int, C.c_int,
                                       C.c_int, C.c_float, _fp]),
+    'scf_resize_bilinear2': (C.c_int, [_fp, _fp, _fp, C.c_int64, C.c_float, _fp, _fp, _fp, C.c_int64, C.c_float,
+                                           _fp, C.c_int, C.c_int64, C.c_int, C.c_int, C.c_int, C.c_int, _fp]),
     'scf_convex_upsample': (C.c_int, [_fp, _fp, _fp, C.c_int, C.c_int, C.c_int, C.c_int, C.c_int,
                                       C.c_float, C.c_float, _fp]),
     'scf_avgpool2x2': (C.c_int, [_fp, _fp, C.c_int64, C.c_int, C.c_int, _fp]),
diff --git a/scflow_amd/csrc/conv_kernels.h b/scflow_amd/csrc/conv_kernels.h
--- a/scflow_amd/csrc/conv_kernels.h
+++ b/scflow_amd/csrc/conv_kernels.h
@@ -32,7 +32,12 @@
   int kslices;
   long long slice_ns;
   int slice_blocks;
+  const float* in0_hi; int n_split;
 };
+
+__device__ __forceinline__ const float* scf_conv_in0(const ConvK& p, int n) {
+  return (p.n_split > 0 && n >= p.n_split) ? p.in0_hi + (long long)(n - p.n_split) * p.in0_ns : p.in0 + (long long)n * p.in0_ns;
+}
 
 struct ConvEpi {
   float* out; const float* res; const float* gru_h; float* gru_aux; const float* gru_z;
diff --git a/scflow_amd/csrc/conv_mfma.hip b/scflow_amd/csrc/conv_mfma.hip
--- a/scflow_amd/csrc/conv_mfma.hip
+++ b/scflow_amd/csrc/conv_mfma.hip
@@ -378,7 +378,11 @@
       return SCF_EINVAL;
   }
 
+  if (d->n_split < 0 || (d->n_split > 0 && (!d->in0_hi || d->n_split >= d->N))) return SCF_EINVAL;
+  if (d->n_split > 0 && (d->C1 > 0 || !d->wp_taps || d->k_slices > 1)) return SCF_EUNSUPPORTED;
+
   ConvK& k = plan->k;
+  k.in0_hi = d->n_split > 0 ? d->in0_hi : nullptr; k.n_split = d->n_split > 0 ? d->n_split : 0;
   k.in0 = d->in0; k.in1 = d->C1 > 0 ? d->in1 : nullptr;
   k.C0 = d->C0; k.Cin = d->C0 + d->C1;
   k.in0_ns = d->in0_nstride; k.in1_ns = d->in1_nstride;
@@ -543,6 +547,10 @@
     r.which = SCF_KERNEL_DMA;
     return want_dma(d) ? scf_conv_dma_dispatch(k, N, dry, info, st, r.cap) : SCF_EUNSUPPORTED;
   }
+  if (d->n_split > 0) {
+    r.which = SCF_KERNEL_TAPS;
+    return scf_conv_taps_dispatch(k, d->wp_taps, N, dry, info, st, r.cap);
+  }
   if (took(SCF_KERNEL_THIN, scf_conv_thin_dispatch(k, N, dry, st, r.cap))) return out;
   if (d->wp_taps && took(SCF_KERNEL_TAPS, scf_conv_taps_dispatch(k, d->wp_taps, N, dry, info, st, r.cap))) return out;
   if (d->wp_wino) {
@@ -615,6 +623,8 @@
 int scf_lookup_store_set(int v);
 int scf_iter_merge_set(int v);
 int scf_wino1d4_half_set(int v);
+int scf_pool_merge_set(int v);
+int scf_resize_gather_set(int v);
 
 extern "C" int scf_tune(int key, int value) {
   if (key == SCF_TUNE_WINO_VARIANT) return scf_wino_variant_set(value);
@@ -624,6 +634,8 @@
   if (key == SCF_TUNE_LOOKUP_STORE) return scf_lookup_store_set(value);
   if (key == SCF_TUNE_ITER_MERGE) return scf_iter_merge_set(value);
   if (key == SCF_TUNE_WINO1D4_HALF) return scf_wino1d4_half_set(value);
+  if (key == SCF_TUNE_POOL_MERGE) return scf_pool_merge_set(value);
+  if (key == SCF_TUNE_RESIZE_GATHER) return scf_resize_gather_set(value);
   if (key == SCF_TUNE_CONV_AUTOSLICE) {
     if (value < 0 || value > 1) return SCF_EINVAL;
     return g_autoslice.exchange(value);
diff --git a/scflow_amd/csrc/conv_taps.hip b/scflow_amd/csrc/conv_taps.hip
--- a/scflow_amd/csrc/conv_taps.hip
+++ b/scflow_amd/csrc/conv_taps.hip
@@ -73,7 +73,7 @@
     int n, ty0, tx0;
     tile_coords(tile, n, ty0, tx0);
     const int iy0 = ty0 * st - p.pad_h, ix0 = tx0 * st - p.pad_w;
-    const scf_rsrc4 xrs = scf_make_rsrc(p.in0 + (long long)n * p.in0_ns, (unsigned)((long long)p.Cin * HW * 4));
+    const scf_rsrc4 xrs = scf_make_rsrc(scf_conv_in0(p, n), (unsigned)((long long)p.Cin * HW * 4));
     const int tbase = iy0 * p.W + ix0;
     const unsigned dst = xl + (unsigned)(b * x_cells + wave * 64) * 4u;
 #pragma unroll
diff --git a/scflow_amd/csrc/conv_taps_body.h b/scflow_amd/csrc/conv_taps_body.h
--- a/scflow_amd/csrc/conv_taps_body.h
+++ b/scflow_amd/csrc/conv_taps_body.h
@@ -45,7 +45,7 @@
       scf_bdma_b128(wrs, voff, wl + (unsigned)c0 * 16u);
     }
     const int HW = p.H * p.W;
-    const scf_rsrc4 xrs = scf_make_rsrc(p.in0 + (long long)n * p.in0_ns, (unsigned)((long long)p.Cin * HW * 4));
+    const scf_rsrc4 xrs = scf_make_rsrc(scf_conv_in0(p, n), (unsigned)((long long)p.Cin * HW * 4));
     const unsigned xl = scf_lds_addr(Xs);
     const float rPHW = 1.0f / (float)PHW, rPW = 1.0f / (float)PWp;
     for (int c0 = wave * 64; c0 < x_cells; c0 += 256) {
diff --git a/scflow_amd/csrc/corr_gemm.hip b/scflow_amd/csrc/corr_gemm.hip
--- a/scflow_amd/csrc/corr_gemm.hip
+++ b/scflow_amd/csrc/corr_gemm.hip
@@ -217,6 +217,11 @@
 
 int scf_avgpool2x2_layout(const float* x, float* out, int64_t planes, int Hin, int Win, int in_tiled,
                           int out_tiled, hipStream_t st);
+int scf_avgpool2x2_layout2(const float* x, float* mid, float* out, int64_t planes, int Hin, int Win, int in_tiled,
+                           int mid_tiled, int out_tiled, hipStream_t st);
+
+static std::atomic<int> g_pool_merge{1};
+int scf_pool_merge_set(int v) { return (v < 0 || v > 1) ? SCF_EINVAL : g_pool_merge.exchange(v); }
 
 extern "C" int scf_corr_build_ex(const float* feat1, const float* feat2, float* const* levels, int N,
                                  int C, int h, int w, int L, unsigned tiled_levels, scf_stream_t stream) {
@@ -247,6 +252,13 @@
   }
   if (rc != SCF_OK) return rc;
   for (int l = done; l < L; ++l) {
+    if (l + 1 < L && g_pool_merge.load(std::memory_order_relaxed) != 0) {
+      rc = scf_avgpool2x2_layout2(levels[l - 1], levels[l], levels[l + 1], (int64_t)N * hw, h >> (l - 1), w >> (l - 1),
+                                  (tiled_levels >> (l - 1)) & 1u, (tiled_levels >> l) & 1u, (tiled_levels >> (l + 1)) & 1u, st);
+      if (rc != SCF_OK) return rc;
+      ++l;
+      continue;
+    }
     rc = scf_avgpool2x2_layout(levels[l - 1], levels[l], (int64_t)N * hw, h >> (l - 1), w >> (l - 1),
                                (tiled_levels >> (l - 1)) & 1u, (tiled_levels >> l) & 1u, st);
     if (rc != SCF_OK) return rc;
diff --git a/scflow_amd/csrc/norm.hip b/scflow_amd/csrc/norm.hip
--- a/scflow_amd/csrc/norm.hip
+++ b/scflow_amd/csrc/norm.hip
@@ -119,6 +119,87 @@
   else if (vec && n4 <= 8192) scf_launch((instance_norm_kernel<8, 1024>), grid, dim3(1024), 0, st, x, res, out, HW, eps, relu);
   else if (vec && n4 <= 20480) scf_launch((instance_norm_kernel<20, 1024>), grid, dim3(1024), 0, st, x, res, out, HW, eps, relu);
   else scf_launch(instance_norm_generic_kernel, grid, blk, 0, st, x, res, out, HW, eps, relu);
+  return scf_launch_status();
+}
+
+template <int VEC4>
+__global__ __launch_bounds__(256) void instance_norm_pair_kernel(const float* y, const float* s, float* out, int HW,
+                                                                 float eps, int relu) {
+#pragma clang fp contract(off)
+  constexpr bool FMAQ = VEC4 > 1;
+  __shared__ float red[4];
+  const long long pl = blockIdx.x;
+  const float4* yp = reinterpret_cast<const float4*>(y + pl * HW);
+  const float4* sp = reinterpret_cast<const float4*>(s + pl * HW);
+  const int n4 = HW >> 2;
+  float4 v[VEC4], u[VEC4];
+#pragma unroll
+  for (int i = 0; i < VEC4; ++i) {
+    const int idx = i * 256 + threadIdx.x;
+    v[i] = idx < n4 ? yp[idx] : make_float4(0.f, 0.f, 0.f, 0.f);
+    u[i] = idx < n4 ? sp[idx] : make_float4(0.f, 0.f, 0.f, 0.f);
+  }
+  float sv = 0.f, su = 0.f;
+#pragma unroll
+  for (int i = 0; i < VEC4; ++i) {
+    sv += (v[i].x + v[i].y) + (v[i].z + v[i].w);
+    su += (u[i].x + u[i].y) + (u[i].z + u[i].w);
+  }
+  const float mv = block_sum<256>(sv, red) / (float)HW;
+  const float mu = block_sum<256>(su, red) / (float)HW;
+  float qv = 0.f, qu = 0.f;
+#pragma unroll
+  for (int i = 0; i < VEC4; ++i) {
+    const int idx = i * 256 + threadIdx.x;
+    if (idx < n4) {
+      const float a = v[i].x - mv, b = v[i].y - mv, c = v[i].z - mv, d = v[i].w - mv;
+      const float e = u[i].x - mu, f = u[i].y - mu, g = u[i].z - mu, h = u[i].w - mu;
+      if (FMAQ) {
+        qv += __builtin_fmaf(a, a, b * b) + __builtin_fmaf(c, c, d * d);
+        qu += __builtin_fmaf(e, e, f * f) + __builtin_fmaf(g, g, h * h);
+      } else {
+        qv += (a * a + b * b) + (c * c + d * d);
+        qu += (e * e + f * f) + (g * g + h * h);
+      }
+    }
+  }
+  const float rv = 1.0f / sqrtf(block_sum<256>(qv, red) / (float)HW + eps);
+  const float ru = 1.0f / sqrtf(block_sum<256>(qu, red) / (float)HW + eps);
+  float4* op = reinterpret_cast<float4*>(out + pl * HW);
+#pragma unroll
+  for (int i = 0; i < VEC4; ++i) {
+    const int idx = i * 256 + threadIdx.x;
+    if (idx < n4) {
+      float4 o;
+      o.x = (v[i].x - mv) * rv + (u[i].x - mu) * ru;
+      o.y = (v[i].y - mv) * rv + (u[i].y - mu) * ru;
+      o.z = (v[i].z - mv) * rv + (u[i].z - mu) * ru;
+      o.w = (v[i].w - mv) * rv + (u[i].w - mu) * ru;
+      if (relu) {
+        o.x = fmaxf(o.x, 0.f); o.y = fmaxf(o.y, 0.f); o.z = fmaxf(o.z, 0.f); o.w = fmaxf(o.w, 0.f);
+      }
+      scf_store4<(SCF_ST_SC1 & 2) != 0>(reinterpret_cast<float*>(op + idx), o.x, o.y, o.z, o.w);
+    }
+  }
+}
+
+extern "C" int scf_instance_norm_pair(const float* y, float* s, float* out, int64_t planes, int HW, float eps, int relu,
+                                      scf_stream_t stream) {
+  if (!y || !s || !out || planes <= 0 || HW <= 0) return SCF_EINVAL;
+  if (y == s) return SCF_EINVAL;
+  if (planes > 0x7fffffffLL) return SCF_EUNSUPPORTED;
+  const bool vec = (HW % 4 == 0) && ((((uintptr_t)y | (uintptr_t)s | (uintptr_t)out) & 15) == 0);
+  const int n4 = HW / 4;
+  if (!vec || n4 > 4096) {
+    const int rc = scf_instance_norm(s, nullptr, s, planes, HW, eps, 0, stream);
+    return rc != SCF_OK ? rc : scf_instance_norm(y, s, out, planes, HW, eps, relu, stream);
+  }
+  hipStream_t st = scf_stream(stream);
+  const dim3 grid((unsigned)planes), blk(256);
+  const float* sc = s;
+  if (n4 <= 256) scf_launch(instance_norm_pair_kernel<1>, grid, blk, 0, st, y, sc, out, HW, eps, relu);
+  else if (n4 <= 1024) scf_launch(instance_norm_pair_kernel<4>, grid, blk, 0, st, y, sc, out, HW, eps, relu);
+  else scf_launch(instance_norm_pair_kernel<16>, grid, blk, 0, st, y, sc, out, HW, eps, relu);
   return scf_launch_status();
 }
 
diff --git a/scflow_amd/csrc/resample.hip b/scflow_amd/csrc/resample.hip
--- a/scflow_amd/csrc/resample.hip
+++ b/scflow_amd/csrc/resample.hip
@@ -3,7 +3,7 @@
 struct ResizeJob {
   const float* a; const float* b; float* out; float mul;
 };
-template <bool VEC>
+template <bool VEC, bool NARROW>
 __global__ __launch_bounds__(256) void resize_bilinear_kernel(ResizeJob j0, ResizeJob j1, int planes0,
                                                               int planes, int Hin, int Win,
                                                               int Hout, int Wout, float sh, float sw,
@@ -39,14 +39,40 @@
     const float* s0 = b ? b + base + (long long)y0 * Win : nullptr;
     const float* s1 = b ? b + base + (long long)y1 * Win : nullptr;
     float v[4];
+    float p0[3], p1[3];
+    if (NARROW) {
+#pragma unroll
+      for (int k = 0; k < 3; ++k) {
+        const int c = x0[0] + k < Win - 1 ? x0[0] + k : Win - 1;
+        p0[k] = r0[c];
+        p1[k] = r1[c];
+      }
+      if (b) {
+#pragma unroll
+        for (int k = 0; k < 3; ++k) {
+          const int c = x0[0] + k < Win - 1 ? x0[0] + k : Win - 1;
+          p0[k] += s0[c];
+          p1[k] += s1[c];
+        }
+      }
+    }
 #pragma unroll
     for (int i = 0; i < 4; ++i) {
-      float v00 = r0[x0[i]], v01 = r0[x1[i]], v10 = r1[x0[i]], v11 = r1[x1[i]];
-      if (b) {
-        v00 += s0[x0[i]];
-        v01 += s0[x1[i]];
-        v10 += s1[x0[i]];
-        v11 += s1[x1[i]];
+      float v00, v01, v10, v11;
+      if (NARROW) {
+        const int k0 = x0[i] - x0[0], k1 = x1[i] - x0[0];
+        v00 = k0 == 0 ? p0[0] : p0[1];
+        v10 = k0 == 0 ? p1[0] : p1[1];
+        v01 = k1 == 0 ? p0[0] : k1 == 1 ? p0[1] : p0[2];
+        v11 = k1 == 0 ? p1[0] : k1 == 1 ? p1[1] : p1[2];
+      } else {
+        v00 = r0[x0[i]], v01 = r0[x1[i]], v10 = r1[x0[i]], v11 = r1[x1[i]];
+        if (b) {
+          v00 += s0[x0[i]];
+          v01 += s0[x1[i]];
+          v10 += s1[x0[i]];
+          v11 += s1[x1[i]];
+        }
       }
       const float hx = 1.f - lx[i];
       v[i] = mul * (hy * (hx * v00 + lx[i] * v01) + ly * (hx * v10 + lx[i] * v11));
@@ -68,6 +94,9 @@
     }
   }
 }
+
+static std::atomic<int> g_resize_gather{0};
+int scf_resize_gather_set(int v) { return (v < 0 || v > 1) ? SCF_EINVAL : g_resize_gather.exchange(v); }
 
 int scf_resize_bilinear_jobs(const float* a, const float* b, float* out, int64_t planes, float mul,
                              const float* a1, const float* b1, float* out1, int64_t planes1, float mul1,
@@ -87,13 +116,23 @@
   const ResizeJob j0 = {a, b, out, mul}, j1 = {a1, b1, out1, mul1};
   const bool vec = (Wout & 3) == 0 && ((uintptr_t)out & 15) == 0 && (planes1 == 0 || ((uintptr_t)out1 & 15) == 0) &&
                    (!out2 || (((uintptr_t)out2 & 15) == 0 && (out2_gstride & 3) == 0));
-  if (vec)
-    scf_launch(resize_bilinear_kernel<true>, grid, dim3(256), 0, scf_stream(stream), j0, j1, (int)planes, (int)total,
-               Hin, Win, Hout, Wout, sh, sw, out2, out2_group, (long long)out2_gstride);
-  else
-    scf_launch(resize_bilinear_kernel<false>, grid, dim3(256), 0, scf_stream(stream), j0, j1, (int)planes, (int)total,
-               Hin, Win, Hout, Wout, sh, sw, out2, out2_group, (long long)out2_gstride);
-  return scf_launch_status();
+  const bool narrow = 4LL * (Win - 1) <= (long long)Wout - 1 && g_resize_gather.load(std::memory_order_relaxed) == 0;
+#define SCF_RESIZE_LAUNCH(V, NW)                                                                                          \
+  scf_launch((resize_bilinear_kernel<V, NW>), grid, dim3(256), 0, scf_stream(stream), j0, j1, (int)planes, (int)total, Hin, \
+             Win, Hout, Wout, sh, sw, out2, out2_group, (long long)out2_gstride)
+  if (vec && narrow) SCF_RESIZE_LAUNCH(true, true);
+  else if (vec) SCF_RESIZE_LAUNCH(true, false);
+  else if (narrow) SCF_RESIZE_LAUNCH(false, true);
+  else SCF_RESIZE_LAUNCH(false, false);
+#undef SCF_RESIZE_LAUNCH
+  return scf_launch_status();
+}
+
+extern "C" int scf_resize_bilinear2(const float* a, const float* b, float* out, int64_t planes, float mul, const float* a1,
+                                    const float* b1, float* out1, int64_t planes1, float mul1, float* out2, int out2_group,
+                                    int64_t out2_gstride, int Hin, int Win, int Hout, int Wout, scf_stream_t stream) {
+  return scf_resize_bilinear_jobs(a, b, out, planes, mul, a1, b1, out1, planes1, mul1, out2, out2_group, out2_gstride, Hin, Win,
+                                  Hout, Wout, stream);
 }
 
 extern "C" int scf_resize_bilinear(const float* a, const float* b, float* out, int64_t planes,
@@ -166,6 +205,56 @@
   return scf_launch_status();
 }
 
+__global__ __launch_bounds__(256) void avgpool2x2_layout2_kernel(const float* __restrict__ x, float* __restrict__ mid,
+                                                                 float* __restrict__ out, long long planes, int Win,
+                                                                 int in_pw4, int in_msz, int Hm, int Wm, int mid_pw4,
+                                                                 int mid_msz, int Ho, int Wo, int out_pw4, int out_msz) {
+#pragma clang fp contract(off)
+  const int Hc = (Hm + 1) >> 1, Wc = (Wm + 1) >> 1;
+  const long long total = planes * Hc * Wc;
+  for (long long idx = (long long)blockIdx.x * blockDim.x + threadIdx.x; idx < total;
+       idx += (long long)gridDim.x * blockDim.x) {
+    const int cx = (int)(idx % Wc);
+    const long long t = idx / Wc;
+    const int cy = (int)(t % Hc);
+    const long long pl = t / Hc;
+    const float* s = x + pl * in_msz;
+    float p[2][2];
+#pragma unroll
+    for (int dy = 0; dy < 2; ++dy) {
+#pragma unroll
+      for (int dx = 0; dx < 2; ++dx) {
+        const int my = 2 * cy + dy, mx = 2 * cx + dx;
+        p[dy][dx] = 0.f;
+        if (my < Hm && mx < Wm) {
+          const int y = 2 * my, xx = 2 * mx;
+          const float a = s[pyr_offset(y, xx, in_pw4, Win)], b = s[pyr_offset(y, xx + 1, in_pw4, Win)];
+          const float c = s[pyr_offset(y + 1, xx, in_pw4, Win)], d = s[pyr_offset(y + 1, xx + 1, in_pw4, Win)];
+          p[dy][dx] = (((a + b) + c) + d) * 0.25f;
+          mid[pl * mid_msz + pyr_offset(my, mx, mid_pw4, Wm)] = p[dy][dx];
+        }
+      }
+    }
+    if (cy < Ho && cx < Wo)
+      out[pl * out_msz + pyr_offset(cy, cx, out_pw4, Wo)] = (((p[0][0] + p[0][1]) + p[1][0]) + p[1][1]) * 0.25f;
+  }
+}
+
+int scf_avgpool2x2_layout2(const float* x, float* mid, float* out, int64_t planes, int Hin, int Win, int in_tiled,
+                           int mid_tiled, int out_tiled, hipStream_t st) {
+  if (!x || !mid || !out || planes <= 0 || Hin < 4 || Win < 4) return SCF_EINVAL;
+  const int Hm = Hin / 2, Wm = Win / 2, Ho = Hm / 2, Wo = Wm / 2;
+  const int in_pw = (Win + 7) / 8 * 8, in_ph = (Hin + 3) / 4 * 4;
+  const int mid_pw = (Wm + 7) / 8 * 8, mid_ph = (Hm + 3) / 4 * 4;
+  const int out_pw = (Wo + 7) / 8 * 8, out_ph = (Ho + 3) / 4 * 4;
+  const long long total = (long long)planes * ((Hm + 1) / 2) * ((Wm + 1) / 2);
+  const int grid = (int)(scf_cdiv(total, 256) < 262144 ? scf_cdiv(total, 256) : 262144);
+  scf_launch(avgpool2x2_layout2_kernel, dim3(grid), dim3(256), 0, st, x, mid, out, (long long)planes, Win,
+             in_tiled ? in_pw * 4 : 0, in_tiled ? in_ph * in_pw : Hin * Win, Hm, Wm, mid_tiled ? mid_pw * 4 : 0,
+             mid_tiled ? mid_ph * mid_pw : Hm * Wm, Ho, Wo, out_tiled ? out_pw * 4 : 0, out_tiled ? out_ph * out_pw : Ho * Wo);
+  return scf_launch_status();
+}
+
 __global__ __launch_bounds__(256) void mul_mask_kernel(const float* __restrict__ x, long long xns,
                                                        const float* __restrict__ mask,
                                                        float* __restrict__ out, long long ons, int N,
diff --git a/scflow_amd/modules.py b/scflow_amd/modules.py
--- a/scflow_amd/modules.py
+++ b/scflow_amd/modules.py
@@ -159,11 +159,8 @@
         ops.instance_norm(y, relu=True, out=y)
         y2 = ops.conv2d(p['c2'], y)
         if 'ds' in p:
-            idt = ops.conv2d(p['ds'], x)
-            ops.instance_norm(idt, out=idt)
-        else:
-            idt = x
-        return ops.instance_norm(y2, res=idt, relu=True, out=y2)
+            return ops.instance_norm_pair(y2, ops.conv2d(p['ds'], x), relu=True, out=y2)
+        return ops.instance_norm(y2, res=x, relu=True, out=y2)
 
 
 @ENCODERS.register_module()
@@ -208,12 +205,12 @@
                     head=PackedConv.from_weight(self.conv2.weight, self.conv2.bias, 1, 0))
 
     def forward(self, x: Tensor, out: Optional[Tensor] = None, head_act: int = ACT_NONE,
-                head_act2: int = ACT_NONE, head_split: int = 0) -> Tensor:
+                head_act2: int = ACT_NONE, head_split: int = 0, x_hi: Optional[Tensor] = None) -> Tensor:
         p = self.packed
         if self.kind == 'BN':
-            x = ops.conv2d(p['stem'], x, act=ACT_RELU)
+            x = ops.conv2d(p['stem'], x, act=ACT_RELU, x0_hi=x_hi)
         else:
-            x = ops.conv2d(p['stem'], x)
+            x = ops.conv2d(p['stem'], x, x0_hi=x_hi)
             ops.instance_norm(x, relu=True, out=x)
         for name in self.res_layers:
             for blk in getattr(self, name):
@@ -228,11 +225,12 @@
 
 
 def raft_encoder_pair(fe: 'RAFTEncoder', xf: Tensor, ce: 'RAFTEncoder', xc: Tensor, out_c: Optional[Tensor] = None,
-                      head_act: int = ACT_NONE, head_act2: int = ACT_NONE, head_split: int = 0) -> Tuple[Tensor, Tensor]:
+                      head_act: int = ACT_NONE, head_act2: int = ACT_NONE, head_split: int = 0,
+                      xf_hi: Optional[Tensor] = None) -> Tuple[Tensor, Tensor]:
     if not encoder_pair_supported(fe, ce):
         raise ValueError('raft_encoder_pair: (InstanceNorm feature encoder, BatchNorm context encoder) of one layer geometry')
     pf, pc = fe.packed, ce.packed
-    yf, yc = ops.conv2d_pair((pf['stem'], xf), (pc['stem'], xc, dict(act=ACT_RELU)))
+    yf, yc = ops.conv2d_pair((pf['stem'], xf, dict(x0_hi=xf_hi)), (pc['stem'], xc, dict(act=ACT_RELU)))
     ops.instance_norm(yf, relu=True, out=yf)
     for name in fe.res_layers:
         for bf, bc in zip(getattr(fe, name), getattr(ce, name)):
@@ -241,11 +239,13 @@
             ops.instance_norm(tf_, relu=True, out=tf_)
             if 'ds' in qf:
                 if_, ic_ = ops.conv2d_pair((qf['ds'], yf), (qc['ds'], yc))
-                ops.instance_norm(if_, out=if_)
             else:
                 if_, ic_ = yf, yc
             uf_, yc = ops.conv2d_pair((qf['c2'], tf_), (qc['c2'], tc_, dict(res=ic_, act=ACT_RELU)))
-            yf = ops.instance_norm(uf_, res=if_, relu=True, out=uf_)
+            if 'ds' in qf:
+                yf = ops.instance_norm_pair(uf_, if_, relu=True, out=uf_)
+            else:
+                yf = ops.instance_norm(uf_, res=if_, relu=True, out=uf_)
     return ops.conv2d_pair((pf['head'], yf), (pc['head'], yc, dict(out=out_c, act=head_act, act2=head_act2,
                                                                   act_split=head_split)))
 
diff --git a/scflow_amd/ops.py b/scflow_amd/ops.py
--- a/scflow_amd/ops.py
+++ b/scflow_amd/ops.py
@@ -16,7 +16,7 @@
 
 __all__ = ['record_conv_kernels', 'PackedConv', 'conv_desc', 'gru_passes', 'scflow_iteration', 'side_stream_handle', 'pyramid_layout', 'untile_level', 'level_storage_shape', 'sepconv_gru', 'pack_conv_weight', 'pack_conv_weight_f16x3', 'set_conv_precision', 'set_conv_winograd', 'get_conv_winograd', 'pack_conv_weight_wino', 'pack_conv_weight_wino1d', 'pack_conv_weight_wino1d4',
            'get_conv_precision', 'set_conv_kslices', 'conv_kslices', 'conv_kslices_for', 'constant', 'clear_constants', 'register_conv_workspace', 'choose_kc', 'conv2d', 'conv2d_pair', 'corr_build', 'corr_lookup',
-           'instance_norm', 'group_norm_relu', 'linear', 'fc_splitk', 'fc_slices', 'pose_update', 'reproject_flow',
+           'instance_norm', 'instance_norm_pair', 'group_norm_relu', 'linear', 'fc_splitk', 'fc_slices', 'pose_update', 'reproject_flow', 'resize_bilinear_jobs',
            'flow_corr_2d3d', 'pnp_params', 'pnp_ransac', 'pnp',
            'unproject_depth', 'linear_pair', 'resize_bilinear', 'convex_upsample', 'avgpool2x2', 'copy_channels',
            'ACT_NONE', 'ACT_RELU', 'ACT_SIGMOID', 'ACT_TANH', 'CONV_PLAIN', 'CONV_GRU_ZR',
@@ -395,8 +395,14 @@
            *, res: Optional[Tensor] = None, act: int = ACT_NONE, act2: int = ACT_NONE,
            act_split: int = 0, mode: int = CONV_PLAIN, gru_h: Optional[Tensor] = None,
            gru_aux: Optional[Tensor] = None, gru_z: Optional[Tensor] = None, kslices: int = 1,
-           _launch: bool = True):
+           x0_hi: Optional[Tensor] = None, _launch: bool = True):
     p0, n, c0, h, w, s0 = _nchw(x0, 'x0')
+    n_lo = 0
+    if x0_hi is not None:
+        ph, nh, ch, hh, wh, sh = _nchw(x0_hi, 'x0_hi')
+        if (ch, hh, wh, sh) != (c0, h, w, s0) or x1 is not None or kslices > 1:
+            raise _lib.ScflowHipError('conv2d(x0_hi): one segment, the geometry and sample stride of x0')
+        n_lo, n = n, n + nh
     p1, c1, s1 = None, 0, 0
     if x1 is not None:
         p1, n1, c1, h1, w1, s1 = _nchw(x1, 'x1')
@@ -428,6 +434,8 @@
     d.in0, d.in1, d.C0, d.C1 = p0, p1, c0, c1
     d.in0_nstride, d.in1_nstride = s0, s1
     d.N, d.H, d.W = n, h, w
+    if n_lo:
+        d.in0_hi, d.n_split = ph, n_lo
     d.out, d.out_nstride = po, so
     if sliced is not None:
         d.k_slices, d.out_slice_stride = kslices, sliced.stride(0)
@@ -684,7 +692,7 @@
     return list(zip(_read_timers([e[0] for e in evs]), [e[1] for e in evs], [e[2] for e in evs]))
 
 
-TUNE_KEYS = {'wino_variant': 1, 'dma_force_ksplit': 2, 'dma_ksplit_groups': 3, 'wino1d4': 4, 'lookup_pipe': 5, 'lookup_store': 6, 'conv_autoslice': 7, 'iter_merge': 8, 'wino1d4_half': 9, 'conv_pair': 10}
+TUNE_KEYS = {'wino_variant': 1, 'dma_force_ksplit': 2, 'dma_ksplit_groups': 3, 'wino1d4': 4, 'lookup_pipe': 5, 'lookup_store': 6, 'conv_autoslice': 7, 'iter_merge': 8, 'wino1d4_half': 9, 'conv_pair': 10, 'pool_merge': 11, 'resize_gather': 12}
 
 
 def tune(key: str, value: int) -> int:
@@ -926,6 +934,19 @@
     _lib.check(_lib.load().scf_instance_norm(px, _opt(res, 'res'), _dense(out, 'out'), n * c,
                                              h * w, eps, int(relu), _stream()),
                'scf_instance_norm')
+    return out
+
+
+def instance_norm_pair(y: Tensor, s: Tensor, relu: bool = True, out: Optional[Tensor] = None,
+                       eps: float = 1e-5) -> Tensor:
+    py, ps = _dense(y, 'y'), _dense(s, 's')
+    if y.shape != s.shape:
+        raise _lib.ScflowHipError(f'instance_norm_pair: shapes {tuple(y.shape)} and {tuple(s.shape)}')
+    n, c, h, w = y.shape
+    if out is None:
+        out = torch.empty_like(y)
+    _lib.check(_lib.load().scf_instance_norm_pair(py, ps, _dense(out, 'out'), n * c, h * w, eps, int(relu), _stream()),
+               'scf_instance_norm_pair')
     return out
 
 
@@ -1037,6 +1058,33 @@
         _dense(rot, 'rot'), _dense(trans, 'trans'), _dense(out, 'out'), n, h, w,
         float(invalid_num), _stream()), 'scf_reproject_flow')
     return out
+
+
+def resize_bilinear_jobs(a: Tensor, out_hw: Tuple[int, int], mul: float = 1.0, b: Optional[Tensor] = None,
+                         out: Optional[Tensor] = None, a1: Optional[Tensor] = None, mul1: float = 1.0,
+                         b1: Optional[Tensor] = None, out1: Optional[Tensor] = None, copy: Optional[Tensor] = None):
+    n, c, h, w = a.shape
+    ho, wo = out_hw
+    if out is None:
+        out = torch.empty((n, c, ho, wo), dtype=torch.float32, device=a.device)
+    p1 = pb1 = po1 = None
+    planes1 = 0
+    if a1 is not None:
+        if tuple(a1.shape[2:]) != (h, w):
+            raise _lib.ScflowHipError('resize_bilinear_jobs: both jobs share one geometry')
+        if out1 is None:
+            out1 = torch.empty((a1.shape[0], a1.shape[1], ho, wo), dtype=torch.float32, device=a.device)
+        p1, pb1, po1, planes1 = _dense(a1, 'a1'), _opt(b1, 'b1'), _dense(out1, 'out1'), a1.shape[0] * a1.shape[1]
+    pc, grp, cs = None, 1, 0
+    if copy is not None:
+        if tuple(copy.shape) != (n, c, ho, wo) or copy[0].stride() != out[0].stride():
+            raise _lib.ScflowHipError('resize_bilinear_jobs: copy must be an (N,C,ho,wo) view with dense samples')
+        _dev(copy, 'copy')
+        pc, grp, cs = copy.data_ptr(), c, copy.stride(0)
+    _lib.check(_lib.load().scf_resize_bilinear2(_dense(a, 'a'), _opt(b, 'b'), _dense(out, 'out'), n * c, float(mul),
+                                                    p1, pb1, po1, planes1, float(mul1), pc, grp, cs, h, w, ho, wo,
+                                                    _stream()), 'scf_resize_bilinear2')
+    return out, out1
 
 
 def filter_flow_by_mask_(flow: Tensor, mask: Tensor, invalid_num: float = 400.,
diff --git a/scflow_amd/refiner.py b/scflow_amd/refiner.py
--- a/scflow_amd/refiner.py
+++ b/scflow_amd/refiner.py
@@ -120,20 +120,15 @@
         fork = ops.fork_point() if ov_ctx else None
         if (not self.seperate_encoder and ops.branch_mode(n, H, W, 'context') == 2 and ops._CONV_EVENTS is None
                 and encoder_pair_supported(self.render_encoder, self.context)):
-            both = torch.empty((2 * n, 3, H, W), dtype=torch.float32, device=dev)
-            ops.copy_channels(rend, both[:n])
-            ops.copy_channels(real_images.contiguous(), both[n:])
-            feats, _ = raft_encoder_pair(self.render_encoder, both, self.context, rend, out_c=hx[:, :hc + cc],
-                                         head_act=ACT_TANH, head_act2=ACT_RELU, head_split=hc)
+            feats, _ = raft_encoder_pair(self.render_encoder, rend, self.context, rend, out_c=hx[:, :hc + cc],
+                                         head_act=ACT_TANH, head_act2=ACT_RELU, head_split=hc,
+                                         xf_hi=real_images.contiguous())
             return feats[:n], feats[n:], hx[:, :hc], hx[:, hc:hc + cc]
         if self.seperate_encoder:
             render_feat = self.render_encoder(rend)
             real_feat = self.real_encoder(real_images.contiguous())
         else:
-            both = torch.empty((2 * n, 3, H, W), dtype=torch.float32, device=dev)
-            ops.copy_channels(rend, both[:n])
-            ops.copy_channels(real_images.contiguous(), both[n:])
-            feats = self.render_encoder(both)
+            feats = self.render_encoder(rend, x_hi=real_images.contiguous())
             render_feat, real_feat = feats[:n], feats[n:]
         br = ops.side_stream(ov_ctx, after=fork)
         with br:
```

Result: no change. 2331, median of 6 (+0.5%).
